# lmcinnes/pynndescent

Measured on AMD Instinct MI355X. Metric: index build: points indexed/sec (recall@10 vs brute force reported alongside), higher is better.
Workload: dtype f32

## Files before the change

include/pynnd_amd.h:

```cpp
#ifndef PYNND_AMD_H
#define PYNND_AMD_H

#include <stdint.h>

#ifdef __cplusplus
extern "C" {
#endif

#define NND_METRIC_SQEUCLIDEAN 0
#define NND_METRIC_ALT_COSINE 1
#define NND_METRIC_ALT_DOT 2
#define NND_METRIC_ALT_INNER_PRODUCT 3
#define NND_METRIC_CORRELATION 4
#define NND_METRIC_ALT_HELLINGER 5

#define NND_ABI_VERSION 6

typedef struct nnd_handle_s *nnd_handle_t;

typedef struct nnd_params {
    int64_t n;
    int32_t dim;
    int32_t metric;
    int32_t n_neighbors;
    int32_t n_trees;
    int32_t leaf_size;
    int32_t max_depth;
    int32_t max_candidates;
    int32_t n_iters;
    float delta;
    int64_t rng_state[3];
    int64_t tree_rng[3];
    int32_t device;
    int32_t join_blocks;
    int32_t flags;
    int32_t reserved[5];
} nnd_params;

#define NND_FLAG_NO_GRAPH 1
#define NND_FLAG_NO_PREP 2
#define NND_FLAG_TEST_SELECT_WAVE 4
#define NND_FLAG_TEST_SMALL_REGIONS 8
#define NND_FLAG_TEST_ROUTE_PLAIN 16
#define NND_FLAG_TEST_FOREST_BY_TREE 32
#define NND_FLAG_TEST_FAIL 64
#define NND_FLAG_TEST_VANISH 128
#define NND_FLAG_TEST_SAMPLE_ATOMIC 256
#define NND_FLAG_TEST_FOREST_FALLBACK_TOPS 512
#define NND_FLAG_TEST_FOREST_FALLBACK_SHARE 1024
#define NND_TEST_FALLBACK_AT(flags) ((((flags) & 512) ? 1 : 0) + (((flags) & 1024) ? 2 : 0))
#define NND_FLAG_TEST_SAMPLE_NOMEM 2048
#define NND_FLAG_TEST_SELECT_HALF 4096
#define NND_FLAG_TEST_GATHER_INLINE 8192
#define NND_FLAG_TEST_JOIN_UNSTAGED 16384

typedef struct nnd_stats {
    int64_t n_iters_run;
    int64_t n_leaves;
    int64_t tree_levels;
    int64_t leaf_pairs;
    int64_t leaf_rows;
    int64_t join_pairs[64];
    int64_t join_rows[64];
    int64_t join_active[64];
    int64_t proposals[64];
    int64_t updates[64];
    float ms_prep, ms_forest, ms_leaf_init, ms_random_init, ms_descent, ms_finalize;
    float ms_sample[64], ms_join[64], ms_merge[64];
    int64_t join_mfma[64];
    int64_t leaf_mfma;
    int64_t n_cells;
    int64_t join_substeps[64];
} nnd_stats;

int32_t nnd_abi_version(void);
const char *nnd_last_global_error(void);
const char *nnd_last_error(nnd_handle_t h);

int32_t nnd_create(nnd_handle_t *out, const nnd_params *params);
int32_t nnd_destroy(nnd_handle_t h);
int32_t nnd_release_pending(void);

int32_t nnd_host_copy(void *dst, const void *src, int64_t bytes);
int32_t nnd_host_sqrt_f32(float *dst, const float *src, int64_t count);
void *nnd_host_alloc(int64_t bytes);
int32_t nnd_host_free(void *p);

int32_t nnd_set_data_host(nnd_handle_t h, const float *x);
int32_t nnd_set_data_device(nnd_handle_t h, const float *x_dev);
int32_t nnd_data_nonfinite(nnd_handle_t h, int32_t *out);
int32_t nnd_data_negative(nnd_handle_t h, int32_t *out);

int32_t nnd_make_forest(nnd_handle_t h);
int32_t nnd_leaf_array_shape(nnd_handle_t h, int64_t *n_leaves, int32_t *max_leaf_size);
int32_t nnd_get_leaf_array(nnd_handle_t h, int32_t *out_host);

int32_t nnd_reset_graph(nnd_handle_t h);
int32_t nnd_init_from_leaves(nnd_handle_t h);
int32_t nnd_init_from_leaf_array(nnd_handle_t h, const int32_t *leaf_array, int64_t n_leaves, int32_t max_leaf_size);
int32_t nnd_init_random(nnd_handle_t h);
int32_t nnd_init_from_graph(nnd_handle_t h, const int32_t *init_idx, const float *init_dist, int32_t width);
int32_t nnd_init_from_neighbor_graph(nnd_handle_t h, const int32_t *init_idx, const float *init_dist, int32_t width);

int32_t nnd_descent_iter(nnd_handle_t h, int64_t *c_out);
int32_t nnd_descent(nnd_handle_t h);

int32_t nnd_finalize_host(nnd_handle_t h, int32_t *out_idx, float *out_dist);
int32_t nnd_finalize_device(nnd_handle_t h, int32_t *out_idx_dev, float *out_dist_dev);

int32_t nnd_build_device(nnd_handle_t h, int32_t *out_idx_dev, float *out_dist_dev);

int32_t nnd_build(const nnd_params *params, const float *x, const int32_t *init_idx, const float *init_dist,
                  int32_t init_width, int32_t *out_idx, float *out_dist, nnd_stats *stats, char *err,
                  int32_t errlen);

int32_t nnd_get_stats(nnd_handle_t h, nnd_stats *out);
int32_t nnd_synchronize(nnd_handle_t h);

int32_t nnd_get_graph(nnd_handle_t h, int32_t *idx, float *dist, uint8_t *flags);
int32_t nnd_get_candidates(nnd_handle_t h, int32_t *new_idx, int32_t *old_idx);
int32_t nnd_sample_candidates(nnd_handle_t h);
int32_t nnd_pairwise_gram(nnd_handle_t h, const int32_t *rows_a, int32_t na, const int32_t *rows_b, int32_t nb,
                          float *out);

typedef struct nnd_comm_s *nnd_comm_t;
#define NND_COMM_ID_BYTES 128
int32_t nnd_comm_unique_id(void *id_out );
int32_t nnd_comm_create_rccl(nnd_comm_t *out, const void *id, int32_t world, int32_t rank, int32_t device);
int32_t nnd_comm_create_local(nnd_comm_t *out , int32_t world, const int32_t *devices );
typedef int32_t (*nnd_host_exchange_fn)(void *user, const void *send, const int64_t *send_off, const int64_t *send_bytes,
                                        void *recv, const int64_t *recv_off, const int64_t *recv_bytes);
int32_t nnd_comm_create_host(nnd_comm_t *out, int32_t world, int32_t rank, int32_t device, nnd_host_exchange_fn fn, void *user);
int32_t nnd_comm_add_channel_rccl(nnd_comm_t c, const void *id );
int32_t nnd_comm_set_timeout(nnd_comm_t c, int64_t timeout_ms);
int32_t nnd_comm_destroy(nnd_comm_t c);
int32_t nnd_comm_abort(nnd_comm_t c);
int32_t nnd_comm_info(nnd_comm_t c, int32_t *out );
int32_t nnd_comm_self_test(nnd_comm_t c);
int32_t nnd_comm_local_set_serial(nnd_comm_t c, int32_t on);
const char *nnd_comm_last_error(nnd_comm_t c );

typedef struct nnd_shard_s *nnd_shard_t;
typedef struct nnd_shard_info {
    int64_t n_total, own_lo, own_hi;
    int32_t world, rank, local_trees, iters;
    int64_t c[64];
    int64_t offer_records[64];
    int64_t proposal_records[64];
    int64_t deferred[64];
    int64_t dropped_offers;
    int64_t bytes_sent;
    float ms_total;
    float ms_allgather, ms_klist_exchange;
    int32_t n_sections;
    float section_ms[256];
    int64_t section_bytes[256];
    int32_t forest_by_cell;
    int32_t n_sections_overlap;
    int64_t forest_positions;
    int64_t gather_bytes[64];
    int32_t gather_section[64];
} nnd_shard_info;
int32_t nnd_shard_create(nnd_shard_t *out, const nnd_params *params, nnd_comm_t comm, const int64_t *shard_sizes);
int32_t nnd_shard_build(nnd_shard_t s, const float *x_local_dev, void *x_stream, int32_t *out_idx_dev, float *out_dist_dev);
int32_t nnd_shard_build_from_graph(nnd_shard_t s, const float *x_local_dev, void *x_stream, const int32_t *init_idx_dev,
                                   const float *init_dist_dev, int32_t init_width, int32_t *out_idx_dev, float *out_dist_dev);
int32_t nnd_shard_build_update(nnd_shard_t s, const float *x_local_dev, void *x_stream, const int32_t *old_idx_dev, const float *old_dist_dev,
                               int32_t width, int32_t *out_idx_dev, float *out_dist_dev);
int32_t nnd_shard_get_info(nnd_shard_t s, nnd_shard_info *out);
int32_t nnd_shard_get_stats(nnd_shard_t s, nnd_stats *out);
nnd_handle_t nnd_shard_handle(nnd_shard_t s);
int32_t nnd_shard_destroy(nnd_shard_t s);
const char *nnd_shard_last_error(nnd_shard_t s );

int32_t nnd_build_multi(const nnd_params *params, const float *x, int32_t n_devices, const int32_t *devices, int32_t *out_idx,
                        float *out_dist, nnd_stats *stats, nnd_shard_info *info_rank0 , char *err, int32_t errlen);
int32_t nnd_build_multi_from_graph(const nnd_params *params, const float *x, int32_t n_devices, const int32_t *devices,
                                   const int32_t *init_idx, const float *init_dist, int32_t init_width, int32_t *out_idx, float *out_dist,
                                   nnd_stats *stats, nnd_shard_info *info_rank0 , char *err, int32_t errlen);
int32_t nnd_build_multi_update(const nnd_params *params, const float *x, int32_t n_devices, const int32_t *devices, const int32_t *old_idx,
                               const float *old_dist, int32_t width, int32_t *out_idx, float *out_dist, nnd_stats *stats,
                               nnd_shard_info *info_rank0 , char *err, int32_t errlen);

int32_t nnd_set_stream(nnd_handle_t h, void *hip_stream);
int32_t nnd_descent_sample(nnd_handle_t h);
int32_t nnd_descent_join(nnd_handle_t h);

typedef struct nnd_prune_opts {
    float prune_probability;
    int32_t degree_aware;
    int32_t max_degree;
    float aggressiveness;
    float alpha;
    uint32_t seed;
    int32_t reserved[2];
} nnd_prune_opts;
int32_t nnd_diversify_host(nnd_handle_t h, int32_t *idx, float *dist, const nnd_prune_opts *opts, const int32_t *degree);
int32_t nnd_diversify_csr_host(nnd_handle_t h, const int32_t *indptr, const int32_t *indices, float *data, int64_t nnz,
                               const nnd_prune_opts *opts, const int32_t *degree);
int32_t nnd_degree_prune_host(nnd_handle_t h, const int32_t *indptr, float *data, int64_t nnz, int32_t max_degree);

typedef struct nnd_search_graph_stats {
    int64_t forward_nnz;
    int64_t reverse_nnz;
    int64_t union_nnz;
    int64_t final_nnz;
    float min_distance;
    int32_t max_degree_out;
    float ms_device;
    int32_t reserved[3];
} nnd_search_graph_stats;
int32_t nnd_search_graph(nnd_handle_t h, const int32_t *idx, const float *dist, int32_t on_device, int32_t n_neighbors,
                         float pruning_degree_multiplier, float diversify_prob, int32_t degree_aware, float degree_prune_aggressiveness,
                         uint32_t seed, int32_t *fwd_rows_host, float *fwd_dist_host, nnd_search_graph_stats *stats);
int32_t nnd_search_graph_fetch(nnd_handle_t h, int32_t *indptr_host, int32_t *indices_host);

int32_t nnd_hub_tree_build(nnd_handle_t h, const int32_t *rank_order_host, int32_t leaf_size, int32_t max_depth,
                           int64_t *n_nodes_out);
int32_t nnd_hub_tree_fetch(nnd_handle_t h, float *hyperplanes, float *offsets, int32_t *children, int32_t *indices,
                           int32_t *max_leaf_size);

typedef struct nnd_searcher_s *nnd_searcher_t;
int32_t nnd_searcher_create(nnd_searcher_t *out, int32_t device, int64_t n, int32_t dim, int32_t metric, const float *data,
                            const int32_t *indptr, const int32_t *indices, int64_t nnz, const float *hyperplanes,
                            const float *offsets, const int32_t *children, const int32_t *tree_indices, int64_t n_nodes,
                            float min_distance, int32_t n_neighbors, const int64_t *search_rng_state );
int32_t nnd_searcher_query(nnd_searcher_t s, const float *queries , int64_t nq, int32_t k, float epsilon,
                           int32_t *out_idx , float *out_dist );
int64_t nnd_searcher_last_spilled(nnd_searcher_t s);
int32_t nnd_searcher_set_tier(nnd_searcher_t s, int32_t tier);
int32_t nnd_searcher_quantize_u8(nnd_searcher_t s, const float *rows , const float *values, int32_t n_values,
                                 uint8_t *codes_out );
int32_t nnd_searcher_set_codes_u8(nnd_searcher_t s, const float *values, int32_t n_values, const uint8_t *codes );
int32_t nnd_searcher_query_proxy(nnd_searcher_t s, const float *queries , int64_t nq, int32_t k, int32_t search_k,
                                 float epsilon, int32_t *out_idx , float *out_dist );
int32_t nnd_searcher_destroy(nnd_searcher_t s);
const char *nnd_searcher_last_error(nnd_searcher_t s );

#ifdef __cplusplus
}
#endif
#endif
```

pynndescent_amd/_capi.py:

```python
import ctypes as C
import os

import numpy as np

_HERE = os.path.dirname(os.path.abspath(__file__))
LIB_PATH = os.environ.get("PYNND_AMD_LIB", os.path.join(_HERE, "libpynnd_amd.so"))

NND_METRIC_SQEUCLIDEAN = 0
NND_METRIC_ALT_COSINE = 1
NND_METRIC_ALT_DOT = 2
NND_METRIC_ALT_INNER_PRODUCT = 3
NND_METRIC_CORRELATION = 4
NND_METRIC_ALT_HELLINGER = 5
METRIC_CODES = {"euclidean": NND_METRIC_SQEUCLIDEAN, "l2": NND_METRIC_SQEUCLIDEAN, "sqeuclidean": NND_METRIC_SQEUCLIDEAN,
                "cosine": NND_METRIC_ALT_COSINE, "dot": NND_METRIC_ALT_DOT, "inner_product": NND_METRIC_ALT_INNER_PRODUCT,
                "correlation": NND_METRIC_CORRELATION, "hellinger": NND_METRIC_ALT_HELLINGER}
NND_FLAG_NO_GRAPH = 1
NND_FLAG_NO_PREP = 2
NND_FLAG_TEST_SELECT_WAVE = 4
NND_FLAG_TEST_SMALL_REGIONS = 8
NND_FLAG_TEST_ROUTE_PLAIN = 16
NND_FLAG_TEST_FOREST_BY_TREE = 32
NND_FLAG_TEST_FAIL = 64
NND_FLAG_TEST_VANISH = 128
NND_FLAG_TEST_FOREST_FALLBACK_TOPS = 512
NND_FLAG_TEST_FOREST_FALLBACK_SHARE = 1024
NND_FLAG_TEST_GATHER_INLINE = 8192
NND_FLAG_TEST_JOIN_UNSTAGED = 16384
NND_FLAG_TEST_SELECT_HALF = 4096
NND_FLAG_TEST_SAMPLE_NOMEM = 2048
NND_FLAG_TEST_SAMPLE_ATOMIC = 256


class NNDParams(C.Structure):
    _fields_ = [
        ("n", C.c_int64),
        ("dim", C.c_int32),
        ("metric", C.c_int32),
        ("n_neighbors", C.c_int32),
        ("n_trees", C.c_int32),
        ("leaf_size", C.c_int32),
        ("max_depth", C.c_int32),
        ("max_candidates", C.c_int32),
        ("n_iters", C.c_int32),
        ("delta", C.c_float),
        ("rng_state", C.c_int64 * 3),
        ("tree_rng", C.c_int64 * 3),
        ("device", C.c_int32),
        ("join_blocks", C.c_int32),
        ("flags", C.c_int32),
        ("reserved", C.c_int32 * 5),
    ]


class NNDSearchGraphStats(C.Structure):
    _fields_ = [("forward_nnz", C.c_int64), ("reverse_nnz", C.c_int64), ("union_nnz", C.c_int64), ("final_nnz", C.c_int64),
                ("min_distance", C.c_float), ("max_degree_out", C.c_int32), ("ms_device", C.c_float), ("reserved", C.c_int32 * 3)]


class NNDStats(C.Structure):
    _fields_ = [
        ("n_iters_run", C.c_int64),
        ("n_leaves", C.c_int64),
        ("tree_levels", C.c_int64),
        ("leaf_pairs", C.c_int64),
        ("leaf_rows", C.c_int64),
        ("join_pairs", C.c_int64 * 64),
        ("join_rows", C.c_int64 * 64),
        ("join_active", C.c_int64 * 64),
        ("proposals", C.c_int64 * 64),
        ("updates", C.c_int64 * 64),
        ("ms_prep", C.c_float),
        ("ms_forest", C.c_float),
        ("ms_leaf_init", C.c_float),
        ("ms_random_init", C.c_float),
        ("ms_descent", C.c_float),
        ("ms_finalize", C.c_float),
        ("ms_sample", C.c_float * 64),
        ("ms_join", C.c_float * 64),
        ("ms_merge", C.c_float * 64),
        ("join_mfma", C.c_int64 * 64),
        ("leaf_mfma", C.c_int64),
        ("n_cells", C.c_int64),
        ("join_substeps", C.c_int64 * 64),
    ]

    def as_dict(self):
        it = int(self.n_iters_run)
        m = min(it, 64)
        out = {
            "n_iters_run": it, "n_leaves": int(self.n_leaves), "tree_levels": int(self.tree_levels),
            "leaf_pairs": int(self.leaf_pairs), "leaf_rows": int(self.leaf_rows), "leaf_mfma": int(self.leaf_mfma), "n_cells": int(self.n_cells),
        }
        for name in ("join_pairs", "join_rows", "join_active", "proposals", "updates", "join_mfma", "join_substeps"):
            out[name] = [int(v) for v in getattr(self, name)[:m]]
        for name in ("ms_prep", "ms_forest", "ms_leaf_init", "ms_random_init", "ms_descent", "ms_finalize"):
            out[name] = float(getattr(self, name))
        for name in ("ms_sample", "ms_join", "ms_merge"):
            out[name] = [float(v) for v in getattr(self, name)[:m]]
        return out


class NNDShardInfo(C.Structure):
    _fields_ = [
        ("n_total", C.c_int64), ("own_lo", C.c_int64), ("own_hi", C.c_int64),
        ("world", C.c_int32), ("rank", C.c_int32), ("local_trees", C.c_int32), ("iters", C.c_int32),
        ("c", C.c_int64 * 64),
        ("offer_records", C.c_int64 * 64),
        ("proposal_records", C.c_int64 * 64),
        ("deferred", C.c_int64 * 64),
        ("dropped_offers", C.c_int64),
        ("bytes_sent", C.c_int64),
        ("ms_total", C.c_float), ("ms_allgather", C.c_float), ("ms_klist_exchange", C.c_float),
        ("n_sections", C.c_int32),
        ("section_ms", C.c_float * 256),
        ("section_bytes", C.c_int64 * 256),
        ("forest_by_cell", C.c_int32),
        ("n_sections_overlap", C.c_int32),
        ("forest_positions", C.c_int64),
        ("gather_bytes", C.c_int64 * 64),
        ("gather_section", C.c_int32 * 64),
    ]

    def as_dict(self):
        it = min(int(self.iters), 64)
        ns = int(self.n_sections)
        return {"n_total": int(self.n_total), "range": (int(self.own_lo), int(self.own_hi)), "world": int(self.world),
                "rank": int(self.rank), "local_trees": int(self.local_trees), "iters": int(self.iters),
                "c": [int(v) for v in self.c[:it]], "offer_records": [int(v) for v in self.offer_records[:it]],
                "proposal_records": [int(v) for v in self.proposal_records[:it]],
                "exchanged_records": [int(a) + int(b) for a, b in zip(self.offer_records[:it], self.proposal_records[:it])],
                "deferred": [int(v) for v in self.deferred[:it]], "dropped_offers": int(self.dropped_offers),
                "bytes_sent": int(self.bytes_sent), "ms_total": float(self.ms_total),
                "ms_allgather": float(self.ms_allgather), "ms_klist_exchange": float(self.ms_klist_exchange),
                "section_ms": [float(v) for v in self.section_ms[:ns]],
                "section_bytes": [int(v) for v in self.section_bytes[:ns]],
                "forest_by_cell": bool(self.forest_by_cell), "n_sections_overlap": int(self.n_sections_overlap),
                "forest_positions": int(self.forest_positions),
                "gather_bytes": [int(v) for v in self.gather_bytes[:it]], "gather_section": [int(v) for v in self.gather_section[:it]]}


HOST_EXCHANGE_FN = C.CFUNCTYPE(C.c_int32, C.c_void_p, C.c_void_p, C.POINTER(C.c_int64), C.POINTER(C.c_int64), C.c_void_p,
                               C.POINTER(C.c_int64), C.POINTER(C.c_int64))


class NNDPruneOpts(C.Structure):
    _fields_ = [
        ("prune_probability", C.c_float),
        ("degree_aware", C.c_int32),
        ("max_degree", C.c_int32),
        ("aggressiveness", C.c_float),
        ("alpha", C.c_float),
        ("seed", C.c_uint32),
        ("reserved", C.c_int32 * 2),
    ]


_H = C.c_void_p
_SIGNATURES = [
    ("nnd_abi_version", C.c_int32, []),
    ("nnd_last_global_error", C.c_char_p, []),
    ("nnd_last_error", C.c_char_p, [_H]),
    ("nnd_create", C.c_int32, [C.POINTER(_H), C.POINTER(NNDParams)]),
    ("nnd_destroy", C.c_int32, [_H]),
    ("nnd_set_data_host", C.c_int32, [_H, C.c_void_p]),
    ("nnd_set_data_device", C.c_int32, [_H, C.c_void_p]),
    ("nnd_data_nonfinite", C.c_int32, [_H, C.POINTER(C.c_int32)]),
    ("nnd_data_negative", C.c_int32, [_H, C.POINTER(C.c_int32)]),
    ("nnd_release_pending", C.c_int32, []),
    ("nnd_host_copy", C.c_int32, [C.c_void_p, C.c_void_p, C.c_int64]),
    ("nnd_host_sqrt_f32", C.c_int32, [C.c_void_p, C.c_void_p, C.c_int64]),
    ("nnd_host_alloc", C.c_void_p, [C.c_int64]),
    ("nnd_host_free", C.c_int32, [C.c_void_p]),
    ("nnd_make_forest", C.c_int32, [_H]),
    ("nnd_leaf_array_shape", C.c_int32, [_H, C.POINTER(C.c_int64), C.POINTER(C.c_int32)]),
    ("nnd_get_leaf_array", C.c_int32, [_H, C.c_void_p]),
    ("nnd_reset_graph", C.c_int32, [_H]),
    ("nnd_init_from_leaves", C.c_int32, [_H]),
    ("nnd_init_from_leaf_array", C.c_int32, [_H, C.c_void_p, C.c_int64, C.c_int32]),
    ("nnd_init_random", C.c_int32, [_H]),
    ("nnd_init_from_graph", C.c_int32, [_H, C.c_void_p, C.c_void_p, C.c_int32]),
    ("nnd_init_from_neighbor_graph", C.c_int32, [_H, C.c_void_p, C.c_void_p, C.c_int32]),
    ("nnd_descent_iter", C.c_int32, [_H, C.POINTER(C.c_int64)]),
    ("nnd_descent", C.c_int32, [_H]),
    ("nnd_finalize_host", C.c_int32, [_H, C.c_void_p, C.c_void_p]),
    ("nnd_finalize_device", C.c_int32, [_H, C.c_void_p, C.c_void_p]),
    ("nnd_build_device", C.c_int32, [_H, C.c_void_p, C.c_void_p]),
    ("nnd_build", C.c_int32, [C.POINTER(NNDParams), C.c_void_p, C.c_void_p, C.c_void_p, C.c_int32, C.c_void_p,
                              C.c_void_p, C.POINTER(NNDStats), C.c_char_p, C.c_int32]),
    ("nnd_get_stats", C.c_int32, [_H, C.POINTER(NNDStats)]),
    ("nnd_synchronize", C.c_int32, [_H]),
    ("nnd_get_graph", C.c_int32, [_H, C.c_void_p, C.c_void_p, C.c_void_p]),
    ("nnd_get_candidates", C.c_int32, [_H, C.c_void_p, C.c_void_p]),
    ("nnd_sample_candidates", C.c_int32, [_H]),
    ("nnd_pairwise_gram", C.c_int32, [_H, C.c_void_p, C.c_int32, C.c_void_p, C.c_int32, C.c_void_p]),
    ("nnd_descent_sample", C.c_int32, [_H]),
    ("nnd_descent_join", C.c_int32, [_H]),
    ("nnd_set_stream", C.c_int32, [_H, C.c_void_p]),
    ("nnd_comm_unique_id", C.c_int32, [C.c_void_p]),
    ("nnd_comm_create_rccl", C.c_int32, [C.POINTER(_H), C.c_void_p, C.c_int32, C.c_int32, C.c_int32]),
    ("nnd_comm_create_local", C.c_int32, [C.POINTER(_H), C.c_int32, C.c_void_p]),
    ("nnd_comm_create_host", C.c_int32, [C.POINTER(_H), C.c_int32, C.c_int32, C.c_int32, C.c_void_p, C.c_void_p]),
    ("nnd_comm_add_channel_rccl", C.c_int32, [_H, C.c_void_p]),
    ("nnd_comm_set_timeout", C.c_int32, [_H, C.c_int64]),
    ("nnd_comm_info", C.c_int32, [_H, C.POINTER(C.c_int32)]),
    ("nnd_comm_self_test", C.c_int32, [_H]),
    ("nnd_comm_destroy", C.c_int32, [_H]),
    ("nnd_comm_abort", C.c_int32, [_H]),
    ("nnd_comm_local_set_serial", C.c_int32, [_H, C.c_int32]),
    ("nnd_comm_last_error", C.c_char_p, [_H]),
    ("nnd_shard_create", C.c_int32, [C.POINTER(_H), C.POINTER(NNDParams), _H, C.c_void_p]),
    ("nnd_shard_build", C.c_int32, [_H, C.c_void_p, C.c_void_p, C.c_void_p, C.c_void_p]),
    ("nnd_shard_get_info", C.c_int32, [_H, C.POINTER(NNDShardInfo)]),
    ("nnd_shard_get_stats", C.c_int32, [_H, C.POINTER(NNDStats)]),
    ("nnd_shard_handle", _H, [_H]),
    ("nnd_shard_destroy", C.c_int32, [_H]),
    ("nnd_shard_last_error", C.c_char_p, [_H]),
    ("nnd_build_multi", C.c_int32, [C.POINTER(NNDParams), C.c_void_p, C.c_int32, C.c_void_p, C.c_void_p, C.c_void_p,
                                    C.POINTER(NNDStats), C.POINTER(NNDShardInfo), C.c_char_p, C.c_int32]),
    ("nnd_build_multi_from_graph", C.c_int32, [C.POINTER(NNDParams), C.c_void_p, C.c_int32, C.c_void_p, C.c_void_p, C.c_void_p, C.c_int32,
                                               C.c_void_p, C.c_void_p, C.POINTER(NNDStats), C.POINTER(NNDShardInfo), C.c_char_p, C.c_int32]),
    ("nnd_shard_build_from_graph", C.c_int32, [_H, C.c_void_p, C.c_void_p, C.c_void_p, C.c_void_p, C.c_int32, C.c_void_p, C.c_void_p]),
    ("nnd_shard_build_update", C.c_int32, [_H, C.c_void_p, C.c_void_p, C.c_void_p, C.c_void_p, C.c_int32, C.c_void_p, C.c_void_p]),
    ("nnd_build_multi_update", C.c_int32, [C.POINTER(NNDParams), C.c_void_p, C.c_int32, C.c_void_p, C.c_void_p, C.c_void_p, C.c_int32,
                                           C.c_void_p, C.c_void_p, C.POINTER(NNDStats), C.POINTER(NNDShardInfo), C.c_char_p, C.c_int32]),
    ("nnd_diversify_host", C.c_int32, [_H, C.c_void_p, C.c_void_p, C.POINTER(NNDPruneOpts), C.c_void_p]),
    ("nnd_diversify_csr_host", C.c_int32, [_H, C.c_void_p, C.c_void_p, C.c_void_p, C.c_int64, C.POINTER(NNDPruneOpts),
                                           C.c_void_p]),
    ("nnd_degree_prune_host", C.c_int32, [_H, C.c_void_p, C.c_void_p, C.c_int64, C.c_int32]),
    ("nnd_search_graph", C.c_int32, [_H, C.c_void_p, C.c_void_p, C.c_int32, C.c_int32, C.c_float, C.c_float, C.c_int32, C.c_float, C.c_uint32,
                                     C.c_void_p, C.c_void_p, C.POINTER(NNDSearchGraphStats)]),
    ("nnd_search_graph_fetch", C.c_int32, [_H, C.c_void_p, C.c_void_p]),
    ("nnd_hub_tree_build", C.c_int32, [_H, C.c_void_p, C.c_int32, C.c_int32, C.POINTER(C.c_int64)]),
    ("nnd_hub_tree_fetch", C.c_int32, [_H, C.c_void_p, C.c_void_p, C.c_void_p, C.c_void_p, C.POINTER(C.c_int32)]),
    ("nnd_searcher_create", C.c_int32, [C.POINTER(_H), C.c_int32, C.c_int64, C.c_int32, C.c_int32, C.c_void_p, C.c_void_p, C.c_void_p,
                                        C.c_int64, C.c_void_p, C.c_void_p, C.c_void_p, C.c_void_p, C.c_int64, C.c_float, C.c_int32,
                                        C.c_void_p]),
    ("nnd_searcher_query", C.c_int32, [_H, C.c_void_p, C.c_int64, C.c_int32, C.c_float, C.c_void_p, C.c_void_p]),
    ("nnd_searcher_last_spilled", C.c_int64, [_H]),
    ("nnd_searcher_set_tier", C.c_int32, [_H, C.c_int32]),
    ("nnd_searcher_quantize_u8", C.c_int32, [_H, C.c_void_p, C.c_void_p, C.c_int32, C.c_void_p]),
    ("nnd_searcher_set_codes_u8", C.c_int32, [_H, C.c_void_p, C.c_int32, C.c_void_p]),
    ("nnd_searcher_query_proxy", C.c_int32, [_H, C.c_void_p, C.c_int64, C.c_int32, C.c_int32, C.c_float, C.c_void_p, C.c_void_p]),
    ("nnd_searcher_destroy", C.c_int32, [_H]),
    ("nnd_searcher_last_error", C.c_char_p, [_H]),
]
EXPORTED_SYMBOLS = [s[0] for s in _SIGNATURES]

_lib = None


def load_library():
    global _lib
    if _lib is not None:
        return _lib
    if not os.path.exists(LIB_PATH):
        raise RuntimeError(
            "%s not found: build it with `python -c 'import __graft_entry__ as g; g.build()'` or "
            "`make -C pynndescent_amd/csrc`. pynndescent_amd has no CPU fallback." % LIB_PATH
        )
    lib = C.CDLL(LIB_PATH)
    for name, restype, argtypes in _SIGNATURES:
        fn = getattr(lib, name)
        fn.restype = restype
        fn.argtypes = argtypes
    _lib = lib
    return lib


def _ptr(a):
    return None if a is None else a.ctypes.data_as(C.c_void_p)


class NNDError(RuntimeError):
    pass


class Builder:

    def __init__(self, n, dim, metric, n_neighbors, n_trees, leaf_size, max_depth, max_candidates, n_iters, delta,
                 rng_state, tree_rng, device=0, join_blocks=0, flags=0):
        self.lib = load_library()
        p = NNDParams()
        p.n, p.dim, p.metric = int(n), int(dim), int(metric)
        p.n_neighbors, p.n_trees, p.leaf_size = int(n_neighbors), int(n_trees), int(leaf_size)
        p.max_depth, p.max_candidates, p.n_iters = int(max_depth), int(max_candidates), int(n_iters)
        p.delta = float(delta)
        for i in range(3):
            p.rng_state[i] = int(rng_state[i])
            p.tree_rng[i] = int(tree_rng[i])
        p.device, p.join_blocks, p.flags = int(device), int(join_blocks), int(flags)
        self.params = p
        self.n, self.dim, self.k, self.mc = int(n), int(dim), int(n_neighbors), int(max_candidates)
        self._h = _H()
        if self.lib.nnd_create(C.byref(self._h), C.byref(p)) != 0:
            raise NNDError(self.lib.nnd_last_global_error().decode())
        self._keepalive = None

    def _check(self, rc):
        if rc != 0:
            raise NNDError(self.lib.nnd_last_error(self._h).decode())

    def close(self):
        if getattr(self, "_h", None) is not None and self._h.value:
            self.lib.nnd_destroy(self._h)
            self._h = _H()

    def __del__(self):
        try:
            self.close()
        except Exception:
            pass

    def set_data_host(self, x):
        x = np.ascontiguousarray(x, dtype=np.float32)
        assert x.shape == (self.n, self.dim)
        self._check(self.lib.nnd_set_data_host(self._h, _ptr(x)))

    def data_nonfinite(self):
        out = C.c_int32()
        self._check(self.lib.nnd_data_nonfinite(self._h, C.byref(out)))
        return bool(out.value)

    def data_negative(self):
        out = C.c_int32()
        self._check(self.lib.nnd_data_negative(self._h, C.byref(out)))
        return bool(out.value)

    def set_data_device(self, dev_ptr, keepalive=None):
        self._keepalive = keepalive
        self._check(self.lib.nnd_set_data_device(self._h, C.c_void_p(int(dev_ptr))))

    def make_forest(self):
        self._check(self.lib.nnd_make_forest(self._h))

    def leaf_array(self):
        nl, ms = C.c_int64(), C.c_int32()
        self._check(self.lib.nnd_leaf_array_shape(self._h, C.byref(nl), C.byref(ms)))
        out = np.empty((max(nl.value, 1), max(ms.value, 1)), np.int32)
        self._check(self.lib.nnd_get_leaf_array(self._h, _ptr(out)))
        return out[: nl.value]

    def reset_graph(self):
        self._check(self.lib.nnd_reset_graph(self._h))

    def init_from_leaves(self):
        self._check(self.lib.nnd_init_from_leaves(self._h))

    def init_from_leaf_array(self, leaf_array):
        la = np.ascontiguousarray(leaf_array, dtype=np.int32)
        assert la.ndim == 2
        self._check(self.lib.nnd_init_from_leaf_array(self._h, _ptr(la), la.shape[0], la.shape[1]))

    def init_random(self):
        self._check(self.lib.nnd_init_random(self._h))

    def init_from_graph(self, idx, dist=None):
        idx = np.ascontiguousarray(idx, np.int32)
        dist = None if dist is None else np.ascontiguousarray(dist, np.float32)
        self._check(self.lib.nnd_init_from_graph(self._h, _ptr(idx), _ptr(dist), idx.shape[1]))

    def init_from_neighbor_graph(self, idx, dist):
        idx = np.ascontiguousarray(idx, np.int32)
        dist = np.ascontiguousarray(dist, np.float32)
        self._check(self.lib.nnd_init_from_neighbor_graph(self._h, _ptr(idx), _ptr(dist), idx.shape[1]))

    def descent_iter(self):
        c = C.c_int64()
        self._check(self.lib.nnd_descent_iter(self._h, C.byref(c)))
        return c.value

    def descent(self):
        self._check(self.lib.nnd_descent(self._h))

    def sample_candidates(self):
        self._check(self.lib.nnd_sample_candidates(self._h))

    def finalize(self):
        idx = host_pool.empty((self.n, self.k), np.int32)
        dist = host_pool.empty((self.n, self.k), np.float32)
        self._check(self.lib.nnd_finalize_host(self._h, _ptr(idx), _ptr(dist)))
        return idx, dist

    def finalize_device(self, idx_ptr, dist_ptr):
        self._check(self.lib.nnd_finalize_device(self._h, C.c_void_p(int(idx_ptr)), C.c_void_p(int(dist_ptr))))

    def build_device(self, idx_ptr, dist_ptr):
        self._check(self.lib.nnd_build_device(self._h, C.c_void_p(int(idx_ptr)), C.c_void_p(int(dist_ptr))))

    def synchronize(self):
        self._check(self.lib.nnd_synchronize(self._h))

    def stats(self, raw=False):
        s = NNDStats()
        self._check(self.lib.nnd_get_stats(self._h, C.byref(s)))
        return s if raw else s.as_dict()

    def graph(self):
        idx = np.empty((self.n, self.k), np.int32)
        dist = np.empty((self.n, self.k), np.float32)
        flags = np.empty((self.n, self.k), np.uint8)
        self._check(self.lib.nnd_get_graph(self._h, _ptr(idx), _ptr(dist), _ptr(flags)))
        return idx, dist, flags

    def candidates(self):
        new = np.empty((self.n, self.mc), np.int32)
        old = np.empty((self.n, self.mc), np.int32)
        self._check(self.lib.nnd_get_candidates(self._h, _ptr(new), _ptr(old)))
        return new, old

    def set_stream(self, stream_ptr):
        self._check(self.lib.nnd_set_stream(self._h, C.c_void_p(int(stream_ptr)) if stream_ptr else None))

    def descent_sample(self):
        self._check(self.lib.nnd_descent_sample(self._h))

    def descent_join(self):
        self._check(self.lib.nnd_descent_join(self._h))

    @staticmethod
    def _prune_opts(prune_probability=1.0, degree_aware=False, max_degree=1, aggressiveness=1.0, alpha=1.0, seed=0):
        o = NNDPruneOpts()
        o.prune_probability, o.degree_aware, o.max_degree = float(prune_probability), int(bool(degree_aware)), int(max_degree)
        o.aggressiveness, o.alpha, o.seed = float(aggressiveness), float(alpha), int(seed) & 0xFFFFFFFF
        return o

    def diversify(self, idx, dist, degree=None, **opts):
        idx = np.ascontiguousarray(idx, np.int32).copy()
        dist = np.ascontiguousarray(dist, np.float32).copy()
        assert idx.shape == (self.n, self.k) and dist.shape == idx.shape
        o = self._prune_opts(**opts)
        degree = None if degree is None else np.ascontiguousarray(degree, np.int32)
        self._check(self.lib.nnd_diversify_host(self._h, _ptr(idx), _ptr(dist), C.byref(o), _ptr(degree)))
        return idx, dist

    def diversify_csr(self, indptr, indices, data, degree=None, **opts):
        indptr = np.ascontiguousarray(indptr, np.int32)
        indices = np.ascontiguousarray(indices, np.int32)
        data = np.ascontiguousarray(data, np.float32).copy()
        assert indptr.shape[0] == self.n + 1
        o = self._prune_opts(**opts)
        degree = None if degree is None else np.ascontiguousarray(degree, np.int32)
        self._check(self.lib.nnd_diversify_csr_host(self._h, _ptr(indptr), _ptr(indices), _ptr(data), data.shape[0],
                                                    C.byref(o), _ptr(degree)))
        return data

    def search_graph(self, idx, dist, n_neighbors, pruning_degree_multiplier=1.5, diversify_prob=1.0, degree_aware=False,
                     degree_prune_aggressiveness=1.0, seed=0, on_device=False, want_forward=False):
        st = NNDSearchGraphStats()
        fr = fd = None
        if want_forward:
            fr = np.empty((self.n, self.k), np.int32)
            fd = np.empty((self.n, self.k), np.float32)
        if on_device:
            pi, pd = C.c_void_p(int(idx)), C.c_void_p(int(dist))
        else:
            idx = np.ascontiguousarray(idx, dtype=np.int32)
            dist = np.ascontiguousarray(dist, dtype=np.float32)
            assert idx.shape == (self.n, self.k) and dist.shape == (self.n, self.k)
            pi, pd = _ptr(idx), _ptr(dist)
        self._check(self.lib.nnd_search_graph(self._h, pi, pd, 1 if on_device else 0, int(n_neighbors), float(pruning_degree_multiplier),
                                              float(diversify_prob), 1 if degree_aware else 0, float(degree_prune_aggressiveness),
                                              int(seed) & 0xFFFFFFFF, _ptr(fr) if want_forward else None, _ptr(fd) if want_forward else None,
                                              C.byref(st)))
        indptr = np.empty(self.n + 1, np.int32)
        indices = np.empty(max(int(st.final_nnz), 1), np.int32)
        self._check(self.lib.nnd_search_graph_fetch(self._h, _ptr(indptr), _ptr(indices)))
        stats = {f: getattr(st, f) for f, _ in NNDSearchGraphStats._fields_ if f != "reserved"}
        out = (indptr, indices[: int(st.final_nnz)], stats)
        return out + (fr, fd) if want_forward else out

    def degree_prune(self, indptr, data, max_degree):
        indptr = np.ascontiguousarray(indptr, np.int32)
        data = np.ascontiguousarray(data, np.float32).copy()
        self._check(self.lib.nnd_degree_prune_host(self._h, _ptr(indptr), _ptr(data), data.shape[0], int(max_degree)))
        return data

    def hub_tree(self, rank_order, leaf_size, max_depth):
        ro = np.ascontiguousarray(rank_order, np.int32)
        assert ro.shape == (self.n,)
        nn = C.c_int64()
        self._check(self.lib.nnd_hub_tree_build(self._h, _ptr(ro), int(leaf_size), int(max_depth), C.byref(nn)))
        hyper = np.empty((nn.value, self.dim), np.float32)
        offs = np.empty((nn.value,), np.float32)
        children = np.empty((nn.value, 2), np.int32)
        indices = np.empty((self.n,), np.int32)
        ml = C.c_int32()
        self._check(self.lib.nnd_hub_tree_fetch(self._h, _ptr(hyper), _ptr(offs), _ptr(children), _ptr(indices), C.byref(ml)))
        return hyper, offs, children, indices, int(ml.value)

    def pairwise_gram(self, rows_a, rows_b):
        a = np.ascontiguousarray(rows_a, np.int32)
        b = np.ascontiguousarray(rows_b, np.int32)
        out = np.empty((a.shape[0], b.shape[0]), np.float32)
        self._check(self.lib.nnd_pairwise_gram(self._h, _ptr(a), a.shape[0], _ptr(b), b.shape[0], _ptr(out)))
        return out


class Searcher:

    def __init__(self, data, search_graph, tree, metric, min_distance, n_neighbors, search_rng_state, device=0):
        self.lib = load_library()
        data = np.ascontiguousarray(data, np.float32)
        self.n, self.dim = data.shape
        indptr = np.ascontiguousarray(search_graph.indptr, np.int32)
        indices = np.ascontiguousarray(search_graph.indices, np.int32)
        if tree is not None:
            hyper = np.ascontiguousarray(tree.hyperplanes, np.float32)
            offs = np.ascontiguousarray(tree.offsets, np.float32)
            children = np.ascontiguousarray(tree.children, np.int32)
            tidx = np.ascontiguousarray(tree.indices, np.int32)
            n_nodes = hyper.shape[0]
        else:
            hyper = offs = children = tidx = None
            n_nodes = 0
        rng = np.ascontiguousarray(search_rng_state, np.int64)
        self.has_codes = False
        self._h = _H()
        rc = self.lib.nnd_searcher_create(C.byref(self._h), int(device), self.n, self.dim, int(metric), _ptr(data), _ptr(indptr),
                                          _ptr(indices), int(indices.shape[0]), _ptr(hyper), _ptr(offs), _ptr(children), _ptr(tidx),
                                          int(n_nodes), float(min_distance), int(n_neighbors), _ptr(rng))
        if rc != 0:
            raise NNDError(self.lib.nnd_searcher_last_error(None).decode())

    def query(self, queries, k, epsilon):
        q = np.ascontiguousarray(queries, np.float32)
        assert q.ndim == 2 and q.shape[1] == self.dim
        idx = np.empty((q.shape[0], k), np.int32)
        dist = np.empty((q.shape[0], k), np.float32)
        if self.lib.nnd_searcher_query(self._h, _ptr(q), q.shape[0], int(k), float(epsilon), _ptr(idx), _ptr(dist)) != 0:
            raise NNDError(self.lib.nnd_searcher_last_error(self._h).decode())
        return idx, dist

    def quantize_u8(self, values, rows=None, fetch=True):
        values = np.ascontiguousarray(values, np.float32)
        if rows is not None:
            rows = np.ascontiguousarray(rows, np.float32)
            assert rows.shape == (self.n, self.dim)
        codes = np.empty((self.n, self.dim), np.uint8) if fetch else None
        if self.lib.nnd_searcher_quantize_u8(self._h, _ptr(rows), _ptr(values), int(values.shape[0]), _ptr(codes)) != 0:
            raise NNDError(self.lib.nnd_searcher_last_error(self._h).decode())
        self.has_codes = True
        return codes

    def set_codes_u8(self, values, codes):
        values = np.ascontiguousarray(values, np.float32)
        codes = np.ascontiguousarray(codes, np.uint8)
        assert codes.shape == (self.n, self.dim)
        if self.lib.nnd_searcher_set_codes_u8(self._h, _ptr(values), int(values.shape[0]), _ptr(codes)) != 0:
            raise NNDError(self.lib.nnd_searcher_last_error(self._h).decode())
# ... 109 lines not shown
```

pynndescent_amd/csrc/capi.hip:

```cpp
#include <stdlib.h>
#include <string.h>

#include <atomic>
#include <mutex>
#include <string>
#include <thread>
#include <vector>

#include "common.h"
#include "state.h"

static thread_local char g_err[512] = {0};

static void gerr(const char *fmt, ...) {
    va_list ap;
    va_start(ap, fmt);
    vsnprintf(g_err, sizeof(g_err), fmt, ap);
    va_end(ap);
}

extern "C" int32_t nnd_abi_version(void) { return NND_ABI_VERSION; }
extern "C" const char *nnd_last_global_error(void) { return g_err; }
extern "C" const char *nnd_last_error(nnd_handle_t h) { return h ? h->err : g_err; }

#define API_HIP(expr)                                                                                \
    do {                                                                                             \
        hipError_t _e = (expr);                                                                      \
        if (_e != hipSuccess) {                                                                      \
            ctx->set_error("%s failed: %s (%s:%d)", #expr, hipGetErrorString(_e), __FILE__, __LINE__); \
            return 1;                                                                                \
        }                                                                                            \
    } while (0)

void nnd_release_parked();
template <typename T>
static int dalloc(nnd_ctx *ctx, T **p, size_t count) {
    if (hipMalloc((void **)p, sizeof(T) * (count ? count : 1)) != hipSuccess) {
        (void)hipGetLastError();
        nnd_release_parked();
        API_HIP(hipMalloc((void **)p, sizeof(T) * (count ? count : 1)));
    }
    static const int poison = [] { const char *e = nnd_knob("NND_POISON"); return e ? atoi(e) : 0; }();
    if (poison) {
        API_HIP(hipMemsetAsync(*p, poison & 0xFF, sizeof(T) * (count ? count : 1), ctx->stream));
        API_HIP(hipStreamSynchronize(ctx->stream));
    }
    return 0;
}

struct nnd_scratch {
    std::vector<void *> ptrs;
    ~nnd_scratch() {
        for (void *p : ptrs)
            if (p) (void)hipFree(p);
    }
    template <typename T>
    T *get(nnd_ctx *ctx, size_t count) {
        void *p = nullptr;
        hipError_t e = hipMalloc(&p, sizeof(T) * (count ? count : 1));
        if (e != hipSuccess) {
            ctx->set_error("hipMalloc of %zu scratch bytes failed: %s", sizeof(T) * count, hipGetErrorString(e));
            return nullptr;
        }
        ptrs.push_back(p);
        return (T *)p;
    }
};

std::recursive_mutex &nnd_lifecycle_mutex() {
#ifdef NND_TEST_NO_LIFECYCLE_LOCK
    static thread_local std::recursive_mutex m;
#else
    static std::recursive_mutex m;
#endif
    return m;
}

static void free_all(nnd_ctx *ctx) {
    auto F = [](void *p) {
        if (p) (void)hipFree(p);
    };
    if (ctx->x_owned) F((void *)ctx->x_orig);
    for (void *&a : ctx->slim_alloc) { F(a); a = nullptr; }
    F(ctx->xp); F(ctx->nrm); F(ctx->nr2); F(ctx->xh); F(ctx->mean); F(ctx->knn_e); F(ctx->knn_d); F(ctx->th); F(ctx->pbuf_r);
    F(ctx->pdirty); F(ctx->out_idx); F(ctx->out_dist);
    F(ctx->rv_pos); F(ctx->rv_in_cursor); F(ctx->rv_in_rec); F(ctx->rv_ov);
    for (int i = 0; i < 2; i++) { F(ctx->perm[i]); F(ctx->pos_seg[i]); F(ctx->seg_start[i]); F(ctx->seg_len[i]); }
    F(ctx->inv); F(ctx->side); F(ctx->side_pt); F(ctx->leaf_flag); F(ctx->scan_out); F(ctx->scan_blk); F(ctx->seg_nleft); F(ctx->seg_child);
    F(ctx->xs); F(ctx->xsh); F(ctx->nr2s); F(ctx->node_hf); F(ctx->node_hh); F(ctx->node_child); F(ctx->node_pack); F(ctx->node_hfc); F(ctx->route_roots); F(ctx->route_ws); F(ctx->s_leaf_depth);
    F(ctx->cell_count); F(ctx->cell_start); F(ctx->cell_depth); F(ctx->small_list);
    F(ctx->hyper); F(ctx->hyper_h); F(ctx->leaf_start); F(ctx->leaf_len); F(ctx->wl_start); F(ctx->wl_len); F(ctx->colsum_partial); F(ctx->counters_sum);
    if (ctx->h_pin) { (void)hipHostFree(ctx->h_pin); ctx->h_pin = nullptr; }
    if (ctx->h_tree_begin) { (void)hipHostFree(ctx->h_tree_begin); ctx->h_tree_begin = nullptr; }
    F(ctx->tree_begin_dev); F(ctx->counters);
    if (ctx->ev0) (void)hipEventDestroy(ctx->ev0);
    if (ctx->ev1) (void)hipEventDestroy(ctx->ev1);
    if (ctx->ev_spin) (void)hipEventDestroy(ctx->ev_spin);
    for (hipEvent_t e : ctx->tev) if (e) (void)hipEventDestroy(e);
    ctx->tev.clear();
    F(ctx->shard_bounds); F(ctx->shard_cursors);
    nnd_hub_tree_free(ctx);
    nnd_search_graph_free(ctx);
    if (ctx->stream && ctx->stream_owned) (void)hipStreamDestroy(ctx->stream);
}

static nnd_ctx *take_parked(const nnd_params *p);
extern "C" int32_t nnd_create(nnd_handle_t *out, const nnd_params *p) { return nnd_create_impl(out, p, nullptr, 0, 0); }

static void jb_knobs(nnd_ctx *ctx) {
    if (const char *e = nnd_knob("NND_JB_MAX")) ctx->jb_max = atoi(e) < 1 ? 1 : atoi(e);
    if (const char *e = nnd_knob("NND_JB_DIV")) ctx->jb_div = atoi(e) < 1 ? 1 : atoi(e);
    if (const char *e = nnd_knob("NND_JB_FIRST")) ctx->jb_first = atoi(e) < 0 ? 0 : atoi(e);
}
static int auto_join_blocks(int k, int mc) { return (k <= 64 ? 1 : (k + 31) / 32) * (mc > 64 ? 2 : 1); }

int nnd_create_impl(nnd_handle_t *out, const nnd_params *p, const int64_t *bounds_host, int n_ranks, int rank) {
    if (!out || !p) { gerr("nnd_create: null argument"); return 1; }
    *out = nullptr;
    if (p->n < 1 || p->dim < 1) { gerr("nnd_create: need n >= 1 and dim >= 1 (got n=%lld dim=%d)", (long long)p->n, p->dim); return 1; }
    if (p->metric < NND_METRIC_SQEUCLIDEAN || p->metric > NND_METRIC_ALT_HELLINGER) { gerr("nnd_create: unknown metric %d", p->metric); return 1; }
    if (p->n_neighbors < 1 || p->n_neighbors > NND_WIDE_K) { gerr("nnd_create: n_neighbors must be in 1..%d (got %d)", NND_WIDE_K, p->n_neighbors); return 1; }
    if (p->max_candidates < 1 || p->max_candidates > 128) { gerr("nnd_create: max_candidates must be in 1..128 (got %d)", p->max_candidates); return 1; }
    if (p->n_trees < 0 || p->n_trees > 4096 || p->leaf_size < 1) { gerr("nnd_create: bad n_trees (0..4096) / leaf_size"); return 1; }
    if (p->n >= (int64_t)0x7FFFFFF0) { gerr("nnd_create: n too large for int32 ids"); return 1; }
    if (p->n_trees > 0 && (int64_t)p->n_trees * p->n >= (int64_t)0x7FFFFFF0) {
        gerr("nnd_create: n_trees * n = %lld exceeds the forest's int32 position space (2^31)", (long long)((int64_t)p->n_trees * p->n));
        return 1;
    }
    int ndev = 0;
    if (hipGetDeviceCount(&ndev) != hipSuccess || ndev == 0) { gerr("nnd_create: no HIP device visible (this library has no CPU path)"); return 1; }
    if (p->device < 0 || p->device >= ndev) { gerr("nnd_create: device %d out of range (%d visible)", p->device, ndev); return 1; }
    hipDeviceProp_t prop;
    if (hipGetDeviceProperties(&prop, p->device) != hipSuccess) { gerr("nnd_create: hipGetDeviceProperties failed"); return 1; }
    if (strncmp(prop.gcnArchName, "gfx950", 6) != 0) { gerr("nnd_create: device %d is %s; this build targets gfx950 (MI355X) only", p->device, prop.gcnArchName); return 1; }
    if (hipSetDevice(p->device) != hipSuccess) { gerr("nnd_create: hipSetDevice failed"); return 1; }
    if (!bounds_host) {
        if (nnd_ctx *parked = take_parked(p)) {
            *out = parked;
            return 0;
        }
        nnd_release_parked();
    }

    std::lock_guard<std::recursive_mutex> lifecycle(nnd_lifecycle_mutex());
    nnd_ctx *ctx = new nnd_ctx();
    ctx->p = *p;
    ctx->n = p->n;
    ctx->own_lo = 0;
    ctx->own_hi = p->n;
    if (bounds_host) {
        if (n_ranks < 1 || n_ranks > 64 || rank < 0 || rank >= n_ranks || bounds_host[0] != 0 || bounds_host[n_ranks] != p->n) {
            gerr("nnd_create: bad shard bounds (need 1 <= n_ranks <= 64, bounds from 0 to n)");
            delete ctx;
            return 1;
        }
        for (int r = 0; r < n_ranks; r++)
            if (bounds_host[r] > bounds_host[r + 1]) { gerr("nnd_create: shard bounds must not decrease"); delete ctx; return 1; }
        ctx->n_ranks = n_ranks;
        ctx->own_lo = bounds_host[rank];
        ctx->own_hi = bounds_host[rank + 1];
        ctx->slim = n_ranks > 1;
    }
    ctx->d = p->dim;
    ctx->dp = (p->dim + 31) & ~31;
    ctx->k = p->n_neighbors;
    ctx->ks = (p->n_neighbors + 15) & ~15;
    ctx->mc = p->max_candidates;
    ctx->mcp = p->max_candidates <= 16 ? 16 : (p->max_candidates <= 32 ? 32 : (p->max_candidates <= 64 ? 64 : 128));
    if (ctx->ks > 64 && ctx->mcp < 32) ctx->mcp = 32;
    ctx->rcap = p->max_candidates <= 32 ? 32 : (p->max_candidates <= 64 ? 64 : 128);
    if (const char *rc_env = nnd_knob("NND_RCAP")) {
        const int r = atoi(rc_env);
        if (r == 16 || r == 32 || r == 64) ctx->rcap = r;
    }
    ctx->pcap = 64;
    if (const char *pc_env = nnd_knob("NND_PCAP")) {
        const int r = atoi(pc_env);
        if (r == 16 || r == 32 || r == 64) ctx->pcap = r;
    }
    ctx->jb_auto = ctx->p.join_blocks < 1;
    if (ctx->p.join_blocks < 1) ctx->p.join_blocks = auto_join_blocks(ctx->p.n_neighbors, ctx->p.max_candidates);
    jb_knobs(ctx);
    ctx->seed = nnd_mix32((uint32_t)p->rng_state[0] ^ nnd_mix32((uint32_t)p->rng_state[1] + 0x9E3779B9u) ^
                          nnd_mix32((uint32_t)p->rng_state[2] + 0x7F4A7C15u));
    ctx->tree_seed = nnd_mix32((uint32_t)p->tree_rng[0] ^ nnd_mix32((uint32_t)p->tree_rng[1] + 0x9E3779B9u) ^
                               nnd_mix32((uint32_t)p->tree_rng[2] + 0x7F4A7C15u));
    int rc = 0;
    do {
        if (hipStreamCreateWithFlags(&ctx->stream, hipStreamNonBlocking) != hipSuccess) { ctx->set_error("hipStreamCreate failed"); rc = 1; break; }
        if (hipEventCreate(&ctx->ev0) != hipSuccess || hipEventCreate(&ctx->ev1) != hipSuccess ||
            hipEventCreateWithFlags(&ctx->ev_spin, hipEventDisableTiming) != hipSuccess) { ctx->set_error("hipEventCreate failed"); rc = 1; break; }
        const size_t n = (size_t)ctx->n;
        const bool graph = !(p->flags & NND_FLAG_NO_GRAPH), prepared = !(p->flags & NND_FLAG_NO_PREP);
        if (!prepared && graph) { ctx->set_error("NND_FLAG_NO_PREP needs NND_FLAG_NO_GRAPH (the build reads the prepared rows)"); rc = 1; break; }
        if (prepared) {
            if ((rc = dalloc(ctx, &ctx->xp, n * ctx->dp))) break;
            if ((rc = dalloc(ctx, &ctx->nrm, n))) break;
            if (p->n_trees > 0 && (rc = dalloc(ctx, &ctx->xh, n * ctx->dp))) break;
            if (p->n_trees > 0 && (rc = dalloc(ctx, &ctx->nr2, n))) break;
            if ((rc = dalloc(ctx, &ctx->mean, (size_t)ctx->dp + 4))) break;
        }
        if (graph) {
            if ((rc = dalloc(ctx, &ctx->knn_e, n * ctx->ks))) break;
            if ((rc = dalloc(ctx, &ctx->knn_d, n * ctx->ks))) break;
            if ((rc = dalloc(ctx, &ctx->th, n))) break;
            const size_t rows = ctx->slim ? (size_t)(ctx->own_hi - ctx->own_lo) : n;
            int32_t *a_cand = nullptr;
            uint32_t *a_rbuf = nullptr;
            uint8_t *a_active = nullptr;
            if ((rc = dalloc(ctx, &a_cand, rows * 2 * ctx->mcp))) break;
            ctx->slim_alloc[0] = a_cand;
            if ((rc = dalloc(ctx, &a_rbuf, rows * 2 * ctx->rcap))) break;
            ctx->slim_alloc[1] = a_rbuf;
            if ((rc = dalloc(ctx, &a_active, rows))) break;
            ctx->slim_alloc[2] = a_active;
            ctx->cand = a_cand - (size_t)ctx->own_lo * (ctx->slim ? 1 : 0) * 2 * ctx->mcp;
            ctx->rbuf = a_rbuf - (size_t)ctx->own_lo * (ctx->slim ? 1 : 0) * 2 * ctx->rcap;
            ctx->active = a_active - (size_t)ctx->own_lo * (ctx->slim ? 1 : 0);
            uint64_t *a_pbuf = nullptr;
            if ((rc = dalloc(ctx, &a_pbuf, rows * ctx->pcap))) break;
            ctx->slim_alloc[3] = a_pbuf;
            ctx->pbuf = a_pbuf - (size_t)ctx->own_lo * (ctx->slim ? 1 : 0) * ctx->pcap;
            if (ctx->slim && (rc = dalloc(ctx, &ctx->pbuf_r, n * ctx->pcap_r))) break;
            if ((rc = dalloc(ctx, &ctx->pdirty, n))) break;
            if (hipMemsetAsync(ctx->pdirty, 0, n, ctx->stream) != hipSuccess) { ctx->set_error("hipMemset failed"); rc = 1; break; }
            if (ctx->n_ranks > 0) {
                if (hipMalloc((void **)&ctx->shard_bounds, sizeof(int64_t) * 65) != hipSuccess || hipMalloc((void **)&ctx->shard_cursors, sizeof(long long) * 66) != hipSuccess ||
                    hipMemcpy(ctx->shard_bounds, bounds_host, sizeof(int64_t) * (size_t)(n_ranks + 1), hipMemcpyHostToDevice) != hipSuccess) {
                    ctx->set_error("allocation of the shard tables failed"); rc = 1; break;
                }
            }
        }
        if ((rc = dalloc(ctx, &ctx->counters, (size_t)CNT_COUNT * NND_CNT_STRIPES))) break;
        if ((rc = dalloc(ctx, &ctx->counters_sum, (size_t)CNT_COUNT))) break;
        if (hipHostMalloc((void **)&ctx->h_pin, sizeof(nnd_pin_words), hipHostMallocDefault) != hipSuccess) { ctx->set_error("hipHostMalloc failed"); rc = 1; break; }
        memset(ctx->h_pin, 0, sizeof(nnd_pin_words));
        if (hipHostGetDevicePointer((void **)&ctx->h_pin_dev, ctx->h_pin, 0) != hipSuccess) { (void)hipGetLastError(); ctx->h_pin_dev = nullptr; }
        if (p->n_trees > 0) {
            ctx->P = (int64_t)p->n_trees * ctx->n;
            const size_t P = (size_t)ctx->P;
            ctx->max_segs = ctx->P / (p->leaf_size + 1) + p->n_trees + 8;
            const char *whole = nnd_knob("NND_FOREST_WHOLE");
            if (graph && p->n >= 131072 && ctx->dp <= 256 && !(whole && whole[0] == '1')) {
                const char *ss = nnd_knob("NND_SAMPLE_STRIDE");
                ctx->s_stride = ss ? atoi(ss) : 16;
                if (ctx->s_stride < 2) ctx->s_stride = 2;
                ctx->s_m = p->n / ctx->s_stride;
                const char *cl = nnd_knob("NND_CELL_LEAF");
                const char *es = nnd_knob("NND_EARLY_STOP");
                ctx->early_stop = es ? atoi(es) : 0;
                ctx->cell_leaf = cl ? atoi(cl) : 24;
                if (ctx->cell_leaf < 8) ctx->cell_leaf = 8;
                const int64_t Ps = (int64_t)p->n_trees * ctx->s_m;
                ctx->node_cap = Ps / (ctx->cell_leaf / 4 > 1 ? ctx->cell_leaf / 4 : 1) + 4 * p->n_trees + 64;
                ctx->cell_cap = ctx->node_cap + p->n_trees;
                ctx->max_segs += ctx->cell_cap;
                if ((rc = dalloc(ctx, &ctx->xs, (size_t)ctx->s_m * ctx->dp))) break;
                if ((rc = dalloc(ctx, &ctx->xsh, (size_t)ctx->s_m * ctx->dp))) break;
                if ((rc = dalloc(ctx, &ctx->nr2s, (size_t)ctx->s_m))) break;
                if ((rc = dalloc(ctx, &ctx->node_hf, (size_t)ctx->node_cap * (ctx->dp + 4)))) break;
                if ((rc = dalloc(ctx, &ctx->node_hh, (size_t)ctx->node_cap * ctx->dp))) break;
                if ((rc = dalloc(ctx, &ctx->node_child, (size_t)ctx->node_cap * 2))) break;
                if ((rc = dalloc(ctx, &ctx->node_pack, (size_t)ctx->node_cap * (2 * ctx->dp + 16)))) break;
                if ((rc = dalloc(ctx, &ctx->node_hfc, (size_t)ctx->node_cap * (ctx->dp + 4)))) break;
                if ((rc = dalloc(ctx, &ctx->route_roots, (size_t)NND_ROUTE_ROOTS_WORDS))) break;
                if ((rc = dalloc(ctx, &ctx->s_leaf_depth, (size_t)Ps))) break;
                if ((rc = dalloc(ctx, &ctx->cell_count, (size_t)ctx->cell_cap))) break;
                if ((rc = dalloc(ctx, &ctx->cell_start, (size_t)ctx->cell_cap))) break;
                if ((rc = dalloc(ctx, &ctx->cell_depth, (size_t)ctx->cell_cap))) break;
                if ((rc = dalloc(ctx, &ctx->small_list, (size_t)ctx->cell_cap * NND_WORK_LIST_ROWS))) break;
            }
            const size_t S = (size_t)ctx->max_segs;
            for (int i = 0; i < 2 && !rc; i++) {
                if ((rc = dalloc(ctx, &ctx->perm[i], P))) break;
                if ((rc = dalloc(ctx, &ctx->pos_seg[i], P))) break;
                if ((rc = dalloc(ctx, &ctx->seg_start[i], S))) break;
                if ((rc = dalloc(ctx, &ctx->seg_len[i], S))) break;
            }
            if (rc) break;
            if ((rc = dalloc(ctx, &ctx->inv, P))) break;
            if ((rc = dalloc(ctx, &ctx->side, P))) break;
            if ((rc = dalloc(ctx, &ctx->side_pt, P))) break;
            if ((rc = dalloc(ctx, &ctx->leaf_flag, P))) break;
            if ((rc = dalloc(ctx, &ctx->scan_out, P + 1))) break;
            if ((rc = dalloc(ctx, &ctx->scan_blk, P / 2048 + 2))) break;
            if ((rc = dalloc(ctx, &ctx->seg_nleft, S))) break;
            if ((rc = dalloc(ctx, &ctx->seg_child, (NND_SEG_CHILD_WORDS + NND_WORK_LIST_ROWS) * S))) break;
            if ((rc = dalloc(ctx, &ctx->hyper, S * (size_t)(ctx->dp + 4)))) break;
            if ((rc = dalloc(ctx, &ctx->hyper_h, S * (size_t)ctx->dp))) break;
            if ((rc = dalloc(ctx, &ctx->tree_begin_dev, (size_t)4097))) break;
            if (hipHostMalloc((void **)&ctx->h_tree_begin, sizeof(long long) * (size_t)4097, hipHostMallocDefault) != hipSuccess) { ctx->set_error("hipHostMalloc failed"); rc = 1; break; }
        }
    } while (0);
    if (rc) {
        gerr("nnd_create: %s", ctx->err);
        free_all(ctx);
        delete ctx;
        return 1;
    }
    *out = ctx;
    return 0;
}

static std::mutex g_park_mu;
static nnd_ctx *g_parked = nullptr;

static void destroy_now(nnd_ctx *ctx) {
    std::lock_guard<std::recursive_mutex> lifecycle(nnd_lifecycle_mutex());
    (void)hipSetDevice(ctx->p.device);
    if (ctx->stream) (void)hipStreamSynchronize(ctx->stream);
    free_all(ctx);
    delete ctx;
}
void nnd_release_parked() {
    nnd_ctx *old = nullptr;
    {
        std::lock_guard<std::mutex> lk(g_park_mu);
        old = g_parked;
        g_parked = nullptr;
    }
    if (old) destroy_now(old);
}
static bool same_geometry(const nnd_params &a, const nnd_params &b) {
    return a.n == b.n && a.dim == b.dim && a.metric == b.metric && a.n_neighbors == b.n_neighbors && a.n_trees == b.n_trees &&
           a.leaf_size == b.leaf_size && a.max_candidates == b.max_candidates && a.device == b.device && a.flags == b.flags;
}
static nnd_ctx *take_parked(const nnd_params *p) {
    nnd_ctx *ctx = nullptr;
    {
        std::lock_guard<std::mutex> lk(g_park_mu);
        if (g_parked && same_geometry(g_parked->p, *p)) {
            ctx = g_parked;
            g_parked = nullptr;
        }
    }
    if (!ctx) return nullptr;
    (void)hipSetDevice(p->device);
    ctx->p = *p;
    jb_knobs(ctx);
    ctx->jb_auto = ctx->p.join_blocks < 1;
    if (ctx->p.join_blocks < 1) ctx->p.join_blocks = auto_join_blocks(ctx->p.n_neighbors, ctx->p.max_candidates);
    ctx->seed = nnd_mix32((uint32_t)p->rng_state[0] ^ nnd_mix32((uint32_t)p->rng_state[1] + 0x9E3779B9u) ^ nnd_mix32((uint32_t)p->rng_state[2] + 0x7F4A7C15u));
    ctx->tree_seed = nnd_mix32((uint32_t)p->tree_rng[0] ^ nnd_mix32((uint32_t)p->tree_rng[1] + 0x9E3779B9u) ^ nnd_mix32((uint32_t)p->tree_rng[2] + 0x7F4A7C15u));
    ctx->iter = 0;
    ctx->stats = nnd_stats{};
    ctx->err[0] = 0;
    ctx->forest_built = false;
    ctx->h_leaf_valid = false;
    ctx->n_leaves = 0;
    ctx->max_leaf = 0;
    ctx->own_order = nullptr;
    ctx->lists_replicated = false;
    nnd_hub_tree_free(ctx);
    if (!ctx->stream_owned) {
        ctx->stream = nullptr;
        if (hipStreamCreateWithFlags(&ctx->stream, hipStreamNonBlocking) != hipSuccess) { destroy_now(ctx); return nullptr; }
        ctx->stream_owned = true;
    }
    if (!ctx->x_owned) ctx->x_orig = nullptr;
    ctx->x_valid = false;
    ctx->tlog.clear();
    ctx->tev_used = 0;
    return ctx;
}

extern "C" int32_t nnd_destroy(nnd_handle_t ctx) {
    if (!ctx) return 0;
    (void)hipSetDevice(ctx->p.device);
    if (ctx->stream) (void)hipStreamSynchronize(ctx->stream);
    nnd_ctx *old = nullptr;
    if (ctx->n_ranks == 0) {
        std::lock_guard<std::mutex> lk(g_park_mu);
        old = g_parked;
        g_parked = ctx;
    } else {
        old = ctx;
    }
    if (old) destroy_now(old);
    return 0;
}
extern "C" int32_t nnd_release_pending(void) {
    nnd_release_parked();
    return 0;
}

#define ENTER(ctx)                                           \
    if (!ctx) { gerr("null handle"); return 1; }             \
    API_HIP(hipSetDevice(ctx->p.device));

static int need_data(nnd_ctx *ctx) {
    if (!ctx->x_orig || !ctx->x_valid) { ctx->set_error("no data set (call nnd_set_data_host/device first)"); return 1; }
    return 0;
}
static int need_graph(nnd_ctx *ctx) {
    if (ctx->p.flags & NND_FLAG_NO_GRAPH) { ctx->set_error("this handle was created with NND_FLAG_NO_GRAPH: it has no k-lists / candidate tables (pruning pass and hub tree only)"); return 1; }
    return 0;
}

static int after_data(nnd_ctx *ctx) {
    if (ctx->p.flags & NND_FLAG_NO_PREP) return 0;
    const int t_ = t_begin(ctx);
    if (nnd_launch_prep(ctx)) return 1;
    if (!(ctx->p.flags & NND_FLAG_NO_GRAPH) && nnd_launch_reset_graph(ctx)) return 1;
    t_end(ctx, t_, &ctx->stats.ms_prep, false);
    t_flush(ctx);
    return 0;
}

static std::mutex g_up_mu[64];
static char *g_up_stage[64][16] = {};
static hipEvent_t g_up_ev[64][16] = {};
static int h2d_parallel(nnd_ctx *ctx, void *dst_dev, const void *src, size_t bytes) {
    constexpr size_t STAGE = (size_t)8 << 20;
    int P = 8;
    if (const char *e = nnd_knob("NND_H2D_THREADS")) { const int v = atoi(e); if (v >= 1 && v <= 16) P = v; }
    bool direct = bytes < (size_t)(16u << 20) || ctx->p.device < 0 || ctx->p.device >= 64;
    if (!direct) {
        hipPointerAttribute_t at;
        if (hipPointerGetAttributes(&at, src) == hipSuccess && at.type == hipMemoryTypeHost) direct = true;
        else (void)hipGetLastError();
    }
    if (direct) {
        API_HIP(hipMemcpyAsync(dst_dev, src, bytes, hipMemcpyHostToDevice, ctx->stream));
        return 0;
    }
    const int dev = ctx->p.device;
    std::lock_guard<std::mutex> lk(g_up_mu[dev]);
    API_HIP(hipSetDevice(dev));
    for (int b = 0; b < P; b++) {
        if (!g_up_stage[dev][b] && hipHostMalloc((void **)&g_up_stage[dev][b], STAGE, hipHostMallocDefault) != hipSuccess) {
            (void)hipGetLastError();
            g_up_stage[dev][b] = nullptr;
            API_HIP(hipMemcpyAsync(dst_dev, src, bytes, hipMemcpyHostToDevice, ctx->stream));
            return 0;
        }
        if (!g_up_ev[dev][b]) API_HIP(hipEventCreateWithFlags(&g_up_ev[dev][b], hipEventDisableTiming));
    }
    const size_t nchunks = (bytes + STAGE - 1) / STAGE;
    std::atomic<int> failed{0};
    hipStream_t st = ctx->stream;
    auto work = [&](int t) {
        if (hipSetDevice(dev) != hipSuccess) { failed = 1; return; }
        bool first = true;
        for (size_t c = (size_t)t; c < nchunks && !failed; c += P) {
            const size_t o = c * STAGE, len = bytes - o < STAGE ? bytes - o : STAGE;
            if (!first && hipEventSynchronize(g_up_ev[dev][t]) != hipSuccess) { failed = 1; return; }
            first = false;
            memcpy(g_up_stage[dev][t], (const char *)src + o, len);
            if (hipMemcpyAsync((char *)dst_dev + o, g_up_stage[dev][t], len, hipMemcpyHostToDevice, st) != hipSuccess ||
                hipEventRecord(g_up_ev[dev][t], st) != hipSuccess) { failed = 1; return; }
        }
        if (!first && hipEventSynchronize(g_up_ev[dev][t]) != hipSuccess) failed = 1;
    };
    std::vector<std::thread> th;
    for (int t = 1; t < P; t++) th.emplace_back(work, t);
    work(0);
    for (auto &t : th) t.join();
    if (failed) {
        (void)hipStreamSynchronize(st);
        (void)hipGetLastError();
        ctx->set_error("nnd_set_data_host: staged host-to-device copy failed");
        return 1;
    }
// ... 298 lines not shown
                if (po >= len) break;
                const size_t pl = len - po < piece ? len - po : piece;
                th.emplace_back([=] { memcpy(to + po, from + po, pl); });
            }
            memcpy(to, from, len < piece ? len : piece);
            for (auto &t : th) t.join();
        }
    }
    return 0;
}

template <typename F>
static void host_parallel(size_t bytes, size_t unit, F fn) {
    const size_t total = bytes / unit;
    int parts = bytes >= ((size_t)32 << 20) ? 16 : (bytes >= ((size_t)4 << 20) ? 8 : 1);
    const unsigned hc = std::thread::hardware_concurrency();
    if (hc && (unsigned)parts > hc) parts = (int)hc;
    const size_t per = ((total + parts - 1) / parts + (4096 / unit) - 1) / (4096 / unit) * (4096 / unit);
    std::vector<std::thread> th;
    for (int t = 1; t < parts; t++) {
        const size_t o = (size_t)t * per;
        if (o >= total) break;
        const size_t c = total - o < per ? total - o : per;
        th.emplace_back([=] { fn(o, c); });
    }
    fn(0, total < per ? total : per);
    for (auto &t : th) t.join();
}
extern "C" void *nnd_host_alloc(int64_t bytes) {
    void *p = nullptr;
    if (bytes <= 0) return nullptr;
    if (hipHostMalloc(&p, (size_t)bytes, hipHostMallocDefault) != hipSuccess) {
        (void)hipGetLastError();
        return nullptr;
    }
    return p;
}
extern "C" int32_t nnd_host_free(void *p) {
    if (p && hipHostFree(p) != hipSuccess) { (void)hipGetLastError(); gerr("nnd_host_free: not a pointer of nnd_host_alloc"); return 1; }
    return 0;
}
extern "C" int32_t nnd_host_copy(void *dst, const void *src, int64_t bytes) {
    if (bytes < 0 || (bytes > 0 && (!dst || !src))) { gerr("nnd_host_copy: bad arguments"); return 1; }
    host_parallel((size_t)bytes, 1, [=](size_t o, size_t c) { memcpy((char *)dst + o, (const char *)src + o, c); });
    return 0;
}
#if !defined(__HIP_DEVICE_COMPILE__) && (defined(__x86_64__) || defined(_M_X64))
#include <immintrin.h>
__attribute__((target("avx2"))) static void host_sqrt_avx2(float *dst, const float *src, size_t n) {
    size_t i = 0;
    for (; i + 8 <= n; i += 8) _mm256_storeu_ps(dst + i, _mm256_sqrt_ps(_mm256_loadu_ps(src + i)));
    for (; i < n; i++) dst[i] = sqrtf(src[i]);
}
static bool host_has_avx2() { return __builtin_cpu_supports("avx2"); }
#else
static void host_sqrt_avx2(float *dst, const float *src, size_t n) { for (size_t i = 0; i < n; i++) dst[i] = sqrtf(src[i]); }
static bool host_has_avx2() { return false; }
#endif
extern "C" int32_t nnd_host_sqrt_f32(float *dst, const float *src, int64_t count) {
    if (count < 0 || (count > 0 && (!dst || !src))) { gerr("nnd_host_sqrt_f32: bad arguments"); return 1; }
    const bool avx2 = host_has_avx2();
    host_parallel((size_t)count * sizeof(float), sizeof(float), [=](size_t o, size_t c) {
        if (avx2) host_sqrt_avx2(dst + o, src + o, c);
        else
            for (size_t i = o; i < o + c; i++) dst[i] = sqrtf(src[i]);
    });
    return 0;
}

static int out_buffers(nnd_ctx *ctx, size_t cnt) {
    if (cnt <= ctx->out_cap) return 0;
    if (ctx->out_idx) { API_HIP(hipFree(ctx->out_idx)); ctx->out_idx = nullptr; }
    if (ctx->out_dist) { API_HIP(hipFree(ctx->out_dist)); ctx->out_dist = nullptr; }
    ctx->out_cap = 0;
    API_HIP(hipMalloc((void **)&ctx->out_idx, sizeof(int32_t) * cnt));
    API_HIP(hipMalloc((void **)&ctx->out_dist, sizeof(float) * cnt));
    ctx->out_cap = cnt;
    return 0;
}

extern "C" int32_t nnd_finalize_host(nnd_handle_t ctx, int32_t *out_idx, float *out_dist) {
    ENTER(ctx);
    if (need_graph(ctx)) return 1;
    if (need_data(ctx)) return 1;
    size_t cnt = (size_t)(ctx->own_hi - ctx->own_lo) * ctx->k;
    if (out_buffers(ctx, cnt)) return 1;
    if (nnd_finalize_device(ctx, ctx->out_idx, ctx->out_dist)) return 1;
    if (d2h_parallel(ctx, out_idx, ctx->out_idx, sizeof(int32_t) * cnt, 4)) return 1;
    if (d2h_parallel(ctx, out_dist, ctx->out_dist, sizeof(float) * cnt, 4)) return 1;
    return 0;
}

extern "C" int32_t nnd_build_device(nnd_handle_t ctx, int32_t *out_idx_dev, float *out_dist_dev) {
    ENTER(ctx);
    if (need_graph(ctx)) return 1;
    if (need_data(ctx)) return 1;
    if (nnd_launch_reset_graph(ctx)) return 1;
    if (ctx->p.n_trees > 0) {
        const int tf = t_begin(ctx);
        if (nnd_launch_forest(ctx)) return 1;
        t_end(ctx, tf, &ctx->stats.ms_forest, false);
        const int tl = t_begin(ctx);
        if (nnd_launch_leaf_init(ctx)) return 1;
        t_end(ctx, tl, &ctx->stats.ms_leaf_init, false);
    }
    const int tr = t_begin(ctx);
    if (nnd_launch_random_init(ctx)) return 1;
    t_end(ctx, tr, &ctx->stats.ms_random_init, false);
    if (descent_loop(ctx, true)) return 1;
    const int t_ = t_begin(ctx);
    if (nnd_launch_finalize(ctx, out_idx_dev, out_dist_dev)) return 1;
    t_end(ctx, t_, &ctx->stats.ms_finalize, false);
    t_flush(ctx);
    return 0;
}

extern "C" int32_t nnd_build(const nnd_params *params, const float *x, const int32_t *init_idx, const float *init_dist,
                             int32_t init_width, int32_t *out_idx, float *out_dist, nnd_stats *stats, char *err,
                             int32_t errlen) {
    auto fail = [&](const char *msg) {
        if (err && errlen > 0) { strncpy(err, msg, (size_t)errlen - 1); err[errlen - 1] = 0; }
        return 1;
    };
    nnd_handle_t h = nullptr;
    nnd_params p = *params;
    if (init_idx) p.n_trees = 0;
    if (nnd_create(&h, &p)) return fail(g_err);
    int rc = nnd_set_data_host(h, x);
    if (!rc) {
        if (init_idx) {
            rc = nnd_init_from_graph(h, init_idx, init_dist, init_width);
            if (!rc) rc = nnd_descent(h);
            if (!rc) rc = nnd_finalize_host(h, out_idx, out_dist);
        } else {
            if (!rc) rc = out_buffers(h, (size_t)h->n * h->k);
            if (!rc) rc = nnd_build_device(h, h->out_idx, h->out_dist);
            if (!rc) rc = d2h_parallel(h, out_idx, h->out_idx, sizeof(int32_t) * (size_t)h->n * h->k, 4);
            if (!rc) rc = d2h_parallel(h, out_dist, h->out_dist, sizeof(float) * (size_t)h->n * h->k, 4);
        }
    }
    if (stats) *stats = h->stats;
    std::string msg = h->err;
    nnd_destroy(h);
    if (rc) return fail(msg.c_str());
    return 0;
}

extern "C" int32_t nnd_get_stats(nnd_handle_t ctx, nnd_stats *out) {
    if (!ctx || !out) { gerr("null argument"); return 1; }
    *out = ctx->stats;
    return 0;
}

extern "C" int32_t nnd_synchronize(nnd_handle_t ctx) {
    ENTER(ctx);
    API_HIP(nnd_sync_spin(ctx));
    return 0;
}

extern "C" int32_t nnd_get_graph(nnd_handle_t ctx, int32_t *idx, float *dist, uint8_t *flags) {
    ENTER(ctx);
    if (need_graph(ctx)) return 1;
    size_t cnt = (size_t)ctx->n * ctx->ks;
    std::vector<uint32_t> he(cnt);
    std::vector<float> hd(cnt);
    API_HIP(hipMemcpyAsync(he.data(), ctx->knn_e, sizeof(uint32_t) * cnt, hipMemcpyDeviceToHost, ctx->stream));
    API_HIP(hipMemcpyAsync(hd.data(), ctx->knn_d, sizeof(float) * cnt, hipMemcpyDeviceToHost, ctx->stream));
    API_HIP(nnd_sync_spin(ctx));
    for (int64_t v = 0; v < ctx->n; v++)
        for (int j = 0; j < ctx->k; j++) {
            uint32_t e = he[v * ctx->ks + j];
            size_t o = (size_t)v * ctx->k + j;
            if (idx) idx[o] = e == NND_EMPTY_E ? -1 : (int32_t)(e & NND_IDX_MASK);
            if (dist) dist[o] = hd[v * ctx->ks + j];
            if (flags) flags[o] = e == NND_EMPTY_E ? 0 : (uint8_t)(e >> 31);
        }
    return 0;
}

extern "C" int32_t nnd_get_candidates(nnd_handle_t ctx, int32_t *new_idx, int32_t *old_idx) {
    ENTER(ctx);
    if (need_graph(ctx)) return 1;
    size_t cnt = (size_t)ctx->n * 2 * ctx->mcp;
    std::vector<int32_t> hc(cnt);
    API_HIP(hipMemcpyAsync(hc.data(), ctx->cand, sizeof(int32_t) * cnt, hipMemcpyDeviceToHost, ctx->stream));
    API_HIP(nnd_sync_spin(ctx));
    for (int64_t v = 0; v < ctx->n; v++)
        for (int j = 0; j < ctx->mc; j++) {
            if (new_idx) new_idx[v * ctx->mc + j] = hc[v * 2 * ctx->mcp + j];
            if (old_idx) old_idx[v * ctx->mc + j] = hc[v * 2 * ctx->mcp + ctx->mcp + j];
        }
    return 0;
}

extern "C" int32_t nnd_pairwise_gram(nnd_handle_t ctx, const int32_t *rows_a, int32_t na, const int32_t *rows_b,
                                     int32_t nb, float *out) {
    ENTER(ctx);
    if (ctx->p.flags & NND_FLAG_NO_PREP) { ctx->set_error("nnd_pairwise_gram: this handle holds no prepared rows (NND_FLAG_NO_PREP)"); return 1; }
    if (need_data(ctx)) return 1;
    nnd_scratch tmp;
    int32_t *da = tmp.get<int32_t>(ctx, (size_t)na), *db = tmp.get<int32_t>(ctx, (size_t)nb);
    float *dout = tmp.get<float>(ctx, (size_t)na * nb);
    if (!da || !db || !dout) return 1;
    API_HIP(hipMemcpyAsync(da, rows_a, sizeof(int32_t) * na, hipMemcpyHostToDevice, ctx->stream));
    API_HIP(hipMemcpyAsync(db, rows_b, sizeof(int32_t) * nb, hipMemcpyHostToDevice, ctx->stream));
    if (nnd_launch_pairwise(ctx, da, na, db, nb, dout)) return 1;
    API_HIP(hipMemcpyAsync(out, dout, sizeof(float) * (size_t)na * nb, hipMemcpyDeviceToHost, ctx->stream));
    API_HIP(nnd_sync_spin(ctx));
    return 0;
}

extern "C" int32_t nnd_set_stream(nnd_handle_t ctx, void *hip_stream) {
    ENTER(ctx);
    API_HIP(hipStreamSynchronize(ctx->stream));
    if (hip_stream) {
        if (ctx->stream_owned && ctx->stream) { API_HIP(hipStreamDestroy(ctx->stream)); }
        ctx->stream = (hipStream_t)hip_stream;
        ctx->stream_owned = false;
    } else if (!ctx->stream_owned) {
        API_HIP(hipStreamCreateWithFlags(&ctx->stream, hipStreamNonBlocking));
        ctx->stream_owned = true;
    }
    return 0;
}

extern "C" int32_t nnd_descent_sample(nnd_handle_t ctx) {
    ENTER(ctx);
    if (need_graph(ctx)) return 1;
    static float sink;
    const int t_ = t_begin(ctx);
    if (nnd_launch_sample(ctx)) return 1;
    t_end(ctx, t_, ctx->iter < 64 ? &ctx->stats.ms_sample[ctx->iter] : &sink, false);
    return 0;
}
extern "C" int32_t nnd_descent_join(nnd_handle_t ctx) {
    ENTER(ctx);
    if (need_graph(ctx)) return 1;
    if (nnd_zero_counters(ctx)) return 1;
    static float sink;
    const int t_ = t_begin(ctx);
    if (nnd_launch_join(ctx, ctx->own_lo, ctx->own_hi)) return 1;
    t_end(ctx, t_, ctx->iter < 64 ? &ctx->stats.ms_join[ctx->iter] : &sink, false);
    if (nnd_read_counters(ctx)) return 1;
    t_flush(ctx);
    if (ctx->iter < 64) {
        ctx->stats.join_pairs[ctx->iter] = ctx->h_counters[CNT_PAIRS];
        ctx->stats.join_rows[ctx->iter] = ctx->h_counters[CNT_ROWS];
        ctx->stats.join_active[ctx->iter] = ctx->h_counters[CNT_ACTIVE];
        ctx->stats.proposals[ctx->iter] = ctx->h_counters[CNT_PROPOSALS];
    }
    return 0;
}

static nnd_prune_opts prune_defaults(const nnd_prune_opts *o) {
    nnd_prune_opts d{};
    d.prune_probability = 1.0f;
    d.alpha = 1.0f;
    d.max_degree = 1;
    return o ? *o : d;
}

extern "C" int32_t nnd_diversify_host(nnd_handle_t ctx, int32_t *idx , float *dist ,
                                      const nnd_prune_opts *opts, const int32_t *degree ) {
    ENTER(ctx);
    if (ctx->p.flags & NND_FLAG_NO_PREP) { ctx->set_error("nnd_diversify_host: this handle holds no prepared rows (NND_FLAG_NO_PREP)"); return 1; }
    if (need_data(ctx)) return 1;
    const nnd_prune_opts o = prune_defaults(opts);
    if (o.degree_aware && (!degree || o.max_degree < 1)) { ctx->set_error("nnd_diversify_host: the degree-aware method needs degrees and max_degree >= 1"); return 1; }
    size_t cnt = (size_t)ctx->n * ctx->k;
    nnd_scratch tmp;
    int32_t *di = tmp.get<int32_t>(ctx, cnt);
    float *dd = tmp.get<float>(ctx, cnt);
    int32_t *dg = o.degree_aware ? tmp.get<int32_t>(ctx, (size_t)ctx->n) : nullptr;
    if (!di || !dd || (o.degree_aware && !dg)) return 1;
    API_HIP(hipMemcpyAsync(di, idx, sizeof(int32_t) * cnt, hipMemcpyHostToDevice, ctx->stream));
    API_HIP(hipMemcpyAsync(dd, dist, sizeof(float) * cnt, hipMemcpyHostToDevice, ctx->stream));
    if (dg) API_HIP(hipMemcpyAsync(dg, degree, sizeof(int32_t) * (size_t)ctx->n, hipMemcpyHostToDevice, ctx->stream));
    if (nnd_launch_diversify_rows(ctx, di, dd, &o, dg)) return 1;
    API_HIP(hipMemcpyAsync(idx, di, sizeof(int32_t) * cnt, hipMemcpyDeviceToHost, ctx->stream));
    API_HIP(hipMemcpyAsync(dist, dd, sizeof(float) * cnt, hipMemcpyDeviceToHost, ctx->stream));
    API_HIP(nnd_sync_spin(ctx));
    return 0;
}

extern "C" int32_t nnd_diversify_csr_host(nnd_handle_t ctx, const int32_t *indptr , const int32_t *indices,
                                          float *data , int64_t nnz, const nnd_prune_opts *opts,
                                          const int32_t *degree ) {
    ENTER(ctx);
    if (ctx->p.flags & NND_FLAG_NO_PREP) { ctx->set_error("nnd_diversify_csr_host: this handle holds no prepared rows (NND_FLAG_NO_PREP)"); return 1; }
    if (need_data(ctx)) return 1;
    const nnd_prune_opts o = prune_defaults(opts);
    if (o.degree_aware && !degree) { ctx->set_error("nnd_diversify_csr_host: the degree-aware method needs degrees"); return 1; }
    nnd_scratch tmp;
    int32_t *dp = tmp.get<int32_t>(ctx, (size_t)(ctx->n + 1)), *di = tmp.get<int32_t>(ctx, (size_t)nnz);
    float *dd = tmp.get<float>(ctx, (size_t)nnz);
    int *flag = tmp.get<int>(ctx, 1);
    int32_t *dg = o.degree_aware ? tmp.get<int32_t>(ctx, (size_t)ctx->n) : nullptr;
    if (!dp || !di || !dd || !flag || (o.degree_aware && !dg)) return 1;
    API_HIP(hipMemsetAsync(flag, 0, sizeof(int), ctx->stream));
    API_HIP(hipMemcpyAsync(dp, indptr, sizeof(int32_t) * (size_t)(ctx->n + 1), hipMemcpyHostToDevice, ctx->stream));
    API_HIP(hipMemcpyAsync(di, indices, sizeof(int32_t) * (size_t)nnz, hipMemcpyHostToDevice, ctx->stream));
    API_HIP(hipMemcpyAsync(dd, data, sizeof(float) * (size_t)nnz, hipMemcpyHostToDevice, ctx->stream));
    if (dg) API_HIP(hipMemcpyAsync(dg, degree, sizeof(int32_t) * (size_t)ctx->n, hipMemcpyHostToDevice, ctx->stream));
    if (nnd_launch_diversify_csr(ctx, dp, di, dd, flag, &o, dg)) return 1;
    int too_long = 0;
    API_HIP(hipMemcpyAsync(data, dd, sizeof(float) * (size_t)nnz, hipMemcpyDeviceToHost, ctx->stream));
// ... 55 lines not shown
```

pynndescent_amd/csrc/rpforest.hip:

```cpp
#include <atomic>
#include <chrono>

#include "common.h"
#include "state.h"

#define RP_EPS 1e-8f

static constexpr int SCAN_ITEMS = 8;
static constexpr int SCAN_BLOCK = 256;
static constexpr int SCAN_TILE = SCAN_ITEMS * SCAN_BLOCK;

__global__ void k_forest_init(int32_t *__restrict__ perm, int32_t *__restrict__ pos_seg, uint8_t *__restrict__ leaf_flag,
                              int32_t *__restrict__ inv, int64_t n, int64_t P, int splittable) {
    int64_t g = (int64_t)blockIdx.x * blockDim.x + threadIdx.x;
    if (g >= P) return;
    int64_t t = g / n;
    int64_t i = g - t * n;
    perm[g] = (int32_t)i;
    inv[g] = splittable ? (int32_t)t : -1;
    pos_seg[g] = splittable ? (int32_t)t : -1;
    leaf_flag[g] = (!splittable && i == 0) ? 1 : 0;
}
__global__ void k_forest_init_segs(int32_t *__restrict__ seg_start, int32_t *__restrict__ seg_len, int n_trees,
                                   int64_t n) {
// ... 321 lines not shown
#pragma unroll
    for (int i = 0; i < SCAN_ITEMS; i++) {
        if (base + i < P) out[base + i] = run;
        run += f[i];
    }
}

__global__ __launch_bounds__(SCAN_BLOCK) void k_scan_i32_reduce(const int32_t *__restrict__ data, int64_t n, int32_t *__restrict__ blk) {
    __shared__ int wsum[SCAN_BLOCK / 64];
    const int64_t base = (int64_t)blockIdx.x * SCAN_TILE + (int64_t)threadIdx.x * SCAN_ITEMS;
    int s = 0;
#pragma unroll
    for (int i = 0; i < SCAN_ITEMS; i++) s += base + i < n ? data[base + i] : 0;
    s = nnd_wave_sum_i32(s);
    if (nnd_lane() == 0) wsum[threadIdx.x >> 6] = s;
    __syncthreads();
    if (threadIdx.x == 0) {
        int t = 0;
        for (int w = 0; w < SCAN_BLOCK / 64; w++) t += wsum[w];
        blk[blockIdx.x] = t;
    }
}
__global__ __launch_bounds__(SCAN_BLOCK) void k_scan_i32_apply(int32_t *__restrict__ data, int64_t n, const int32_t *__restrict__ blk) {
    __shared__ int wsum[SCAN_BLOCK / 64];
    const int lane = nnd_lane(), w = threadIdx.x >> 6;
    const int64_t base = (int64_t)blockIdx.x * SCAN_TILE + (int64_t)threadIdx.x * SCAN_ITEMS;
    int f[SCAN_ITEMS], s = 0;
#pragma unroll
    for (int i = 0; i < SCAN_ITEMS; i++) {
        f[i] = base + i < n ? data[base + i] : 0;
        s += f[i];
    }
    const int incl = nnd_wave_incl_scan_i32(s);
    if (lane == 63) wsum[w] = incl;
    __syncthreads();
    int run = blk[blockIdx.x] + incl - s;
    for (int i = 0; i < w; i++) run += wsum[i];
#pragma unroll
    for (int i = 0; i < SCAN_ITEMS; i++) {
        if (base + i < n) data[base + i] = run;
        run += f[i];
    }
}

__global__ void k_seg_count(const int32_t *__restrict__ seg_start, const int32_t *__restrict__ seg_len, int n_segs,
                            const int32_t *__restrict__ scan, const int32_t *__restrict__ scan_total, int64_t P,
                            int32_t *__restrict__ nleft) {
    int s = blockIdx.x * blockDim.x + threadIdx.x;
    if (s >= n_segs) return;
    int a = seg_start[s], len = seg_len[s];
    int64_t e = (int64_t)a + len;
    int hi = e < P ? scan[e] : scan_total[0];
    int nl = hi - scan[a];
    if (nl == 0 || nl == len) nl = -((len + 1) / 2) - 1;
    nleft[s] = nl;
}

__global__ __launch_bounds__(256) void k_children(const int32_t *__restrict__ seg_start, const int32_t *__restrict__ seg_len,
                                                  const int32_t *__restrict__ nleft, int n_segs, int leaf_size,
                                                  int child_can_split, int fin_max, int child_depth,
                                                  int32_t *__restrict__ next_start, int32_t *__restrict__ next_len,
                                                  int32_t *__restrict__ seg_child, uint8_t *__restrict__ leaf_flag,
                                                  int32_t *__restrict__ fin_start, int32_t *__restrict__ fin_len,
                                                  int32_t *__restrict__ fin_depth, long long *__restrict__ counters,
                                                  int32_t *__restrict__ node_child, int node_base, int next_base,
                                                  int32_t *__restrict__ leaf_depth, int node_top, long long *__restrict__ host_words,
                                                  long long seq) {
    __shared__ int part[256], partf[256];
    if (threadIdx.x == 0) {
        atomicExch((unsigned long long *)&counters[CNT_ACTIVE_POS], 0ull);
        atomicExch((unsigned long long *)&counters[CNT_MAX_STAY], 0ull);
    }
    int chunk = (n_segs + 255) / 256;
    int s0 = threadIdx.x * chunk, s1 = s0 + chunk < n_segs ? s0 + chunk : n_segs;
    int cnt = 0, cntf = 0;
    for (int s = s0; s < s1; s++) {
        int len = seg_len[s], nl = nleft[s];
        if (nl < 0) nl = -nl - 1;
        int lens[2] = {nl, len - nl};
#pragma unroll
        for (int c = 0; c < 2; c++) {
            if (child_can_split && lens[c] > leaf_size) {
                if (lens[c] > fin_max) cnt++; else cntf++;
            }
        }
    }
    part[threadIdx.x] = cnt;
    partf[threadIdx.x] = cntf;
    __syncthreads();
    if (threadIdx.x == 0) {
        int run = 0, runf = (int)counters[CNT_FIN_COUNT];
        for (int i = 0; i < 256; i++) {
            int v = part[i]; part[i] = run; run += v;
            int vf = partf[i]; partf[i] = runf; runf += vf;
        }
        counters[CNT_ACTIVE_SEGS] = run;
        counters[CNT_FIN_COUNT] = runf;
    }
    __syncthreads();
    int run = part[threadIdx.x], runf = partf[threadIdx.x];
    long long active_pos = 0;
    int max_stay = 0;
    for (int s = s0; s < s1; s++) {
        int a = seg_start[s], len = seg_len[s], nl = nleft[s];
        if (nl < 0) nl = -nl - 1;
        int lens[2] = {nl, len - nl};
        int starts[2] = {a, a + nl};
#pragma unroll
        for (int c = 0; c < 2; c++) {
            if (child_can_split && lens[c] > leaf_size) {
                if (lens[c] > fin_max) {
                    next_start[run] = starts[c];
                    next_len[run] = lens[c];
                    if (node_child) node_child[2 * (node_base + s) + c] = next_base + run;
                    seg_child[2 * s + c] = run++;
                    active_pos += lens[c];
                    if (lens[c] > max_stay) max_stay = lens[c];
                } else {
                    fin_start[runf] = starts[c];
                    fin_len[runf] = lens[c];
                    fin_depth[runf] = child_depth;
                    if (node_child) node_child[2 * (node_base + s) + c] = node_top - runf;
                    runf++;
                    seg_child[2 * s + c] = -1;
                }
            } else {
                seg_child[2 * s + c] = -1;
                if (lens[c] > 0) leaf_flag[starts[c]] = 1;
                if (node_child) {
                    node_child[2 * (node_base + s) + c] = -2 - starts[c];
                    if (lens[c] > 0) leaf_depth[starts[c]] = child_depth;
                }
            }
        }
    }
    if (active_pos) atomicAdd((unsigned long long *)&counters[CNT_ACTIVE_POS], (unsigned long long)active_pos);
    if (max_stay) atomicMax((unsigned long long *)&counters[CNT_MAX_STAY], (unsigned long long)max_stay);
    if (host_words) {
        __syncthreads();
        if (threadIdx.x == 0) {
#pragma unroll
            for (int q = 0; q < NND_LEVEL_WORDS; q++)
                host_words[q] = __hip_atomic_load(&counters[CNT_ACTIVE_SEGS + q], __ATOMIC_RELAXED, __HIP_MEMORY_SCOPE_AGENT);
            __threadfence_system();
            __hip_atomic_store(&host_words[NND_LEVEL_WORDS], seq, __ATOMIC_RELEASE, __HIP_MEMORY_SCOPE_SYSTEM);
        }
    }
}

__global__ void k_scatter(const int32_t *__restrict__ perm, const int32_t *__restrict__ pos_seg,
                          const uint8_t *__restrict__ side, const int32_t *__restrict__ scan,
                          const int32_t *__restrict__ seg_start, const int32_t *__restrict__ nleft,
                          const int32_t *__restrict__ seg_child, int64_t P, int64_t n, int32_t *__restrict__ perm_out,
                          int32_t *__restrict__ pos_seg_out, int32_t *__restrict__ inv) {
    int64_t g = (int64_t)blockIdx.x * blockDim.x + threadIdx.x;
    if (g >= P) return;
    int s = pos_seg[g];
    if (s < 0) {
        perm_out[g] = perm[g];
        pos_seg_out[g] = -1;
        return;
    }
    int a = seg_start[s];
    int nl = nleft[s];
    int right;
    int64_t dest;
    if (nl < 0) {
        nl = -nl - 1;
        int off = (int)(g - a);
        right = off & 1;
        dest = right ? (int64_t)a + nl + (off >> 1) : (int64_t)a + (off >> 1);
    } else {
        int L = scan[g] - scan[a];
        right = side[g];
        dest = right ? (int64_t)a + nl + ((int)(g - a) - L) : (int64_t)a + L;
    }
    int32_t p = perm[g];
    perm_out[dest] = p;
    pos_seg_out[dest] = seg_child[2 * s + right];
    if (inv) inv[(g / n) * n + p] = seg_child[2 * s + right];
}

#ifndef NND_FIN_MAX
#define NND_FIN_MAX 2048
#endif
static constexpr int FIN_MAX = NND_FIN_MAX;
#ifndef NND_BIG_MAX
#define NND_BIG_MAX 8192
#endif
static constexpr int BIG_MAX = NND_BIG_MAX;
static constexpr int FIN_STACK = 40;
static constexpr int FIN_SMALL = 512;
static constexpr int FIN_WS = 40;

__device__ __forceinline__ void rp_top2_push(uint64_t &a, uint64_t &b, uint64_t k) {
    if (k < a) {
        b = a;
        a = k;
    } else if (k < b) {
        b = k;
    }
}
__device__ __forceinline__ uint64_t rp_shfl_xor_u64(uint64_t v, int o) {
    const uint32_t lo = (uint32_t)__shfl_xor((int)(uint32_t)v, o, 64), hi = (uint32_t)__shfl_xor((int)(uint32_t)(v >> 32), o, 64);
    return ((uint64_t)hi << 32) | lo;
}

struct rp_record {
    float *hf;
    uint16_t *hh;
    int32_t *child;
    int32_t *leaf_depth;
    int hs, node_top, down_base, lvl_end;
    int *counter, *overflow;
    int min_len, max_len;
};
struct rp_tree_map {
    int tree_bias = 0;
    const int32_t *tree_begin = nullptr;
    int n_tree_begin = 0;
};
__device__ __forceinline__ uint32_t rp_tree_of(const rp_tree_map &tm, int64_t a, int64_t n) {
    if (!tm.tree_begin) return (uint32_t)(a / n) + (uint32_t)tm.tree_bias;
    int t = 0;
    for (int q = 1; q < tm.n_tree_begin; q++) t = a >= tm.tree_begin[q] ? q : t;
    return (uint32_t)t;
}

template <bool BIG, int NTHR, int CAP, bool RECORD = false>
__global__ __launch_bounds__(NTHR, NTHR == 64 ? 5 : 1) void k_finish_subtrees(const float *__restrict__ xp, const uint16_t *__restrict__ xh,
                                                         const float2 *__restrict__ nr, int metric, int dp, int64_t n,
                                                         int32_t *__restrict__ perm,
                                                         const int32_t *__restrict__ seg_start,
                                                         const int32_t *__restrict__ seg_len,
                                                         const int32_t *__restrict__ seg_depth, int depth0, int n_segs,
                                                         int angular, uint32_t seed, int max_depth, int leaf_size,
                                                         uint8_t *__restrict__ leaf_flag, int32_t *__restrict__ tmp_g,
                                                         uint8_t *__restrict__ side_g, int fin_max,
                                                         int32_t *__restrict__ fin_start, int32_t *__restrict__ fin_len,
                                                         int32_t *__restrict__ fin_depth, long long *__restrict__ fin_count,
                                                         rp_tree_map tm, const float *__restrict__ scal, rp_record rec = rp_record{}) {
    extern __shared__ __attribute__((aligned(16))) unsigned char fsm[];
    const int s = blockIdx.x;
    if (s >= n_segs) return;
    const int a = seg_start[s], len = seg_len[s];
    if (len <= 0) return;
    if (RECORD && (len < rec.min_len || len > rec.max_len)) return;
    constexpr int NLDS = BIG ? 0 : CAP;
    constexpr int NW = NTHR / 64;
    int32_t *ids = BIG ? perm + a : (int32_t *)fsm;
    int32_t *tmp = BIG ? tmp_g + a : (int32_t *)fsm + NLDS;
    uint8_t *sd = BIG ? side_g + a : (uint8_t *)((int32_t *)fsm + 2 * NLDS);
    float *h = (float *)(fsm + (size_t)NLDS * 9);
    uint16_t *hb = (uint16_t *)(h + dp + 4);
    int32_t *stk = (int32_t *)(hb + dp);
    int32_t *wsum = stk + FIN_STACK * 4;
    uint64_t *wkeys = (uint64_t *)(wsum + 8);
    const int tid = threadIdx.x, lane = nnd_lane(), w = tid >> 6;
    const uint32_t seedt = seed ^ (rp_tree_of(tm, a, n) * 0x9E3779B9u);
    const float hsc = scal[0], hinv = 1.0f / hsc, inv_s2 = scal[1];
    float cellA = 0.0f, cellB = 0.0f;
    if (!BIG) {
        for (int i = tid; i < len; i += NTHR) {
            const int32_t id = perm[a + i];
            ids[i] = id;
            const float2 nrv = nr[id];
            const float xnm = nnd_metric_unit(metric) ? nrv.x : sqrtf(nrv.x);
            cellA = fmaxf(cellA, nrv.y + RP_ACC * xnm);
            cellB = fmaxf(cellB, xnm + nrv.y);
        }
        cellA = nnd_wave_max_f32_u(cellA);
        cellB = nnd_wave_max_f32_u(cellB);
        if (NW > 1) {
            if (lane == 0) {
                ((float *)wsum)[w] = cellA;
                ((float *)wsum)[8 + w] = cellB;
            }
            __syncthreads();
#pragma unroll
            for (int q = 0; q < NW; q++) {
                cellA = fmaxf(cellA, ((float *)wsum)[q]);
                cellB = fmaxf(cellB, ((float *)wsum)[8 + q]);
            }
            __syncthreads();
        }
    }
    if (tid == 0) {
        stk[0] = 0; stk[1] = len; stk[2] = seg_depth ? seg_depth[s] : depth0;
        stk[3] = RECORD ? rec.node_top - s : 0;
        wsum[7] = 1;
    }
    __syncthreads();
    while (true) {
        const int sp = wsum[7];
        if (sp == 0) break;
        const int ss = stk[(sp - 1) * 4], l = stk[(sp - 1) * 4 + 1], dep = stk[(sp - 1) * 4 + 2], me = stk[(sp - 1) * 4 + 3];
        __syncthreads();
        if (tid == 0) wsum[7] = sp - 1;
        if (!(l > leaf_size && (max_depth - dep) > 0)) {
            if (tid == 0 && l > 0) leaf_flag[a + ss] = 1;
            if (!RECORD && l > 1) {
                for (int i = tid; i < l; i += NTHR) {
                    const int32_t id = ids[ss + i];
                    int r = 0;
                    for (int j = 0; j < l; j++) r += ids[ss + j] < id ? 1 : 0;
                    tmp[r] = id;
                }
                __syncthreads();
                for (int i = tid; i < l; i += NTHR) ids[ss + i] = tmp[i];
            }
            __syncthreads();
            continue;
        }
        if (BIG && l <= fin_max) {
            if (tid == 0) {
                const int idx = (int)atomicAdd((unsigned long long *)fin_count, 1ull);
                fin_start[idx] = a + ss;
                fin_len[idx] = l;
                fin_depth[idx] = dep;
            }
            __syncthreads();
            continue;
        }
        uint64_t k1 = ~0ull, k2 = ~0ull;
        for (int i = tid; i < l; i += NTHR) {
            const uint32_t id = (uint32_t)ids[ss + i];
            rp_top2_push(k1, k2, ((uint64_t)nnd_hash3(seedt, id, (uint32_t)(2 * dep)) << 32) | id);
        }
        {
            const uint64_t g1 = nnd_wave_min_u64_u(k1);
            const uint64_t g2 = nnd_wave_min_u64_u(k1 == g1 ? k2 : k1);
            k1 = g1;
            k2 = g2;
        }
        if (lane == 0) {
            wkeys[2 * w] = k1;
            wkeys[2 * w + 1] = k2;
        }
        __syncthreads();
        k1 = k2 = ~0ull;
#pragma unroll
        for (int q = 0; q < 2 * NW; q++) rp_top2_push(k1, k2, wkeys[q]);
        const int64_t idl = (int64_t)(uint32_t)k1, idr = (int64_t)(uint32_t)k2;
        const float *xl = xp + idl * dp;
        const float *xr = xp + idr * dp;
        float part = 0.0f, psq = 0.0f;
        for (int j = tid; j < dp; j += NTHR) {
            const float lv = xl[j], rv = xr[j];
            const float v = lv - rv;
            h[j] = v;
            part += angular ? v * v : v * (lv + rv);
            psq += v * v;
        }
        part = nnd_wave_sum_f32_u(part);
        psq = nnd_wave_sum_f32_u(psq);
        if (lane == 0) {
            ((float *)wsum)[w] = part;
        }
        __syncthreads();
        float tot = 0.0f;
#pragma unroll
        for (int q = 0; q < NW; q++) tot += ((float *)wsum)[q];
        __syncthreads();
        if (lane == 0) ((float *)wsum)[w] = psq;
        __syncthreads();
        float totsq = 0.0f;
#pragma unroll
        for (int q = 0; q < NW; q++) totsq += ((float *)wsum)[q];
        __syncthreads();
        if (angular) {
            const float nh = sqrtf(tot);
            const float inv = nh < RP_EPS ? 1.0f : 1.0f / nh;
            for (int j = tid; j < dp; j += NTHR) h[j] *= inv;
            if (tid == 0) { h[dp] = 0.0f; h[dp + 1] = nh * inv; }
        } else if (tid == 0) {
            h[dp] = -0.5f * tot;
            h[dp + 1] = sqrtf(totsq);
        }
        __syncthreads();
        float pres = 0.0f;
        for (int j = tid; j < dp; j += NTHR) {
            const float v = h[j];
            const uint16_t b = nnd_f32_to_h16(v, hsc);
            hb[j] = b;
            const float e = v - nnd_h16_to_f32(b, hinv);
            pres += e * e;
        }
        pres = nnd_wave_sum_f32_u(pres);
        if (lane == 0) ((float *)wsum)[w] = pres;
        __syncthreads();
        float rhv = 0.0f;
#pragma unroll
        for (int q = 0; q < NW; q++) rhv += ((float *)wsum)[q];
        rhv = sqrtf(rhv) * 1.000001f;
        if (RECORD) {
            float *rh = rec.hf + (int64_t)me * rec.hs;
            uint16_t *rb = rec.hh + (int64_t)me * dp;
            for (int j = tid; j < dp; j += NTHR) {
                rh[j] = h[j];
                rb[j] = hb[j];
            }
            if (tid == 0) {
                rh[dp] = h[dp];
                rh[dp + 1] = h[dp + 1];
                rh[dp + 2] = rhv;
            }
        }
        const int sub = tid & 3, grp = tid >> 2;
        const int nch = dp >> 3;
        const float off = h[dp], hnorm = h[dp + 1];
        const uint4 *h8 = (const uint4 *)hb;
        constexpr int GQ = NTHR / 4;
        for (int i0 = 0; i0 < l; i0 += 2 * GQ) {
            int64_t pt[2];
            float acc[2], xn[2], rxv[2];
#pragma unroll
            for (int u = 0; u < 2; u++) {
                const int i = i0 + u * GQ + grp;
                pt[u] = ids[ss + (i < l ? i : 0)];
                acc[u] = 0.0f;
            }
            if (BIG) {
#pragma unroll
                for (int u = 0; u < 2; u++) {
                    const float2 nrv = nr[pt[u]];
                    xn[u] = nrv.x;
                    rxv[u] = nrv.y;
                }
            }
            for (int c = sub; c < nch; c += 16) {
                uint4 q[2][4], p[4];
#pragma unroll
                for (int u = 0; u < 2; u++)
#pragma unroll
                    for (int j = 0; j < 4; j++) q[u][j] = ((const uint4 *)(xh + pt[u] * dp))[c + 4 * j < nch ? c + 4 * j : c];
#pragma unroll
                for (int j = 0; j < 4; j++) p[j] = h8[c + 4 * j < nch ? c + 4 * j : c];
#pragma unroll
                for (int u = 0; u < 2; u++)
#pragma unroll
                    for (int j = 0; j < 4; j++)
                        if (c + 4 * j < nch) acc[u] = rp_dot8(q[u][j], p[j], acc[u]);
            }
#pragma unroll
            for (int u = 0; u < 2; u++) {
                const int i = i0 + u * GQ + grp;
                if (i >= l) continue;
                const float m = rp_quad_sum(acc[u]) * inv_s2 + off;
                const float band = BIG ? rp_band(nnd_metric_unit(metric) ? xn[u] : sqrtf(xn[u]), rxv[u], hnorm, rhv) : hnorm * cellA + rhv * cellB + RP_EPS;
                const uint8_t side = rp_side(m, band, xp + pt[u] * dp, h, off, dp, sub, seedt, (uint32_t)pt[u], dep);
                if (sub == 0) sd[i] = side;
            }
        }
        __syncthreads();
        const int per = (l + NTHR - 1) / NTHR;
        const int b0 = tid * per < l ? tid * per : l, b1 = b0 + per < l ? b0 + per : l;
        int cntl, incl, nl, woff;
        for (int attempt = 0;; attempt++) {
            cntl = 0;
            for (int i = b0; i < b1; i++) cntl += sd[i] == 0;
            incl = nnd_wave_incl_scan_i32(cntl);
            if (lane == 63) wsum[w] = incl;
            __syncthreads();
            woff = 0;
            for (int i = 0; i < w; i++) woff += wsum[i];
            nl = 0;
#pragma unroll
            for (int q = 0; q < NW; q++) nl += wsum[q];
            if (nl != 0 && nl != l) break;
            __syncthreads();
            for (int i = b0; i < b1; i++) {
                const uint32_t id = (uint32_t)ids[ss + i];
                sd[i] = attempt == 0 ? (uint8_t)(nnd_hash3(seedt ^ 0x5bd1e995u, id, (uint32_t)(2 * dep + 1)) & 1u)
                                     : (uint8_t)((int64_t)id == idl ? 0 : 1);
            }
            __syncthreads();
        }
        int run = woff + incl - cntl;
        for (int i = b0; i < b1; i++) {
            int dest;
            if (sd[i] == 0) dest = run++;
            else dest = nl + (i - run);
            tmp[dest] = ids[ss + i];
        }
        __syncthreads();
        for (int i = tid; i < l; i += NTHR) ids[ss + i] = tmp[i];
        if (tid == 0) {
            int top = wsum[7];
            const bool left_big = nl >= l - nl;
#pragma unroll
            for (int q = 0; q < 2; q++) {
                const bool left = (q == 0) == left_big;
                const int cs = left ? ss : ss + nl, cl = left ? nl : l - nl;
                int cid = 0;
                if (RECORD) {
                    bool split = cl > leaf_size && (max_depth - (dep + 1)) > 0;
                    if (split) {
                        cid = rec.down_base - atomicAdd(rec.counter, 1);
                        if (cid <= rec.lvl_end) {
                            *rec.overflow = 1;
                            split = false;
                        }
                    }
                    if (!split) {
                        rec.child[2 * me + (left ? 0 : 1)] = -2 - (a + cs);
                        leaf_flag[a + cs] = 1;
                        rec.leaf_depth[a + cs] = dep + 1;
                        continue;
                    }
                    rec.child[2 * me + (left ? 0 : 1)] = cid;
                }
                stk[top * 4] = cs; stk[top * 4 + 1] = cl; stk[top * 4 + 2] = dep + 1; stk[top * 4 + 3] = cid;
                top++;
            }
            wsum[7] = top;
        }
        __syncthreads();
    }
    if (!BIG)
        for (int i = tid; i < len; i += NTHR) perm[a + i] = ids[i];
}

__global__ void k_leaf_starts(const uint8_t *__restrict__ leaf_flag, const int32_t *__restrict__ scan, int64_t P,
                              int32_t *__restrict__ leaf_start) {
    int64_t g = (int64_t)blockIdx.x * blockDim.x + threadIdx.x;
    if (g < P && leaf_flag[g]) leaf_start[scan[g]] = (int32_t)g;
}
__global__ void k_leaf_lens(const int32_t *__restrict__ leaf_start, int64_t n_leaves, int64_t n, int64_t P,
                            int32_t *__restrict__ leaf_len, int32_t *__restrict__ max_len) {
    int64_t i = (int64_t)blockIdx.x * blockDim.x + threadIdx.x;
    int len = 0;
    if (i < n_leaves) {
        int64_t a = leaf_start[i];
        int64_t e = i + 1 < n_leaves ? leaf_start[i + 1] : P;
        int64_t tree_end = (a / n + 1) * n;
        if (e > tree_end) e = tree_end;
        len = (int)(e - a);
        leaf_len[i] = len;
    }
#pragma unroll
    for (int o = 32; o > 0; o >>= 1) {
        const int other = __shfl_xor(len, o, 64);
        len = other > len ? other : len;
    }
    if (nnd_lane() == 0 && len > 0) atomicMax(max_len, len);
}
__global__ void k_tree_leaf_begin(const int32_t *__restrict__ scan, int n_trees, int64_t n, const int32_t *__restrict__ tree_begin,
                                  int64_t P, int32_t n_leaves, long long *__restrict__ out) {
    int t = blockIdx.x * blockDim.x + threadIdx.x;
    if (t >= n_trees) return;
    const int64_t g = tree_begin ? tree_begin[t] : (int64_t)t * n;
    out[t] = g < P ? scan[g] : n_leaves;
}
__global__ void k_fill_leaf_array(const int32_t *__restrict__ perm, const int32_t *__restrict__ leaf_start,
                                  const int32_t *__restrict__ leaf_len, int64_t n_leaves, int max_leaf,
                                  int32_t *__restrict__ out) {
    int64_t t = (int64_t)blockIdx.x * blockDim.x + threadIdx.x;
    if (t >= n_leaves * max_leaf) return;
    int64_t i = t / max_leaf;
    int j = (int)(t - i * max_leaf);
    out[t] = j < leaf_len[i] ? perm[leaf_start[i] + j] : -1;
}

__global__ void k_gather_sample(const float *__restrict__ xp, const uint16_t *__restrict__ xh, const float2 *__restrict__ nr,
                                int dp, int64_t j_lo, int64_t j_hi, int64_t stride, uint32_t seed, float *__restrict__ xs,
                                uint16_t *__restrict__ xsh, float2 *__restrict__ nrs) {
    const int sub = threadIdx.x & 15;
    const int64_t j = j_lo + (int64_t)blockIdx.x * (blockDim.x >> 4) + (threadIdx.x >> 4);
    if (j >= j_hi) return;
    const int64_t i = j * stride + (int64_t)(nnd_hash2(seed ^ 0x7F4A7C15u, (uint32_t)j) % (uint32_t)stride);
    for (int c = sub; c < (dp >> 2); c += 16) ((float4 *)(xs + j * dp))[c] = ((const float4 *)(xp + i * dp))[c];
    for (int c = sub; c < (dp >> 3); c += 16) ((uint4 *)(xsh + j * dp))[c] = ((const uint4 *)(xh + i * dp))[c];
    if (sub == 0) nrs[j] = nr[i];
}

__device__ __forceinline__ uint32_t rp_pack_h16(float a, float b, float scale) {
    return (uint32_t)nnd_f32_to_h16(a, scale) | ((uint32_t)nnd_f32_to_h16(b, scale) << 16);
}
__device__ __forceinline__ float rp_dot4f(float4 a, float4 b, float acc) {
    acc = __builtin_fmaf(a.x, b.x, acc);
    acc = __builtin_fmaf(a.y, b.y, acc);
    acc = __builtin_fmaf(a.z, b.z, acc);
    return __builtin_fmaf(a.w, b.w, acc);
}

struct rp_pack_map {
    int64_t n_low, high_lo;
    int node_base, cell_base;
    const int32_t *cell_gid;
};
__global__ void k_pack_nodes(const uint16_t *__restrict__ node_hh, const float *__restrict__ node_hf, int hs,
                             const int32_t *__restrict__ node_child, const int32_t *__restrict__ leafscan, int dp, int64_t n_packed,
                             rp_pack_map mp, unsigned char *__restrict__ pack, float *__restrict__ hf_out) {
    const int sub = threadIdx.x & 15;
    const int64_t vp = (int64_t)blockIdx.x * (blockDim.x >> 4) + (threadIdx.x >> 4);
    if (vp >= n_packed) return;
    const int64_t v = vp < mp.n_low ? vp : mp.high_lo + (vp - mp.n_low);
    const int rec = 2 * dp + 16;
    uint4 *dst = (uint4 *)(pack + vp * rec);
    const uint4 *src = (const uint4 *)(node_hh + v * dp);
    for (int c = sub; c < (dp >> 3); c += 16) dst[c] = src[c];
    const float *h = node_hf + v * hs;
    if (hf_out)
        for (int c = sub; c < (hs >> 2); c += 16) ((float4 *)(hf_out + vp * hs))[c] = ((const float4 *)h)[c];
    if (sub == 0) {
        int ch[2];
#pragma unroll
        for (int q = 0; q < 2; q++) {
            const int c = node_child[2 * v + q];
            if (c >= 0) {
                ch[q] = (int)((int64_t)c < mp.n_low ? c : c - (mp.high_lo - mp.n_low)) + mp.node_base;
            } else {
                const int lc = leafscan[-2 - c];
                ch[q] = -2 - (mp.cell_gid ? mp.cell_gid[lc] : mp.cell_base + lc);
            }
        }
        dst[dp >> 3] = make_uint4(__float_as_uint(h[dp]), (rp_bf16_up(h[dp + 1]) << 16) | rp_bf16_up(h[dp + 2]), (uint32_t)ch[0], (uint32_t)ch[1]);
    }
}

template <int NC, int TB>
__global__ __launch_bounds__(512) void k_route(const float *__restrict__ xp, const float2 *__restrict__ nr, int metric, int dp,
                                               int64_t n, int n_trees, const unsigned char *__restrict__ node_pack,
                                               const float *__restrict__ node_hf, int hs, uint32_t seed,
                                               int32_t *__restrict__ cell_count, int32_t *__restrict__ cell_of,
                                               int32_t *__restrict__ rank_of, int n_top, int l_top, const float *__restrict__ scal) {
    extern __shared__ __attribute__((aligned(16))) unsigned char top_tab[];
    const int rec = 2 * dp + 16;
    const float hsc = scal[0], inv_s2 = scal[1];
    {
        const uint4 *src = (const uint4 *)node_pack;
        uint4 *dst = (uint4 *)top_tab;
        const int total = n_top * (rec >> 4);
        for (int q = threadIdx.x; q < total; q += blockDim.x) dst[q] = src[q];
    }
    __syncthreads();
    const int sub = threadIdx.x & 3;
    const int qpb = blockDim.x >> 2;
    for (int64_t i0 = (int64_t)blockIdx.x * qpb; i0 < n; i0 += (int64_t)gridDim.x * qpb) {
        const int64_t i = i0 + (threadIdx.x >> 2);
        if (i >= n) continue;
        float4 xa[NC], xb[NC];
        uint4 xq[NC];
        {
            const float4 *row = (const float4 *)(xp + i * dp);
#pragma unroll
            for (int q = 0; q < NC; q++) {
                const int c = sub + 4 * q;
                xa[q] = row[2 * c];
                xb[q] = row[2 * c + 1];
            }
#pragma unroll
            for (int q = 0; q < NC; q++)
                xq[q] = make_uint4(rp_pack_h16(xa[q].x, xa[q].y, hsc), rp_pack_h16(xa[q].z, xa[q].w, hsc), rp_pack_h16(xb[q].x, xb[q].y, hsc),
                                   rp_pack_h16(xb[q].z, xb[q].w, hsc));
        }
        const float2 nrv = nr[i];
        const float xn = nrv.x, rx = nrv.y;
        const float xnorm = nnd_metric_unit(metric) ? xn : sqrtf(xn);
        for (int t0 = 0; t0 < n_trees; t0 += TB) {
            int node[TB];
            int rk[TB];
#pragma unroll
            for (int u = 0; u < TB; u++) {
                node[u] = t0 + u < n_trees ? t0 + u : -1;
                rk[u] = 0;
            }
            for (int depth = 0;; depth++) {
                bool any = false;
#pragma unroll
                for (int u = 0; u < TB; u++) any |= node[u] >= 0;
                if (!__ballot(any)) break;
                uint4 p[TB][NC], meta[TB];
                bool high = false;
#pragma unroll
                for (int u = 0; u < TB; u++) high |= node[u] >= n_top;
                if (depth < l_top && !__ballot(high)) {
#pragma unroll
                    for (int u = 0; u < TB; u++) {
                        const uint4 *r8 = (const uint4 *)(top_tab + (size_t)(node[u] >= 0 ? node[u] : 0) * rec);
#pragma unroll
                        for (int q = 0; q < NC; q++) p[u][q] = r8[sub + 4 * q];
                        meta[u] = r8[dp >> 3];
                    }
                } else {
#pragma unroll
                    for (int u = 0; u < TB; u++) {
                        const uint4 *r8 = (const uint4 *)(node_pack + (int64_t)(node[u] >= 0 ? node[u] : 0) * rec);
#pragma unroll
                        for (int q = 0; q < NC; q++) p[u][q] = r8[sub + 4 * q];
                        meta[u] = r8[dp >> 3];
                    }
                }
                float acc[TB];
#pragma unroll
                for (int u = 0; u < TB; u++) {
                    acc[u] = 0.0f;
#pragma unroll
                    for (int q = 0; q < NC; q++) acc[u] = rp_dot8(xq[q], p[u][q], acc[u]);
                }
#pragma unroll
                for (int u = 0; u < TB; u++) {
                    if (node[u] < 0) continue;
                    const float off = __uint_as_float(meta[u].x), hnorm = __uint_as_float(meta[u].y & 0xFFFF0000u),
                                rh = __uint_as_float(meta[u].y << 16);
                    float m = rp_quad_sum(acc[u]) * inv_s2 + off;
                    const float band = rp_band(xnorm, rx, hnorm, rh);
                    if (RP_IN_BAND(m, band)) {
                        const float4 *h4 = (const float4 *)(node_hf + (int64_t)node[u] * hs);
                        float e = 0.0f;
#pragma unroll
                        for (int q = 0; q < NC; q++) {
                            const int c = sub + 4 * q;
                            e = rp_dot4f(xa[q], h4[2 * c], e);
                            e = rp_dot4f(xb[q], h4[2 * c + 1], e);
                        }
                        m = rp_quad_sum(e) + off;
                    }
                    const int64_t slot = (int64_t)(t0 + u) * n + i;
                    int side;
                    if (fabsf(m) < RP_EPS) side = (int)(nnd_hash3(seed ^ 0x5bd1e995u, (uint32_t)slot, (uint32_t)depth) & 1u);
                    else side = m > 0.0f ? 0 : 1;
                    const int nxt = (int)(side ? meta[u].w : meta[u].z);
                    if (nxt <= -2) {
                        if (sub == 0) {
                            const int cell = -2 - nxt;
                            cell_of[slot] = cell;
                            rk[u] = atomicAdd(&cell_count[cell], 1);
                        }
                        node[u] = -1;
                    } else {
                        node[u] = nxt;
                    }
                }
            }
            if (sub == 0) {
#pragma unroll
                for (int u = 0; u < TB; u++)
                    if (t0 + u < n_trees) rank_of[(int64_t)(t0 + u) * n + i] = rk[u];
            }
        }
    }
}

#define RP_GLOBAL_TAG 0x40000000

__global__ __launch_bounds__(256) void k_top_heap(const unsigned char *__restrict__ pack, int rec, int dp, const int32_t *__restrict__ roots,
                                                  int L1, unsigned char *__restrict__ top_rec, int32_t *__restrict__ top_node,
                                                  int32_t *__restrict__ bucket_root) {
    __shared__ int32_t hn[256];
    const int t = blockIdx.x, nslots = 1 << L1, r16 = rec >> 4;
    if (threadIdx.x == 0) {
        hn[0] = -1;
        hn[1] = roots[t];
    }
    __syncthreads();
    for (int l = 0; l < L1; l++) {
        for (int sl = (1 << l) + threadIdx.x; sl < (2 << l); sl += blockDim.x) {
            const int nd = hn[sl];
            int c0 = -1, c1 = -1;
            if (nd >= 0) {
                const uint4 meta = *(const uint4 *)(pack + (int64_t)nd * rec + 2 * dp);
                c0 = (int)meta.z;
                c1 = (int)meta.w;
// ... 362 lines not shown
                }
                int side;
                if (fabsf(m) < RP_EPS) side = (int)(nnd_hash3(seed ^ 0x5bd1e995u, (uint32_t)slot, (uint32_t)depth) & 1u);
                else side = m > 0.0f ? 0 : 1;
                const int nxt = (int)(side ? meta.w : meta.z);
                if (nxt <= -2) {
                    if (sub == 0) {
                        const int cell = -2 - nxt;
                        if (glob) {
                            const int64_t o = (int64_t)t * nrows + (pi - row_lo);
                            cell_of[o] = cell;
                            rank_of[o] = atomicAdd(&cell_count[cell], 1);
                        } else {
                            rk = (cell << 16) | atomicAdd(&lcnt[cell], 1);
                        }
                    }
                    cur = -1;
                } else {
                    cur = nxt;
                }
            }
            if (sub == 0 && on) rowbuf[idx] = (uint32_t)rk;
        }
        __syncthreads();
        for (int q = threadIdx.x; q < R + 8; q += blockDim.x) {
            const int c = lcnt[q];
            if (c) {
                lbase[q] = atomicAdd(&cell_count[lcell[q]], c);
                lcnt[q] = 0;
            }
        }
        __syncthreads();
        for (int idx = threadIdx.x; idx < cnt_rows; idx += blockDim.x) {
            const uint32_t v = rowbuf[idx];
            if (v == 0xFFFFFFFFu) continue;
            const int lc = (int)(v >> 16);
            const int64_t o = (int64_t)t * nrows + (bucket_rows[base + idx] - row_lo);
            cell_of[o] = lcell[lc];
            rank_of[o] = lbase[lc] + (int)(v & 0xFFFFu);
        }
        __syncthreads();
    }
}

__global__ void k_cell_depths(const uint8_t *__restrict__ leaf_flag, const int32_t *__restrict__ leafscan,
                              const int32_t *__restrict__ leaf_depth, int64_t ps, int32_t *__restrict__ cell_depth) {
    const int64_t g = (int64_t)blockIdx.x * blockDim.x + threadIdx.x;
    if (g < ps && leaf_flag[g]) cell_depth[leafscan[g]] = leaf_depth[g];
}

__global__ void k_cell_lists(const int32_t *__restrict__ cell_count, const int32_t *__restrict__ cell_start,
                             const int32_t *__restrict__ cell_depth, int n_cells, int fin_small, int fin_max,
                             int32_t *__restrict__ small_list, int32_t *__restrict__ fin_start, int32_t *__restrict__ fin_len,
                             int32_t *__restrict__ fin_depth, int32_t *__restrict__ big_start, int32_t *__restrict__ big_len,
                             int32_t *__restrict__ big_depth, int64_t list_stride,
                             long long *__restrict__ counts ) {
    const int c = blockIdx.x * blockDim.x + threadIdx.x;
    const int len = c < n_cells ? cell_count[c] : 0;
    const int cls = len <= 0 ? -1 : (len <= fin_small ? 2 : (len <= fin_max ? 0 : 1));
#pragma unroll
    for (int k = 0; k < 3; k++) {
        const unsigned long long m = __ballot(cls == k);
        if (!m) continue;
        long long base = 0;
        if (nnd_lane() == __builtin_ctzll(m)) base = (long long)atomicAdd((unsigned long long *)&counts[k], (unsigned long long)__popcll(m));
        base = ((long long)__shfl((int)(base >> 32), __builtin_ctzll(m), 64) << 32) | (unsigned)__shfl((int)base, __builtin_ctzll(m), 64);
        if (cls == k) {
            const int64_t idx = base + nnd_prefix_popc(m);
            int32_t *st = k == 2 ? small_list : (k == 0 ? fin_start : big_start);
            int32_t *ln = k == 2 ? small_list + list_stride : (k == 0 ? fin_len : big_len);
            int32_t *dp_ = k == 2 ? small_list + 2 * list_stride : (k == 0 ? fin_depth : big_depth);
            st[idx] = cell_start[c];
            ln[idx] = len;
            dp_[idx] = cell_depth[c];
        }
    }
}

__global__ void k_place(const int32_t *__restrict__ cell_of, const int32_t *__restrict__ rank_of,
                        const int32_t *__restrict__ cell_start, int64_t nrows, int64_t row_lo, int32_t *__restrict__ perm) {
    const int64_t r = (int64_t)blockIdx.x * blockDim.x + threadIdx.x;
    if (r >= nrows) return;
    const int64_t slot = (int64_t)blockIdx.y * nrows + r;
    perm[cell_start[cell_of[slot]] + rank_of[slot]] = (int32_t)(row_lo + r);
}

enum forest_rc { FOREST_OK = 0, FOREST_ERROR = 1, FOREST_FALLBACK = 2 };
static forest_rc forest_fallback(const char *reason) {
    if (nnd_knob("NND_FOREST_DEBUG")) fprintf(stderr, "forest: fallback: %s\n", reason);
    return FOREST_FALLBACK;
}
#define FOREST_HIP_CHECK(expr) NND_HIP_CHECK_AS(expr, #expr, FOREST_ERROR)

static forest_rc run_scan(nnd_ctx *ctx, int mode, const int32_t *pos_seg, uint8_t *bytes, int32_t *total_dev, int64_t P, int64_t n,
                          const int32_t *perm = nullptr) {
    int nb = (int)((P + SCAN_TILE - 1) / SCAN_TILE);
    hipLaunchKernelGGL(k_scan_reduce, dim3(nb), dim3(SCAN_BLOCK), 0, ctx->stream, mode, pos_seg, bytes, P, ctx->scan_blk, perm,
                       ctx->side_pt, n);
    hipLaunchKernelGGL(k_scan_apply<true>, dim3(nb), dim3(SCAN_BLOCK), 0, ctx->stream, mode == 2 ? 0 : mode, pos_seg, bytes, P,
                       ctx->scan_blk, ctx->scan_out, total_dev);
    FOREST_HIP_CHECK(hipGetLastError());
    return FOREST_OK;
}

static forest_rc scan_i32_inplace(nnd_ctx *ctx, int32_t *data, int64_t n, int32_t *total_dev) {
    if (n <= SCAN_TILE) {
        hipLaunchKernelGGL(k_scan_blocks, dim3(1), dim3(256), 0, ctx->stream, data, (int)n, total_dev);
    } else {
        const int nb = (int)((n + SCAN_TILE - 1) / SCAN_TILE);
        hipLaunchKernelGGL(k_scan_i32_reduce, dim3(nb), dim3(SCAN_BLOCK), 0, ctx->stream, data, n, ctx->scan_blk);
        hipLaunchKernelGGL(k_scan_blocks, dim3(1), dim3(256), 0, ctx->stream, ctx->scan_blk, nb, total_dev);
        hipLaunchKernelGGL(k_scan_i32_apply, dim3(nb), dim3(SCAN_BLOCK), 0, ctx->stream, data, n, ctx->scan_blk);
    }
    FOREST_HIP_CHECK(hipGetLastError());
    return FOREST_OK;
}

static forest_rc read_scan_total(nnd_ctx *ctx, int32_t *out) {
    FOREST_HIP_CHECK(hipMemcpyAsync(&ctx->h_pin->scan_total, nnd_scan_total(ctx), sizeof(int32_t), hipMemcpyDeviceToHost, ctx->stream));
    FOREST_HIP_CHECK(nnd_sync_spin(ctx));
    *out = ctx->h_pin->scan_total;
    return FOREST_OK;
}

static size_t fin_smem_bytes(int dp, int cap ) {
    const size_t tail = sizeof(float) * (dp + 4) + sizeof(uint16_t) * dp + sizeof(int32_t) * (FIN_STACK * 4 + FIN_WS);
    return (size_t)cap * 9 + tail;
}

struct forest_rows {
    const float *xp;
    const uint16_t *xh;
    const float2 *nr;
    int64_t n;
    int leaf_size;
};
static forest_rows whole_set_rows(const nnd_ctx *ctx) { return {ctx->xp, ctx->xh, ctx->nr2, ctx->n, ctx->p.leaf_size}; }

struct forest_view {
    forest_rows rows;
    int64_t P;
    int fin_max;
    bool record;
    int T = 0;
    rp_tree_map tm;
    int cur = 0, depth = 0;
    int64_t S = 0;
    long long active_pos = 0;
    int64_t node_base = 0;
    bool inv_live = true;
    nnd_level_flag *flag_dev = nullptr;
    std::vector<int64_t> level_base;
    int64_t n_low = 0, high_lo = 0;
};

template <bool BIG, int NTHR, int CAP, bool RECORD = false>
static forest_rc launch_finisher(nnd_ctx *ctx, const forest_rows &r, int32_t *perm, int32_t *other, const nnd_work_list &wl, int depth0,
                                 long long count, const rp_tree_map &tm, const rp_record &rec = rp_record{}) {
    const nnd_work_list fin = nnd_fin_list(ctx);
    hipLaunchKernelGGL((k_finish_subtrees<BIG, NTHR, CAP, RECORD>), dim3((unsigned)count), dim3(NTHR), fin_smem_bytes(ctx->dp, CAP), ctx->stream,
                       r.xp, r.xh, r.nr, ctx->p.metric, ctx->dp, r.n, perm, wl.start, wl.len, wl.depth, depth0, (int)count,
                       nnd_metric_unit(ctx->p.metric), ctx->tree_seed, ctx->p.max_depth, r.leaf_size, ctx->leaf_flag,
                       BIG ? other : (int32_t *)nullptr, BIG ? ctx->side : (uint8_t *)nullptr, FIN_MAX, fin.start, fin.len, fin.depth,
                       ctx->counters + CNT_FIN_COUNT, tm, ctx->mean + ctx->dp, rec);
    FOREST_HIP_CHECK(hipGetLastError());
    return FOREST_OK;
}

static forest_rc read_fin_count(nnd_ctx *ctx, long long *out) {
    FOREST_HIP_CHECK(hipMemcpyAsync(&ctx->h_pin->fin_count, ctx->counters + CNT_FIN_COUNT, sizeof(long long), hipMemcpyDeviceToHost, ctx->stream));
    FOREST_HIP_CHECK(nnd_sync_spin(ctx));
    *out = ctx->h_pin->fin_count;
    return FOREST_OK;
}

static forest_rc launch_finishers(nnd_ctx *ctx, int32_t *perm, int32_t *other, const nnd_work_list &big, int depth0, long long n_big,
                                  long long n_small, const rp_tree_map &tm) {
    const forest_rows rows = whole_set_rows(ctx);
    forest_rc rc;
    if (n_small > 0 && (rc = launch_finisher<false, 64, FIN_SMALL>(ctx, rows, perm, other, nnd_small_list(ctx), 0, n_small, tm))) return rc;
    if (n_big > 0 && (rc = launch_finisher<true, 256, 0>(ctx, rows, perm, other, big, depth0, n_big, tm))) return rc;
    long long nfin = 0;
    if ((rc = read_fin_count(ctx, &nfin))) return rc;
    if (nfin > ctx->max_segs) {
        ctx->set_error("rp-forest: %lld finisher segments exceed the allocation of %lld", nfin, (long long)ctx->max_segs);
        return FOREST_ERROR;
    }
    if (nfin > 0) return launch_finisher<false, 256, FIN_MAX>(ctx, rows, perm, other, nnd_fin_list(ctx), 0, nfin, tm);
    return FOREST_OK;
}

static forest_rc levels_start(nnd_ctx *ctx, forest_view &v) {
    const int64_t n = v.rows.n;
    if (v.T <= 0) v.T = ctx->p.n_trees;
    const int T = v.T;
    const int splittable = (n > v.rows.leaf_size && ctx->p.max_depth > 0) ? 1 : 0;
    hipLaunchKernelGGL(k_forest_init, dim3((unsigned)((v.P + 255) / 256)), dim3(256), 0, ctx->stream, ctx->perm[0], ctx->pos_seg[0],
                       ctx->leaf_flag, ctx->inv, n, v.P, splittable);
    hipLaunchKernelGGL(k_forest_init_segs, dim3((T + 63) / 64), dim3(64), 0, ctx->stream, ctx->seg_start[0],
                       ctx->seg_len[0], T, n);
    v.cur = v.depth = 0;
    v.S = splittable ? T : 0;
    v.active_pos = v.P;
    v.node_base = 0;
    v.inv_live = true;
    v.flag_dev = (ctx->h_pin_dev && !ctx->wait_hook && !nnd_knob("NND_NO_LEVEL_FLAG")) ? &ctx->h_pin_dev->flag : nullptr;
    long long *fin_count = ctx->counters + CNT_FIN_COUNT;
    FOREST_HIP_CHECK(hipMemsetAsync(fin_count, 0, sizeof(long long), ctx->stream));
    if (!v.record && v.S > 0 && n <= v.fin_max) {
        const nnd_work_list fin = nnd_fin_list(ctx);
        std::vector<int32_t> h_s(T), h_l(T), h_d(T, 0);
        for (int t = 0; t < T; t++) { h_s[t] = (int32_t)(t * n); h_l[t] = (int32_t)n; }
        FOREST_HIP_CHECK(hipMemcpyAsync(fin.start, h_s.data(), sizeof(int32_t) * T, hipMemcpyHostToDevice, ctx->stream));
        FOREST_HIP_CHECK(hipMemcpyAsync(fin.len, h_l.data(), sizeof(int32_t) * T, hipMemcpyHostToDevice, ctx->stream));
        FOREST_HIP_CHECK(hipMemcpyAsync(fin.depth, h_d.data(), sizeof(int32_t) * T, hipMemcpyHostToDevice, ctx->stream));
        long long cntf = T;
        FOREST_HIP_CHECK(hipMemcpyAsync(fin_count, &cntf, sizeof(long long), hipMemcpyHostToDevice, ctx->stream));
        FOREST_HIP_CHECK(hipStreamSynchronize(ctx->stream));
        v.S = 0;
    }
    return FOREST_OK;
}

static forest_rc level_launch(nnd_ctx *ctx, forest_view &v) {
    const forest_rows &r = v.rows;
    const int64_t n = r.n, P = v.P, S = v.S, node_base = v.node_base;
    const int dp = ctx->dp, hs = dp + 4, cur = v.cur, depth = v.depth;
    const uint32_t pos_bias = (uint32_t)((int64_t)v.tm.tree_bias * n);
    const unsigned gridP = (unsigned)((P + 255) / 256);
    int32_t *scan_total = nnd_scan_total(ctx);
    if (S > ctx->max_segs) {
        ctx->set_error("rp-forest: %lld segments exceed the allocation of %lld", (long long)S, (long long)ctx->max_segs);
        return FOREST_ERROR;
    }
    if (v.record && node_base + S > ctx->node_cap) return forest_fallback("a recorded level outgrows the node tables");
    if (v.record) v.level_base.push_back(node_base);
    float *hyper = v.record ? ctx->node_hf + node_base * hs : ctx->hyper;
    uint16_t *hyper_h = v.record ? ctx->node_hh + node_base * dp : ctx->hyper_h;
    hipLaunchKernelGGL(k_hyperplane, dim3((unsigned)((S + 3) / 4)), dim3(256), 0, ctx->stream, r.xp, dp,
                       ctx->perm[cur], ctx->seg_start[cur], ctx->seg_len[cur], (int)S, nnd_metric_unit(ctx->p.metric), ctx->tree_seed, depth,
                       hyper, hs, hyper_h, pos_bias, ctx->mean + ctx->dp);
    const bool fused = v.inv_live && (S * (int64_t)dp * 2 <= (int64_t)6 << 20) && (v.active_pos * 2 >= 3 * n);
    if (fused) {
        hipLaunchKernelGGL(k_margin_fused, dim3((unsigned)((n + 63) / 64)), dim3(256), 0, ctx->stream, r.xp, r.xh, r.nr,
                           ctx->p.metric, dp, n, v.T, ctx->inv, hyper, hs, hyper_h, ctx->tree_seed, depth, ctx->side_pt, pos_bias, ctx->mean + ctx->dp);
    } else {
        v.inv_live = false;
        hipLaunchKernelGGL(k_margin, dim3((unsigned)((P + 63) / 64)), dim3(256), 0, ctx->stream, r.xp, r.xh, r.nr,
                           ctx->p.metric, dp, ctx->perm[cur], ctx->pos_seg[cur], P, hyper, hs, hyper_h, ctx->tree_seed, depth,
                           ctx->side, pos_bias, ctx->mean + ctx->dp);
    }
    if (run_scan(ctx, fused ? 2 : 0, ctx->pos_seg[cur], ctx->side, scan_total, P, n, ctx->perm[cur])) return FOREST_ERROR;
    hipLaunchKernelGGL(k_seg_count, dim3((unsigned)((S + 255) / 256)), dim3(256), 0, ctx->stream, ctx->seg_start[cur],
                       ctx->seg_len[cur], (int)S, ctx->scan_out, scan_total, P, ctx->seg_nleft);
    int child_can_split = (ctx->p.max_depth - (depth + 1)) > 0 ? 1 : 0;
    if (v.record && ctx->early_stop > 0 && v.active_pos * ctx->early_stop < P) child_can_split = 0;
    const nnd_work_list fin = nnd_fin_list(ctx);
    hipLaunchKernelGGL(k_children, dim3(1), dim3(256), 0, ctx->stream, ctx->seg_start[cur], ctx->seg_len[cur],
                       ctx->seg_nleft, (int)S, r.leaf_size, child_can_split, v.fin_max, depth + 1, ctx->seg_start[1 - cur],
                       ctx->seg_len[1 - cur], ctx->seg_child, ctx->leaf_flag, fin.start, fin.len, fin.depth, ctx->counters,
                       v.record ? ctx->node_child : (int32_t *)nullptr, (int)node_base, (int)(node_base + S), ctx->s_leaf_depth,
                       (int)ctx->node_cap - 1, (long long *)v.flag_dev, v.flag_dev ? ++ctx->flag_seq : 0);
    hipLaunchKernelGGL(k_scatter, dim3(gridP), dim3(256), 0, ctx->stream, ctx->perm[cur], ctx->pos_seg[cur], ctx->side,
                       ctx->scan_out, ctx->seg_start[cur], ctx->seg_nleft, ctx->seg_child, P, n, ctx->perm[1 - cur],
                       ctx->pos_seg[1 - cur], v.inv_live ? ctx->inv : (int32_t *)nullptr);
    FOREST_HIP_CHECK(hipGetLastError());
    return FOREST_OK;
}

static forest_rc level_handover(nnd_ctx *ctx, const forest_view &v, nnd_level_words *next) {
    if (!v.flag_dev) {
        FOREST_HIP_CHECK(hipMemcpyAsync(&ctx->h_pin->level, ctx->counters + CNT_ACTIVE_SEGS, sizeof(nnd_level_words), hipMemcpyDeviceToHost,
                                        ctx->stream));
        FOREST_HIP_CHECK(nnd_sync_spin(ctx));
        *next = ctx->h_pin->level;
        return FOREST_OK;
    }
    volatile long long *seqw = &ctx->h_pin->flag.seq;
    const auto t_spin = std::chrono::steady_clock::now();
    unsigned spins = 0;
    while (*seqw != ctx->flag_seq) {
        if ((++spins & 0xFFFFu) == 0 && std::chrono::steady_clock::now() - t_spin > std::chrono::seconds(30)) {
            ctx->set_error("rp-forest: the device did not hand over the segment count of level %d within 30 s", v.depth);
            return FOREST_ERROR;
        }
    }
    std::atomic_thread_fence(std::memory_order_acquire);
    *next = ctx->h_pin->flag.w;
    return FOREST_OK;
}

static forest_rc record_subtrees(nnd_ctx *ctx, forest_view &v) {
    const int64_t node_base = v.node_base;
    v.level_base.push_back(node_base);
    forest_rc rc;
    long long nfin = 0;
    if ((rc = read_fin_count(ctx, &nfin))) return rc;
    if (nfin > ctx->max_segs || node_base + nfin + 1 >= ctx->node_cap) return forest_fallback("the subtrees to record outgrow the node tables");
    v.n_low = node_base;
    v.high_lo = ctx->node_cap;
    if (nfin == 0) return FOREST_OK;
    int *flags = (int *)(ctx->counters + CNT_REC_FLAGS);
    FOREST_HIP_CHECK(hipMemsetAsync(flags, 0, 2 * sizeof(int), ctx->stream));
    rp_record rec{ctx->node_hf, ctx->node_hh, ctx->node_child, ctx->s_leaf_depth, ctx->dp + 4, (int)ctx->node_cap - 1,
                  (int)(ctx->node_cap - 1 - nfin), (int)node_base, flags, flags + 1, 0, FIN_MAX};
    rp_record rs = rec, rl = rec;
    rs.min_len = 0; rs.max_len = FIN_SMALL;
    rl.min_len = FIN_SMALL + 1; rl.max_len = FIN_MAX;
    const nnd_work_list fin = nnd_fin_list(ctx);
    if ((rc = launch_finisher<false, 64, FIN_SMALL, true>(ctx, v.rows, ctx->perm[v.cur], nullptr, fin, 0, nfin, v.tm, rs))) return rc;
    if (v.fin_max > FIN_SMALL && (rc = launch_finisher<false, 256, FIN_MAX, true>(ctx, v.rows, ctx->perm[v.cur], nullptr, fin, 0, nfin, v.tm, rl)))
        return rc;
    FOREST_HIP_CHECK(hipMemcpyAsync(ctx->h_pin->rec_flags, flags, 2 * sizeof(int), hipMemcpyDeviceToHost, ctx->stream));
    FOREST_HIP_CHECK(nnd_sync_spin(ctx));
    if (ctx->h_pin->rec_flags[1]) return forest_fallback("the recording finisher ran out of node slots");
    v.high_lo = ctx->node_cap - nfin - ctx->h_pin->rec_flags[0];
    return FOREST_OK;
}

static forest_rc forest_levels(nnd_ctx *ctx, forest_view &v) {
    forest_rc rc = levels_start(ctx, v);
    if (rc) return rc;
    while (v.S > 0) {
        nnd_level_words next;
        if ((rc = level_launch(ctx, v)) || (rc = level_handover(ctx, v, &next))) return rc;
        v.node_base += v.S;
        v.S = next.segs;
        v.active_pos = next.active_pos;
        v.cur = 1 - v.cur;
        v.depth++;
        if (!v.record && v.S > 0 && (v.active_pos * 2 < 3 * v.rows.n) && next.max_stay <= BIG_MAX) {
            const nnd_work_list stayers{ctx->seg_start[v.cur], ctx->seg_len[v.cur], nullptr};
            return launch_finishers(ctx, ctx->perm[v.cur], ctx->perm[1 - v.cur], stayers, v.depth, v.S, 0, v.tm);
        }
    }
    if (v.record) return record_subtrees(ctx, v);
    return launch_finishers(ctx, ctx->perm[v.cur], ctx->perm[1 - v.cur], nnd_work_list{}, 0, 0, 0, v.tm);
}

static forest_rc device_cus(nnd_ctx *ctx, int *out) {
    static int n_cu_dev[64] = {0};
    int &n_cu = n_cu_dev[ctx->p.device & 63];
    if (n_cu == 0) {
        hipDeviceProp_t prop;
        FOREST_HIP_CHECK(hipGetDeviceProperties(&prop, ctx->p.device));
        n_cu = prop.multiProcessorCount;
    }
    *out = n_cu;
    return FOREST_OK;
}

struct rp_route_io {
    const unsigned char *pack;
    const float *hf;
    const int32_t *roots;
    int T;
    int64_t row_lo, nrows;
    int64_t n_cells;
    int32_t *cell_count, *cell_of, *rank_of;
    int32_t *code, *bucket_rows, *bucket_ab;
};

template <int NC, int TB>
static forest_rc launch_route(nnd_ctx *ctx, const rp_route_io &io, int n_top, int l_top) {
    auto kern = k_route<NC, TB>;
    const size_t smem = (size_t)n_top * (2 * ctx->dp + 16);
    static bool attr_dev[64] = {false};
    if (!attr_dev[ctx->p.device & 63]) {
        FOREST_HIP_CHECK(hipFuncSetAttribute((const void *)kern, hipFuncAttributeMaxDynamicSharedMemorySize, 72 * 1024));
        attr_dev[ctx->p.device & 63] = true;
    }
    int n_cu = 0;
    if (device_cus(ctx, &n_cu)) return FOREST_ERROR;
    int64_t blocks = (ctx->n + 127) / 128;
    if (blocks > 2 * (int64_t)n_cu) blocks = 2 * (int64_t)n_cu;
    hipLaunchKernelGGL(kern, dim3((unsigned)blocks), dim3(512), smem, ctx->stream, ctx->xp, ctx->nr2, ctx->p.metric, ctx->dp, ctx->n,
                       io.T, io.pack, io.hf, ctx->dp + 4, ctx->tree_seed, io.cell_count, io.cell_of, io.rank_of, n_top, l_top, ctx->mean + ctx->dp);
    FOREST_HIP_CHECK(hipGetLastError());
    return FOREST_OK;
}

static forest_rc route_plain(nnd_ctx *ctx, const rp_route_io &io, const forest_view &v) {
    const int dp = ctx->dp;
    int l_top = 0;
    while (l_top + 1 < (int)v.level_base.size() && v.level_base[l_top + 1] * (2 * dp + 16) <= 72 * 1024) l_top++;
    const int n_top = (int)v.level_base[l_top];
    switch (dp / 32) {
        case 1: return launch_route<1, 4>(ctx, io, n_top, l_top);
        case 2: return launch_route<2, 4>(ctx, io, n_top, l_top);
        case 3: return launch_route<3, 2>(ctx, io, n_top, l_top);
        case 4: return launch_route<4, 2>(ctx, io, n_top, l_top);
        case 5: return launch_route<5, 1>(ctx, io, n_top, l_top);
        case 6: return launch_route<6, 1>(ctx, io, n_top, l_top);
        case 7: return launch_route<7, 1>(ctx, io, n_top, l_top);
        case 8: return launch_route<8, 1>(ctx, io, n_top, l_top);
        default: break;
    }
    return FOREST_FALLBACK;
}

#ifndef NND_ROUTE_L1
#define NND_ROUTE_L1 6
#endif
#ifndef NND_ROUTE_CHUNK
#define NND_ROUTE_CHUNK 2048
#endif
#ifndef NND_ROUTE_RMAX
#define NND_ROUTE_RMAX 384
#endif

struct rp_route_geom {
    int L1, ns, nb, R, chunk, tg;
    int64_t max_items;
    size_t o_top_rec, o_top_node, o_bucket_root, o_bcount, o_bcursor, o_bstart, o_nitems, o_btcnt, o_btnode, o_btchild, o_btrec, o_btcell, o_items, total;
};
static rp_route_geom route_geometry(int dp, int T, int64_t nrows, int64_t n_cells) {
    rp_route_geom g;
    const int rec = 2 * dp + 16;
    g.L1 = NND_ROUTE_L1;
    if (g.L1 < 7 && n_cells / ((int64_t)T << g.L1) > NND_ROUTE_RMAX / 2) g.L1 = 7;
    g.ns = 1 << g.L1;
    g.nb = T * g.ns;
    int64_t r = 6 * n_cells / g.nb + 16;
    const int64_t r_lds = (int64_t)150 * 1024 / rec;
    if (r > NND_ROUTE_RMAX) r = NND_ROUTE_RMAX;
    if (r > r_lds) r = r_lds;
    g.R = (int)(r < 64 ? 64 : r);
    g.chunk = NND_ROUTE_CHUNK;
    g.tg = (int)((size_t)140 * 1024 / ((size_t)g.ns * (rec + 8)));
    if (g.tg < 1) g.tg = 1;
    if (g.tg > T) g.tg = T;
    g.max_items = (int64_t)g.nb + (int64_t)T * nrows / g.chunk + 1;
    size_t at = 0;
    auto take = [&](size_t bytes) { const size_t o = at; at += (bytes + 255) & ~(size_t)255; return o; };
    g.o_top_rec = take((size_t)g.nb * rec);
    g.o_top_node = take(sizeof(int32_t) * g.nb);
    g.o_bucket_root = take(sizeof(int32_t) * g.nb);
    g.o_bcount = take(sizeof(int32_t) * g.nb);
    g.o_bcursor = take(sizeof(int32_t) * g.nb);
    g.o_bstart = take(sizeof(int32_t) * (g.nb + 1));
    g.o_nitems = take(sizeof(int32_t) * 4);
    g.o_btcnt = take(sizeof(int32_t) * g.nb);
    g.o_btnode = take(sizeof(int32_t) * (size_t)g.nb * g.R);
    g.o_btchild = take(sizeof(int32_t) * (size_t)g.nb * g.R * 2);
    g.o_btrec = take((size_t)g.nb * g.R * rec);
    g.o_btcell = take(sizeof(int32_t) * (size_t)g.nb * (g.R + 8));
    g.o_items = take(sizeof(int2) * (size_t)g.max_items);
    g.total = at;
    return g;
}

template <int NC>
static forest_rc launch_route_coherent(nnd_ctx *ctx, const rp_route_io &io, const rp_route_geom &g) {
    const int dp = ctx->dp, rec = 2 * dp + 16, hs = dp + 4;
    unsigned char *ws = ctx->route_ws;
    unsigned char *top_rec = ws + g.o_top_rec;
    int32_t *top_node = (int32_t *)(ws + g.o_top_node), *bucket_root = (int32_t *)(ws + g.o_bucket_root);
    int32_t *bcount = (int32_t *)(ws + g.o_bcount), *bcursor = (int32_t *)(ws + g.o_bcursor), *bstart = (int32_t *)(ws + g.o_bstart);
    int32_t *n_items = (int32_t *)(ws + g.o_nitems), *bt_cnt = (int32_t *)(ws + g.o_btcnt), *bt_node = (int32_t *)(ws + g.o_btnode);
    int32_t *bt_child = (int32_t *)(ws + g.o_btchild);
    unsigned char *bt_rec = ws + g.o_btrec;
    int32_t *bt_cell = (int32_t *)(ws + g.o_btcell);
    int2 *items = (int2 *)(ws + g.o_items);
    auto ktop = k_route_top<NC>;
    auto kbkt = k_route_bucket<NC>;
    static bool attr_dev[64] = {false};
    if (!attr_dev[ctx->p.device & 63]) {
        FOREST_HIP_CHECK(hipFuncSetAttribute((const void *)ktop, hipFuncAttributeMaxDynamicSharedMemorySize, 160 * 1024));
        FOREST_HIP_CHECK(hipFuncSetAttribute((const void *)kbkt, hipFuncAttributeMaxDynamicSharedMemorySize, 160 * 1024));
        attr_dev[ctx->p.device & 63] = true;
    }
    int n_cu = 0;
    if (device_cus(ctx, &n_cu)) return FOREST_ERROR;
    FOREST_HIP_CHECK(hipMemsetAsync(bcount, 0, g.o_bstart - g.o_bcount, ctx->stream));
    hipLaunchKernelGGL(k_top_heap, dim3((unsigned)io.T), dim3(256), 0, ctx->stream, io.pack, rec, dp, io.roots, g.L1, top_rec, top_node,
                       bucket_root);
    hipLaunchKernelGGL(k_bucket_tables, dim3((unsigned)g.nb), dim3(64), 0, ctx->stream, io.pack, rec, dp, bucket_root, g.R, bt_cnt, bt_node,
                       bt_child, bt_rec, bt_cell);
    for (int tg0 = 0; tg0 < io.T; tg0 += g.tg) {
        const int tgn = io.T - tg0 < g.tg ? io.T - tg0 : g.tg;
        const size_t smem = (size_t)tgn * g.ns * (rec + 8);
        int64_t blocks = (io.nrows + 511) / 512;
        if (blocks > n_cu) blocks = n_cu;
        hipLaunchKernelGGL(ktop, dim3((unsigned)blocks), dim3(1024), smem, ctx->stream, ctx->xp, ctx->xh, ctx->nr2, ctx->p.metric, dp, ctx->n, io.row_lo,
                           io.nrows, tg0, tgn, g.L1, top_rec, top_node, io.hf, hs, ctx->tree_seed, io.cell_count, io.cell_of, io.rank_of,
                           io.code, bcount, ctx->mean + ctx->dp);
    }
    hipLaunchKernelGGL(k_bucket_prefix, dim3(1), dim3(256), 0, ctx->stream, bcount, g.nb, g.chunk, bstart, items, n_items, (int)g.max_items);
    hipLaunchKernelGGL(k_bucket_scatter, dim3((unsigned)((io.nrows + 4095) / 4096), (unsigned)io.T), dim3(256), 0, ctx->stream, io.code,
                       io.nrows, io.row_lo, g.L1, bstart, bcursor, io.bucket_rows, ctx->nr2, ctx->p.metric, (uint32_t *)io.bucket_ab);
    const size_t smem2 = (size_t)g.R * rec + sizeof(int32_t) * 3 * (size_t)(g.R + 8) + sizeof(uint32_t) * (size_t)g.chunk;
    int per_cu = 0;
    FOREST_HIP_CHECK(hipOccupancyMaxActiveBlocksPerMultiprocessor(&per_cu, (const void *)kbkt, 1024, smem2));
    if (per_cu < 1) per_cu = 1;
    int64_t blocks2 = (int64_t)n_cu * per_cu;
    if (blocks2 > g.max_items) blocks2 = g.max_items;
    hipLaunchKernelGGL(kbkt, dim3((unsigned)blocks2), dim3(1024), smem2, ctx->stream, ctx->xp, ctx->xh, ctx->nr2, ctx->p.metric, dp, ctx->n,
                       io.row_lo, io.nrows, g.L1, g.chunk, io.pack, io.hf, hs, items, n_items, bstart, io.bucket_rows, (const uint32_t *)io.bucket_ab, g.R, bt_cnt, bt_node,
                       bt_rec, bt_cell, ctx->tree_seed, io.cell_count, io.cell_of, io.rank_of, ctx->mean + ctx->dp);
    FOREST_HIP_CHECK(hipGetLastError());
    return FOREST_OK;
}

static forest_rc route_coherent(nnd_ctx *ctx, const rp_route_io &io) {
    const int dp = ctx->dp;
    if (dp % 32 != 0 || dp > 256 || io.T < 1 || io.T > NND_ROUTE_TREES_MAX) return FOREST_FALLBACK;
    const rp_route_geom g = route_geometry(dp, io.T, io.nrows, io.n_cells);
    if (g.total > ctx->route_ws_cap) {
        FOREST_HIP_CHECK(hipStreamSynchronize(ctx->stream));
        if (ctx->route_ws) { FOREST_HIP_CHECK(hipFree(ctx->route_ws)); ctx->route_ws = nullptr; }
        ctx->route_ws_cap = 0;
        FOREST_HIP_CHECK(hipMalloc((void **)&ctx->route_ws, g.total + g.total / 4));
        ctx->route_ws_cap = g.total + g.total / 4;
    }
    switch (dp / 32) {
        case 1: return launch_route_coherent<1>(ctx, io, g);
        case 2: return launch_route_coherent<2>(ctx, io, g);
        case 3: return launch_route_coherent<3>(ctx, io, g);
        case 4: return launch_route_coherent<4>(ctx, io, g);
        case 5: return launch_route_coherent<5>(ctx, io, g);
        case 6: return launch_route_coherent<6>(ctx, io, g);
        case 7: return launch_route_coherent<7>(ctx, io, g);
        case 8: return launch_route_coherent<8>(ctx, io, g);
        default: break;
    }
    return FOREST_FALLBACK;
}

__global__ void k_iota_i32(int32_t *__restrict__ out, int n, int base) {
    const int i = blockIdx.x * blockDim.x + threadIdx.x;
    if (i < n) out[i] = base + i;
}

static forest_rc forest_tops(nnd_ctx *ctx, forest_view &v, int32_t *n_cells_out) {
    forest_rc rc = forest_levels(ctx, v);
    if (rc) return rc;
    int32_t n_cells = 0;
    if ((rc = run_scan(ctx, 1, nullptr, ctx->leaf_flag, nnd_scan_total(ctx), v.P, v.rows.n)) || (rc = read_scan_total(ctx, &n_cells))) return rc;
    if (n_cells > ctx->cell_cap) return forest_fallback("the recorded trees have more cells than the cell tables hold");
    hipLaunchKernelGGL(k_cell_depths, dim3((unsigned)((v.P + 255) / 256)), dim3(256), 0, ctx->stream, ctx->leaf_flag, ctx->scan_out,
                       ctx->s_leaf_depth, v.P, ctx->cell_depth);
    FOREST_HIP_CHECK(hipGetLastError());
    *n_cells_out = n_cells;
    return FOREST_OK;
}

static forest_rc forest_place_finish(nnd_ctx *ctx, int32_t n_cells, int T, int64_t row_lo, int64_t nrows, const int32_t *cell_of,
                                     const int32_t *rank_of, int64_t P_used, rp_tree_map tm) {
    FOREST_HIP_CHECK(hipMemcpyAsync(ctx->cell_start, ctx->cell_count, sizeof(int32_t) * (size_t)n_cells, hipMemcpyDeviceToDevice, ctx->stream));
    if (scan_i32_inplace(ctx, ctx->cell_start, n_cells, nnd_scan_total(ctx))) return FOREST_ERROR;
    FOREST_HIP_CHECK(hipMemsetAsync(ctx->leaf_flag, 0, (size_t)P_used, ctx->stream));
    long long *counts = ctx->counters + CNT_FIN_COUNT;
    FOREST_HIP_CHECK(hipMemsetAsync(counts, 0, 3 * sizeof(long long), ctx->stream));
    const nnd_work_list fin = nnd_fin_list(ctx), big = nnd_big_list(ctx), small = nnd_small_list(ctx);
    hipLaunchKernelGGL(k_cell_lists, dim3((unsigned)((n_cells + 255) / 256)), dim3(256), 0, ctx->stream, ctx->cell_count, ctx->cell_start,
                       ctx->cell_depth, (int)n_cells, FIN_SMALL, FIN_MAX, small.start, fin.start, fin.len, fin.depth, big.start,
                       big.len, big.depth, small.len - small.start, counts);
    if (cell_of)
        hipLaunchKernelGGL(k_place, dim3((unsigned)((nrows + 255) / 256), (unsigned)T), dim3(256), 0, ctx->stream, cell_of, rank_of,
                           ctx->cell_start, nrows, row_lo, ctx->perm[0]);
    FOREST_HIP_CHECK(hipGetLastError());
    FOREST_HIP_CHECK(hipMemcpyAsync(&ctx->h_pin->n_big, ctx->counters + CNT_BIG_COUNT, 2 * sizeof(long long), hipMemcpyDeviceToHost, ctx->stream));
    FOREST_HIP_CHECK(nnd_sync_spin(ctx));
    const long long n_big = ctx->h_pin->n_big, n_small = ctx->h_pin->n_small;
    if (n_big > ctx->max_segs) return forest_fallback("more over-long cells than the big work list holds");
    if (launch_finishers(ctx, ctx->perm[0], ctx->perm[1], big, 0, n_big, n_small, tm)) return FOREST_ERROR;
    ctx->cur = 0;
    return FOREST_OK;
}

static forest_rc forest_by_routing(nnd_ctx *ctx, int *levels_out) {
    const int64_t n = ctx->n, P = ctx->P, M = ctx->s_m, Ps = (int64_t)ctx->p.n_trees * M;
    const int T = ctx->p.n_trees, dp = ctx->dp;
    hipLaunchKernelGGL(k_gather_sample, dim3((unsigned)((M + 15) / 16)), dim3(256), 0, ctx->stream, ctx->xp, ctx->xh, ctx->nr2,
                       dp, (int64_t)0, M, ctx->s_stride, ctx->tree_seed, ctx->xs, ctx->xsh, ctx->nr2s);
    static const int rec_fin = [] { const char *e = nnd_knob("NND_REC_FIN"); const int r = e ? atoi(e) : FIN_SMALL; return r <= FIN_SMALL ? FIN_SMALL : FIN_MAX; }();
    forest_view v{{ctx->xs, ctx->xsh, ctx->nr2s, M, ctx->cell_leaf}, Ps, rec_fin, true};
    int32_t n_cells = 0;
    forest_rc rc = forest_tops(ctx, v, &n_cells);
    if (rc) return rc;
    if (n_cells + P / (ctx->p.leaf_size + 1) > ctx->max_segs) return forest_fallback("cells and leaves could outgrow the segment tables");
    FOREST_HIP_CHECK(hipMemsetAsync(ctx->cell_count, 0, sizeof(int32_t) * (size_t)n_cells, ctx->stream));
    const int64_t n_packed = v.n_low + (ctx->node_cap - v.high_lo);
    rp_pack_map mp{v.n_low, v.high_lo, 0, 0, nullptr};
    hipLaunchKernelGGL(k_pack_nodes, dim3((unsigned)((n_packed + 15) / 16)), dim3(256), 0, ctx->stream, ctx->node_hh, ctx->node_hf,
                       dp + 4, ctx->node_child, ctx->scan_out, dp, n_packed, mp, ctx->node_pack, ctx->node_hfc);
    int32_t *roots = ctx->route_roots;
    hipLaunchKernelGGL(k_iota_i32, dim3((unsigned)((T + 255) / 256)), dim3(256), 0, ctx->stream, roots, T, 0);
    rp_route_io io{ctx->node_pack, ctx->node_hfc, roots, T, 0, n, n_cells, ctx->cell_count, ctx->pos_seg[0], ctx->pos_seg[1], ctx->inv, ctx->scan_out, ctx->perm[1]};
    rc = FOREST_FALLBACK;
    if (!(ctx->p.flags & NND_FLAG_TEST_ROUTE_PLAIN)) rc = route_coherent(ctx, io);
    if (rc == FOREST_FALLBACK) rc = route_plain(ctx, io, v);
    if (rc) return rc;
    rc = forest_place_finish(ctx, n_cells, T, 0, n, ctx->pos_seg[0], ctx->pos_seg[1], P, rp_tree_map{});
    if (rc) return rc;
    *levels_out = v.depth;
    ctx->stats.n_cells = n_cells;
    return FOREST_OK;
}

static forest_rc forest_leaf_tables(nnd_ctx *ctx, int64_t P, int T, const int32_t *tree_begin_dev) {
    const int64_t n = ctx->n;
    const int leaf_size = ctx->p.leaf_size;
    unsigned gridP = (unsigned)((P + 255) / 256);
    int32_t nl = 0;
    if (run_scan(ctx, 1, nullptr, ctx->leaf_flag, nnd_scan_total(ctx), P, n) || read_scan_total(ctx, &nl)) return FOREST_ERROR;
    ctx->n_leaves = nl;
    if (nl + 1 > ctx->leaf_cap) {
        if (ctx->leaf_start) { FOREST_HIP_CHECK(hipFree(ctx->leaf_start)); ctx->leaf_start = nullptr; }
        if (ctx->leaf_len) { FOREST_HIP_CHECK(hipFree(ctx->leaf_len)); ctx->leaf_len = nullptr; }
        ctx->leaf_cap = (int64_t)(nl + 1) + (nl + 1) / 4;
        FOREST_HIP_CHECK(hipMalloc((void **)&ctx->leaf_start, sizeof(int32_t) * (size_t)ctx->leaf_cap));
        FOREST_HIP_CHECK(hipMalloc((void **)&ctx->leaf_len, sizeof(int32_t) * (size_t)ctx->leaf_cap));
    }
    hipLaunchKernelGGL(k_leaf_starts, dim3(gridP), dim3(256), 0, ctx->stream, ctx->leaf_flag, ctx->scan_out, P,
                       ctx->leaf_start);
    int32_t *max_len_dev = (int32_t *)(ctx->counters + CNT_MAX_LEAF);
    FOREST_HIP_CHECK(hipMemsetAsync(max_len_dev, 0, sizeof(long long), ctx->stream));
    hipLaunchKernelGGL(k_leaf_lens, dim3((unsigned)((nl + 255) / 256)), dim3(256), 0, ctx->stream, ctx->leaf_start,
                       (int64_t)nl, tree_begin_dev ? P : n, P, ctx->leaf_len, max_len_dev);
    hipLaunchKernelGGL(k_tree_leaf_begin, dim3((T + 63) / 64), dim3(64), 0, ctx->stream, ctx->scan_out, T, n, tree_begin_dev, P, nl, ctx->tree_begin_dev);
    FOREST_HIP_CHECK(hipGetLastError());
    FOREST_HIP_CHECK(hipMemcpyAsync(ctx->h_tree_begin, ctx->tree_begin_dev, sizeof(long long) * T, hipMemcpyDeviceToHost, ctx->stream));
    FOREST_HIP_CHECK(hipMemcpyAsync(ctx->h_pin->max_leaf, max_len_dev, sizeof(long long), hipMemcpyDeviceToHost, ctx->stream));
    FOREST_HIP_CHECK(nnd_sync_spin(ctx));
    ctx->h_leaf_valid = false;
    int32_t mx = leaf_size;
    const int32_t longest = ctx->h_pin->max_leaf[0];
    if (longest > mx) mx = longest;
    ctx->tree_leaf_begin.assign(T + 1, nl);
    for (int t = 0; t < T; t++) ctx->tree_leaf_begin[t] = ctx->h_tree_begin[t];
    ctx->max_leaf = mx;
    ctx->stats.n_leaves = nl;
    ctx->forest_built = true;
    ctx->forest_gen++;
    return FOREST_OK;
}

int nnd_launch_forest(nnd_ctx *ctx) {
    const int64_t n = ctx->n, P = ctx->P;
    const int T = ctx->p.n_trees, leaf_size = ctx->p.leaf_size;
    ctx->forest_built = false;
    ctx->n_leaves = 0;
    ctx->max_leaf = leaf_size;
    ctx->tree_leaf_begin.clear();
    ctx->stats.n_cells = 0;
    if (T <= 0) return 0;
    if (P >= (int64_t)0x7FFFFFF0) {
        ctx->set_error("n_trees * n = %lld exceeds the int32 position space", (long long)P);
        return 1;
    }
    int levels = 0;
    forest_rc rc = FOREST_FALLBACK;
    if (ctx->s_m > 0) rc = forest_by_routing(ctx, &levels);
    if (nnd_knob("NND_FOREST_DEBUG"))
        fprintf(stderr, "forest: n=%lld T=%d s_m=%lld routing rc=%d levels=%d node_cap=%lld cell_cap=%lld max_segs=%lld\n", (long long)n, T,
                (long long)ctx->s_m, rc, levels, (long long)ctx->node_cap, (long long)ctx->cell_cap, (long long)ctx->max_segs);
    if (rc == FOREST_ERROR) return 1;
    if (rc == FOREST_FALLBACK) {
        forest_view v{whole_set_rows(ctx), P, FIN_MAX, false};
        if (forest_levels(ctx, v)) return 1;
        ctx->cur = v.cur;
        levels = v.depth;
    }
    ctx->stats.tree_levels = levels;
    return forest_leaf_tables(ctx, P, T, nullptr);
}


int nnd_forest_sample_gather(nnd_ctx *ctx, int64_t j_lo, int64_t j_hi) {
    if (j_hi <= j_lo) return 0;
    hipLaunchKernelGGL(k_gather_sample, dim3((unsigned)((j_hi - j_lo + 15) / 16)), dim3(256), 0, ctx->stream, ctx->xp, ctx->xh, ctx->nr2,
                       ctx->dp, j_lo, j_hi, ctx->s_stride, ctx->tree_seed, ctx->xs, ctx->xsh, ctx->nr2s);
    NND_HIP_CHECK(hipGetLastError());
    return 0;
}

__global__ void k_tree_cell_begin(const int32_t *__restrict__ leafscan, int T, int64_t M, int32_t *__restrict__ out) {
    const int t = blockIdx.x * blockDim.x + threadIdx.x;
    if (t < T) out[t] = leafscan[(int64_t)t * M];
}

int nnd_forest_tops(nnd_ctx *ctx, int T_loc, int tree_bias, nnd_tops_info *out) {
    out->n_packed = 0;
    out->n_cells = 0;
    out->levels = 0;
    out->n_low = out->high_lo = 0;
    if (T_loc <= 0) return 0;
    const int64_t M = ctx->s_m;
    forest_view v{{ctx->xs, ctx->xsh, ctx->nr2s, M, ctx->cell_leaf}, (int64_t)T_loc * M, FIN_SMALL, true};
    v.T = T_loc;
    v.tm.tree_bias = tree_bias;
    int32_t n_cells = 0;
    const forest_rc rc = forest_tops(ctx, v, &n_cells);
    if (rc == FOREST_FALLBACK) { ctx->set_error("rp-forest (sharded): the recorded tree tops outgrew their tables"); return FOREST_FALLBACK; }
    if (rc) return rc;
    int32_t *tcb = nnd_route_tree_cells(ctx);
    hipLaunchKernelGGL(k_tree_cell_begin, dim3((T_loc + 63) / 64), dim3(64), 0, ctx->stream, ctx->scan_out, T_loc, M, tcb);
    NND_HIP_CHECK(hipMemcpyAsync(ctx->h_tree_begin, tcb, sizeof(int32_t) * T_loc, hipMemcpyDeviceToHost, ctx->stream));
    NND_HIP_CHECK(nnd_sync_spin(ctx));
    const int32_t *hb = (const int32_t *)ctx->h_tree_begin;
    for (int t = 0; t < T_loc; t++) out->tree_cells[t] = (t + 1 < T_loc ? hb[t + 1] : n_cells) - hb[t];
    out->n_cells = n_cells;
    out->n_low = v.n_low;
    out->high_lo = v.high_lo;
    out->n_packed = v.n_low + (ctx->node_cap - v.high_lo);
    out->levels = v.depth;
    return 0;
}

int nnd_forest_tops_pack(nnd_ctx *ctx, const nnd_tops_info *ti, int64_t node_base, const int32_t *cell_gid_dev, unsigned char *pack_dst,
                         float *hf_dst) {
    if (ti->n_packed <= 0) return 0;
    rp_pack_map mp{ti->n_low, ti->high_lo, (int)node_base, 0, cell_gid_dev};
    hipLaunchKernelGGL(k_pack_nodes, dim3((unsigned)((ti->n_packed + 15) / 16)), dim3(256), 0, ctx->stream, ctx->node_hh, ctx->node_hf,
                       ctx->dp + 4, ctx->node_child, ctx->scan_out, ctx->dp, ti->n_packed, mp, pack_dst, hf_dst);
    NND_HIP_CHECK(hipGetLastError());
    return 0;
}

int nnd_forest_route_rows(nnd_ctx *ctx, const unsigned char *pack_all, const float *hf_all, const int32_t *roots_dev, int T_all,
                          int64_t row_lo, int64_t nrows, int64_t n_cells_all, int32_t *cell_count_all) {
    if (nrows <= 0 || T_all <= 0) return 0;
    if ((int64_t)T_all * nrows > ctx->P) { ctx->set_error("rp-forest (sharded): %d trees x %lld rows exceed the position space of %lld", T_all, (long long)nrows, (long long)ctx->P); return 1; }
    rp_route_io io{pack_all, hf_all, roots_dev, T_all, row_lo, nrows, n_cells_all, cell_count_all, ctx->pos_seg[0], ctx->pos_seg[1], ctx->inv, ctx->scan_out, ctx->perm[1]};
    const forest_rc rc = route_coherent(ctx, io);
    if (rc == FOREST_FALLBACK) { ctx->set_error("rp-forest (sharded): the routing passes do not support this row width"); return 1; }
    return rc;
}

__global__ void k_route_records(const int32_t *__restrict__ cell_of, const int32_t *__restrict__ rank_of, const int32_t *__restrict__ cell_scan,
                                int64_t nrows, int64_t row_lo, int32_t *__restrict__ rec_cell, int32_t *__restrict__ rec_row) {
    const int64_t r = (int64_t)blockIdx.x * blockDim.x + threadIdx.x;
    if (r >= nrows) return;
    const int64_t slot = (int64_t)blockIdx.y * nrows + r;
    const int c = cell_of[slot];
    const int at = cell_scan[c] + rank_of[slot];
    rec_cell[at] = c;
    rec_row[at] = (int32_t)(row_lo + r);
}
__global__ void k_dest_offsets(const int32_t *__restrict__ cell_scan, const int32_t *__restrict__ dest_cell, int G, int32_t n_cells_all,
                               const int32_t *__restrict__ total, long long *__restrict__ out) {
    const int q = threadIdx.x;
    if (q > G) return;
    const int c = dest_cell[q];
    const long long at = c < n_cells_all ? cell_scan[c] : total[0];
    out[q] = at;
}
int nnd_forest_route_records(nnd_ctx *ctx, int T_all, int64_t row_lo, int64_t nrows, int32_t n_cells_all, int32_t *cell_count_all ,
                             int32_t *count_copy ,
                             const int32_t *dest_cell_dev, int G, int32_t *rec_cell, int32_t *rec_row, long long *dest_off_dev) {
    int32_t *scan_total = nnd_scan_total(ctx);
    NND_HIP_CHECK(hipMemcpyAsync(count_copy, cell_count_all, sizeof(int32_t) * (size_t)n_cells_all, hipMemcpyDeviceToDevice, ctx->stream));
    if (scan_i32_inplace(ctx, cell_count_all, n_cells_all, scan_total)) return 1;
    if (nrows > 0)
        hipLaunchKernelGGL(k_route_records, dim3((unsigned)((nrows + 255) / 256), (unsigned)T_all), dim3(256), 0, ctx->stream, ctx->pos_seg[0],
                           ctx->pos_seg[1], cell_count_all, nrows, row_lo, rec_cell, rec_row);
    hipLaunchKernelGGL(k_dest_offsets, dim3(1), dim3(128), 0, ctx->stream, cell_count_all, dest_cell_dev, G, n_cells_all, scan_total, dest_off_dev);
    NND_HIP_CHECK(hipGetLastError());
    return 0;
}

__global__ void k_owner_sum_counts(const int32_t *__restrict__ cnt_src , int G, int32_t n_cells, int32_t *__restrict__ cell_count) {
    const int c = blockIdx.x * blockDim.x + threadIdx.x;
    if (c >= n_cells) return;
    int s = 0;
    for (int q = 0; q < G; q++) s += cnt_src[(size_t)q * n_cells + c];
    cell_count[c] = s;
}
__global__ void k_owner_place(const int32_t *__restrict__ rec_cell, const int32_t *__restrict__ rec_row, int64_t n_rec, int32_t cell_base,
                              const int32_t *__restrict__ cell_start, int32_t *__restrict__ cursor, int32_t *__restrict__ perm) {
    const int64_t i = (int64_t)blockIdx.x * blockDim.x + threadIdx.x;
    if (i >= n_rec) return;
    const int c = rec_cell[i] - cell_base;
    perm[cell_start[c] + atomicAdd(&cursor[c], 1)] = rec_row[i];
}
__global__ void k_gather_i32(const int32_t *__restrict__ src, const int32_t *__restrict__ map, int n, int32_t *__restrict__ dst) {
    const int i = blockIdx.x * blockDim.x + threadIdx.x;
    if (i < n) dst[i] = src[map[i]];
}
__global__ void k_tree_pos_begin(const int32_t *__restrict__ cell_start, const int32_t *__restrict__ tree_first_cell, int T, int32_t n_cells,
                                 int32_t P_used, int32_t *__restrict__ out) {
    const int t = blockIdx.x * blockDim.x + threadIdx.x;
    if (t > T) return;
    const int c = t < T ? tree_first_cell[t] : n_cells;
    out[t] = c < n_cells ? cell_start[c] : P_used;
}

int nnd_forest_finish_owned(nnd_ctx *ctx, const int32_t *rec_cell, const int32_t *rec_row, int64_t n_rec, int32_t cell_base, int32_t n_cells_own,
                            const int32_t *cnt_src, int G, const int32_t *cell_depth_all, const int32_t *depth_map_dev,
                            const int32_t *tree_first_cell_dev, int T_all) {
    ctx->forest_built = false;
    ctx->n_leaves = 0;
    ctx->max_leaf = ctx->p.leaf_size;
    ctx->tree_leaf_begin.assign((size_t)T_all + 1, 0);
    if (n_rec > ctx->P || n_cells_own > ctx->cell_cap || n_cells_own + n_rec / (ctx->p.leaf_size + 1) > ctx->max_segs) {
        ctx->set_error("rp-forest (sharded): %lld point-trees / %d cells exceed this rank's forest tables (%lld positions)", (long long)n_rec, n_cells_own,
                       (long long)ctx->P);
        return FOREST_FALLBACK;
    }
    if (n_cells_own <= 0 || n_rec <= 0) {
        ctx->forest_built = true;
        return 0;
    }
    hipLaunchKernelGGL(k_owner_sum_counts, dim3((unsigned)((n_cells_own + 255) / 256)), dim3(256), 0, ctx->stream, cnt_src, G, n_cells_own, ctx->cell_count);
    hipLaunchKernelGGL(k_gather_i32, dim3((unsigned)((n_cells_own + 255) / 256)), dim3(256), 0, ctx->stream, cell_depth_all, depth_map_dev, n_cells_own,
                       ctx->cell_depth);
    NND_HIP_CHECK(hipMemcpyAsync(ctx->cell_start, ctx->cell_count, sizeof(int32_t) * (size_t)n_cells_own, hipMemcpyDeviceToDevice, ctx->stream));
    if (scan_i32_inplace(ctx, ctx->cell_start, n_cells_own, nnd_scan_total(ctx))) return 1;
    int32_t *cursor = nnd_small_list(ctx).start;
    NND_HIP_CHECK(hipMemsetAsync(cursor, 0, sizeof(int32_t) * (size_t)n_cells_own, ctx->stream));
    hipLaunchKernelGGL(k_owner_place, dim3((unsigned)((n_rec + 255) / 256)), dim3(256), 0, ctx->stream, rec_cell, rec_row, n_rec, cell_base, ctx->cell_start,
                       cursor, ctx->perm[0]);
    int32_t *tpb = nnd_route_tree_pos(ctx);
    hipLaunchKernelGGL(k_tree_pos_begin, dim3((T_all + 64) / 64), dim3(64), 0, ctx->stream, ctx->cell_start, tree_first_cell_dev, T_all, n_cells_own,
                       (int32_t)n_rec, tpb);
    NND_HIP_CHECK(hipGetLastError());
    rp_tree_map tm;
    tm.tree_begin = tpb;
    tm.n_tree_begin = T_all;
    const forest_rc rc = forest_place_finish(ctx, n_cells_own, T_all, 0, 0, nullptr, nullptr, n_rec, tm);
    if (rc == FOREST_FALLBACK) { ctx->set_error("rp-forest (sharded): too many over-long cells"); return FOREST_FALLBACK; }
    if (rc) return rc;
    ctx->stats.n_cells = n_cells_own;
    return forest_leaf_tables(ctx, n_rec, T_all, tpb);
}

void nnd_forest_stable_partition(nnd_ctx *ctx, int64_t n, const int32_t *ord, const int32_t *pos, uint8_t *side, const int32_t *seg_start,
                                 const int32_t *seg_len, int n_segs, int32_t *nleft, const int32_t *seg_child, int32_t *ord_out,
                                 int32_t *pos_out) {
    int32_t *scan_total = nnd_scan_total(ctx);
    const int nb = (int)((n + SCAN_TILE - 1) / SCAN_TILE);
    hipLaunchKernelGGL(k_scan_reduce, dim3(nb), dim3(SCAN_BLOCK), 0, ctx->stream, 0, pos, side, n, ctx->scan_blk, (const int32_t *)nullptr,
                       (const uint8_t *)nullptr, n);
    hipLaunchKernelGGL(k_scan_blocks, dim3(1), dim3(256), 0, ctx->stream, ctx->scan_blk, nb, scan_total);
    hipLaunchKernelGGL(k_scan_apply<false>, dim3(nb), dim3(SCAN_BLOCK), 0, ctx->stream, 0, pos, side, n, ctx->scan_blk, ctx->scan_out,
                       (int32_t *)nullptr);
    hipLaunchKernelGGL(k_seg_count, dim3((unsigned)((n_segs + 255) / 256)), dim3(256), 0, ctx->stream, seg_start, seg_len, n_segs,
                       ctx->scan_out, scan_total, n, nleft);
    hipLaunchKernelGGL(k_scatter, dim3((unsigned)((n + 255) / 256)), dim3(256), 0, ctx->stream, ord, pos, side, ctx->scan_out, seg_start,
                       nleft, seg_child, n, n, ord_out, pos_out, (int32_t *)nullptr);
}

int nnd_fetch_leaf_tables(nnd_ctx *ctx) {
    if (ctx->h_leaf_valid) return 0;
    const int64_t nl = ctx->n_leaves;
    ctx->h_leaf_start.resize(nl);
    ctx->h_leaf_len.resize(nl);
    if (nl > 0) {
        NND_HIP_CHECK(hipMemcpyAsync(ctx->h_leaf_start.data(), ctx->leaf_start, sizeof(int32_t) * nl, hipMemcpyDeviceToHost, ctx->stream));
        NND_HIP_CHECK(hipMemcpyAsync(ctx->h_leaf_len.data(), ctx->leaf_len, sizeof(int32_t) * nl, hipMemcpyDeviceToHost, ctx->stream));
        NND_HIP_CHECK(hipStreamSynchronize(ctx->stream));
    }
    ctx->h_leaf_valid = true;
    return 0;
}

int nnd_launch_leaf_array(nnd_ctx *ctx, int32_t *out_dev) {
    int64_t total = ctx->n_leaves * ctx->max_leaf;
    if (total == 0) return 0;
    hipLaunchKernelGGL(k_fill_leaf_array, dim3((unsigned)((total + 255) / 256)), dim3(256), 0, ctx->stream, ctx->perm[ctx->cur],
                       ctx->leaf_start, ctx->leaf_len, ctx->n_leaves, ctx->max_leaf, out_dev);
    NND_HIP_CHECK(hipGetLastError());
    return 0;
}
```

pynndescent_amd/csrc/state.h:

```cpp
#pragma once
#include <mutex>
#include <hip/hip_runtime.h>
#include <stdarg.h>
#include <stddef.h>
#include <stdint.h>
#include <stdio.h>

#include <vector>

#include "../../include/pynnd_amd.h"

#include <stdlib.h>
static inline const char *nnd_knob(const char *name) {
#ifdef NND_EXPERIMENT_KNOBS
    return getenv(name);
#else
    (void)name;
    return nullptr;
#endif
}

enum {
    CNT_ACCEPT = 0,
    CNT_PAIRS,
    CNT_ROWS,
    CNT_PROPOSALS,
    CNT_ACTIVE,
    CNT_DEGENERATE,
    CNT_ACTIVE_SEGS,
    CNT_LEAVES,
    CNT_SCRATCH,
    CNT_MFMA = 12,
    CNT_COUNT = 16
};
enum {
    CNT_ACTIVE_POS = CNT_LEAVES,
    CNT_SCAN_TOTAL = CNT_SCRATCH,
    CNT_FIN_COUNT = CNT_SCRATCH + 1,
    CNT_BIG_COUNT = CNT_SCRATCH + 2,
    CNT_SMALL_COUNT = CNT_SCRATCH + 3,
    CNT_REC_FLAGS = CNT_SCRATCH + 2,
    CNT_MAX_LEAF = CNT_SCRATCH + 2,
    CNT_MAX_STAY = CNT_SCRATCH + 3,
    CNT_PREP_FLAG = CNT_SCRATCH
};
static_assert(CNT_SMALL_COUNT < CNT_MFMA && CNT_MAX_STAY < CNT_MFMA, "the forest's scratch words end below CNT_MFMA");
static_assert(CNT_BIG_COUNT == CNT_FIN_COUNT + 1 && CNT_SMALL_COUNT == CNT_FIN_COUNT + 2, "k_cell_lists counts its three classes in adjacent words");
constexpr int NND_LEVEL_WORDS = 6;
struct nnd_level_words {
    long long segs;
    long long active_pos;
    long long scan_total, fin_count, rec_flags;
    long long max_stay;
};
static_assert(sizeof(nnd_level_words) == NND_LEVEL_WORDS * sizeof(long long), "hand-over layout");
static_assert(CNT_ACTIVE_POS == CNT_ACTIVE_SEGS + 1 && CNT_SCAN_TOTAL == CNT_ACTIVE_SEGS + 2 && CNT_FIN_COUNT == CNT_ACTIVE_SEGS + 3 &&
                  CNT_REC_FLAGS == CNT_ACTIVE_SEGS + 4 && CNT_MAX_STAY == CNT_ACTIVE_SEGS + NND_LEVEL_WORDS - 1,
              "nnd_level_words mirrors the counter layout");
struct nnd_level_flag {
    nnd_level_words w;
    long long seq;
};
static_assert(offsetof(nnd_level_flag, seq) == NND_LEVEL_WORDS * sizeof(long long), "k_children writes seq right behind the words");

struct nnd_sg_tail { uint32_t min_dist_bits, hi0; int32_t max_degree_out, hi1; };
struct nnd_pin_words {
    long long counters[CNT_COUNT];
    nnd_level_words level;
    long long fin_count;
    long long n_big, n_small;
    int32_t rec_flags[2];
    int32_t max_leaf[2];
    int32_t scan_total;
    int32_t sg_forward_nnz, sg_union_nnz, sg_final_nnz;
    long long sg_misc[5];
    nnd_sg_tail sg_tail;
    long long data_flags;
    alignas(64) nnd_level_flag flag;
    long long spare[17];
};
constexpr size_t NND_PIN_WORDS = 64;
static_assert(sizeof(nnd_pin_words) == NND_PIN_WORDS * sizeof(long long), "the pinned block is 64 words");
static_assert(offsetof(nnd_pin_words, n_small) == offsetof(nnd_pin_words, n_big) + sizeof(long long), "one copy brings both counts");

struct nnd_work_list { int32_t *start, *len, *depth; };
constexpr int NND_SEG_CHILD_WORDS = 2;
constexpr int NND_WORK_LIST_ROWS = 3;
constexpr int NND_ROUTE_TREES_MAX = 4096;
constexpr int NND_BY_CELL_TREES_MAX = 1024;
constexpr int NND_BY_CELL_RANK_TREES_MAX = 64;
constexpr int NND_ROUTE_ROOTS_WORDS = 4096;
constexpr int NND_RR_TREE_CELLS = 2048;
constexpr int NND_RR_TREE_POS = NND_RR_TREE_CELLS + NND_BY_CELL_RANK_TREES_MAX;
static_assert(NND_ROUTE_TREES_MAX <= NND_ROUTE_ROOTS_WORDS && NND_RR_TREE_POS + NND_BY_CELL_TREES_MAX + 1 <= NND_ROUTE_ROOTS_WORDS,
              "the sub-tables of route_roots fit its allocation");
#define NND_CNT_STRIPES 512

struct nnd_tlog { int ev; float *dst; bool add; };
struct nnd_hub_result;

struct nnd_handle_s {
    nnd_params p{};
    nnd_stats stats{};
    char err[512] = {0};
    hipStream_t stream = nullptr;
    hipEvent_t ev0 = nullptr, ev1 = nullptr;
    std::vector<hipEvent_t> tev;
    int tev_used = 0;
    std::vector<nnd_tlog> tlog;
    hipEvent_t ev_spin = nullptr;
    int (*wait_hook)(void *user, hipStream_t stream) = nullptr;
    void *wait_user = nullptr;

    int64_t n = 0;
    int d = 0, dp = 0;
    int k = 0, ks = 0;
    int mc = 0, mcp = 0;
    int rcap = 0, pcap = 0;
    int iter = 0;
    int64_t own_lo = 0, own_hi = 0;
    int n_ranks = 0;
    int64_t *shard_bounds = nullptr;
    long long *shard_cursors = nullptr;
    bool stream_owned = true;
    bool lists_replicated = false;
    const int32_t *own_order = nullptr;
    bool slim = false;
    void *slim_alloc[4] = {nullptr, nullptr, nullptr, nullptr};
    int64_t slim_rows() const { return slim ? own_hi - own_lo : n; }
    int64_t slim_row0() const { return slim ? own_lo : 0; }
    uint32_t seed = 0, tree_seed = 0;

    const float *x_orig = nullptr;
    bool x_owned = false;
    bool x_valid = false;
    float *xp = nullptr;
    float *nrm = nullptr;
    float2 *nr2 = nullptr;
    uint16_t *xh = nullptr;
    float *mean = nullptr;

    uint32_t *knn_e = nullptr;
    float *knn_d = nullptr;
    float *th = nullptr;

    int32_t *cand = nullptr;
    uint32_t *rbuf = nullptr;
    uint64_t *pbuf = nullptr;
    uint64_t *pbuf_r = nullptr;
    int pcap_r = 32;
    uint8_t *pdirty = nullptr;
    uint8_t *active = nullptr;

    int64_t P = 0;
    int32_t *perm[2] = {nullptr, nullptr};
    int32_t *pos_seg[2] = {nullptr, nullptr};
    int32_t *inv = nullptr;
    uint8_t *side = nullptr;
    uint8_t *side_pt = nullptr;
    uint8_t *leaf_flag = nullptr;
    int32_t *scan_out = nullptr;
    int32_t *scan_blk = nullptr;
    int32_t *seg_start[2] = {nullptr, nullptr}, *seg_len[2] = {nullptr, nullptr};
    int32_t *seg_nleft = nullptr, *seg_child = nullptr;
    float *hyper = nullptr;
    uint16_t *hyper_h = nullptr;
    int64_t max_segs = 0;
    int cur = 0;
    int64_t s_m = 0, s_stride = 0;
    int cell_leaf = 0;
    int early_stop = 8;
    float *xs = nullptr;
    uint16_t *xsh = nullptr;
    float2 *nr2s = nullptr;
    int64_t node_cap = 0, cell_cap = 0;
    float *node_hf = nullptr;
    uint16_t *node_hh = nullptr;
    int32_t *node_child = nullptr;
    unsigned char *node_pack = nullptr;
    float *node_hfc = nullptr;
    int32_t *route_roots = nullptr;
    unsigned char *route_ws = nullptr;
    size_t route_ws_cap = 0;
    int32_t *s_leaf_depth = nullptr;
    int32_t *cell_count = nullptr, *cell_start = nullptr, *cell_depth = nullptr;
    int32_t *small_list = nullptr;
    int32_t *leaf_start = nullptr, *leaf_len = nullptr;
    double *colsum_partial = nullptr;
    size_t colsum_cap = 0;
    int64_t leaf_cap = 0;
    std::vector<int32_t> h_leaf_start, h_leaf_len;
    bool h_leaf_valid = false;
    long long *tree_begin_dev = nullptr;
    long long *h_tree_begin = nullptr;
    int32_t *wl_start = nullptr, *wl_len = nullptr;
    int64_t wl_cap = 0;
    int64_t n_leaves = 0;
    int32_t max_leaf = 0;
    std::vector<int64_t> tree_leaf_begin;
    bool forest_built = false;
    bool all_new = false;
    int32_t *rv_pos = nullptr;
    int rv_pos_gen = -1;
    int forest_gen = 0;
    uint32_t *rv_in_cursor = nullptr;
    uint2 *rv_in_rec = nullptr;
    uint2 *rv_ov = nullptr;
    int64_t rv_cap_in = 0, rv_cap_ov = 0, rv_cap_pos = 0;
    int rv_in_cap = 0;
    const int32_t *rv_pos_of = nullptr;
    bool rv_off = false;
    bool jb_auto = false;
    int jb_max = 8, jb_div = 2, jb_first = 8;
    int64_t last_updates = -1;
    bool pbuf_clean = false, rbuf_clean = false;

    int32_t *out_idx = nullptr;
    float *out_dist = nullptr;
    size_t out_cap = 0;
    nnd_hub_result *hub = nullptr;
    struct nnd_sg_state *sg = nullptr;

    long long *counters = nullptr;
    long long h_counters[CNT_COUNT] = {0};
    long long *counters_sum = nullptr;
    nnd_pin_words *h_pin = nullptr;
    nnd_pin_words *h_pin_dev = nullptr;
    long long flag_seq = 0;

    void set_error(const char *fmt, ...) {
        va_list ap;
        va_start(ap, fmt);
        vsnprintf(err, sizeof(err), fmt, ap);
        va_end(ap);
    }
};
typedef nnd_handle_s nnd_ctx;

static inline int32_t *nnd_scan_total(const nnd_ctx *ctx) { return (int32_t *)(ctx->counters + CNT_SCAN_TOTAL); }
static inline nnd_work_list nnd_fin_list(const nnd_ctx *ctx) {
    int32_t *s = ctx->seg_child + NND_SEG_CHILD_WORDS * ctx->max_segs;
    return {s, s + ctx->max_segs, s + 2 * ctx->max_segs};
}
static inline nnd_work_list nnd_small_list(const nnd_ctx *ctx) {
    return {ctx->small_list, ctx->small_list + ctx->cell_cap, ctx->small_list + 2 * ctx->cell_cap};
}
static inline nnd_work_list nnd_big_list(const nnd_ctx *ctx) { return {ctx->seg_start[0], ctx->seg_len[0], ctx->seg_nleft}; }
static inline int32_t *nnd_route_tree_cells(const nnd_ctx *ctx) { return &ctx->route_roots[NND_RR_TREE_CELLS]; }
static inline int32_t *nnd_route_tree_pos(const nnd_ctx *ctx) { return &ctx->route_roots[NND_RR_TREE_POS]; }

int nnd_create_impl(nnd_handle_t *out, const nnd_params *p, const int64_t *bounds_host, int n_ranks, int rank);
int nnd_launch_prep(nnd_ctx *ctx);
bool nnd_prep_column_pass(int metric);
void nnd_prep_mean_geometry(int64_t n, int64_t *n_s, int64_t *stride);
int nnd_prep_partial_blocks(int64_t members);
double *nnd_prep_partial_buffer(nnd_ctx *ctx, size_t doubles);
int nnd_prep_mean_partial(nnd_ctx *ctx, const float *x_rows, int64_t row0, int64_t r_lo, int64_t r_hi, int64_t stride, double *partial);
int nnd_prep_mean_finish(nnd_ctx *ctx, const double *partial, int nblocks, int64_t n_s);
// ... 107 lines not shown
```

Measured before the change: 52.20 million.

## Overlap recorded-subtree finishing with forest level splits on an auxiliary stream

Adds an auxiliary HIP stream and events so that subtree-recording finisher kernels run in batches on that stream while the main stream continues splitting later tree levels. The scatter kernel now writes leaf members into a separate buffer so the finisher reads them without rewriting perm, and node packing gains a middle id range for nodes recorded early. The aim is to hide finisher latency behind level launches, at the cost of extra node-table reservation, more fallback conditions, and cross-stream synchronisation complexity.

Result: slower. 48.72 million (-6.7%).

```diff
diff --git a/include/pynnd_amd.h b/include/pynnd_amd.h
--- a/include/pynnd_amd.h
+++ b/include/pynnd_amd.h
@@ -53,6 +53,7 @@
 #define NND_FLAG_TEST_SELECT_HALF 4096
 #define NND_FLAG_TEST_GATHER_INLINE 8192
 #define NND_FLAG_TEST_JOIN_UNSTAGED 16384
+#define NND_FLAG_TEST_FOREST_SERIAL 32768
 
 typedef struct nnd_stats {
     int64_t n_iters_run;
@@ -115,6 +116,7 @@
                   int32_t errlen);
 
 int32_t nnd_get_stats(nnd_handle_t h, nnd_stats *out);
+int32_t nnd_forest_overlap_info(nnd_handle_t h, int32_t *rec_batches, int32_t *pass1_early);
 int32_t nnd_synchronize(nnd_handle_t h);
 
 int32_t nnd_get_graph(nnd_handle_t h, int32_t *idx, float *dist, uint8_t *flags);
diff --git a/pynndescent_amd/_capi.py b/pynndescent_amd/_capi.py
--- a/pynndescent_amd/_capi.py
+++ b/pynndescent_amd/_capi.py
@@ -27,6 +27,7 @@
 NND_FLAG_TEST_FOREST_FALLBACK_SHARE = 1024
 NND_FLAG_TEST_GATHER_INLINE = 8192
 NND_FLAG_TEST_JOIN_UNSTAGED = 16384
+NND_FLAG_TEST_FOREST_SERIAL = 32768
 NND_FLAG_TEST_SELECT_HALF = 4096
 NND_FLAG_TEST_SAMPLE_NOMEM = 2048
 NND_FLAG_TEST_SAMPLE_ATOMIC = 256
@@ -189,6 +190,7 @@
     ("nnd_build", C.c_int32, [C.POINTER(NNDParams), C.c_void_p, C.c_void_p, C.c_void_p, C.c_int32, C.c_void_p,
                               C.c_void_p, C.POINTER(NNDStats), C.c_char_p, C.c_int32]),
     ("nnd_get_stats", C.c_int32, [_H, C.POINTER(NNDStats)]),
+    ("nnd_forest_overlap_info", C.c_int32, [_H, C.POINTER(C.c_int32), C.POINTER(C.c_int32)]),
     ("nnd_synchronize", C.c_int32, [_H]),
     ("nnd_get_graph", C.c_int32, [_H, C.c_void_p, C.c_void_p, C.c_void_p]),
     ("nnd_get_candidates", C.c_int32, [_H, C.c_void_p, C.c_void_p]),
@@ -396,6 +398,11 @@
         self._check(self.lib.nnd_get_stats(self._h, C.byref(s)))
         return s if raw else s.as_dict()
 
+    def forest_overlap_info(self):
+        a, b = C.c_int32(), C.c_int32()
+        self._check(self.lib.nnd_forest_overlap_info(self._h, C.byref(a), C.byref(b)))
+        return a.value, bool(b.value)
+
     def graph(self):
         idx = np.empty((self.n, self.k), np.int32)
         dist = np.empty((self.n, self.k), np.float32)
diff --git a/pynndescent_amd/csrc/capi.hip b/pynndescent_amd/csrc/capi.hip
--- a/pynndescent_amd/csrc/capi.hip
+++ b/pynndescent_amd/csrc/capi.hip
@@ -101,6 +101,8 @@
     F(ctx->shard_bounds); F(ctx->shard_cursors);
     nnd_hub_tree_free(ctx);
     nnd_search_graph_free(ctx);
+    for (hipEvent_t &e : ctx->ev_aux) { if (e) (void)hipEventDestroy(e); e = nullptr; }
+    if (ctx->aux) { (void)hipStreamDestroy(ctx->aux); ctx->aux = nullptr; }
     if (ctx->stream && ctx->stream_owned) (void)hipStreamDestroy(ctx->stream);
 }
 
@@ -188,6 +190,10 @@
     int rc = 0;
     do {
         if (hipStreamCreateWithFlags(&ctx->stream, hipStreamNonBlocking) != hipSuccess) { ctx->set_error("hipStreamCreate failed"); rc = 1; break; }
+        if (hipStreamCreateWithFlags(&ctx->aux, hipStreamNonBlocking) != hipSuccess) { ctx->set_error("hipStreamCreate failed"); rc = 1; break; }
+        for (hipEvent_t &e : ctx->ev_aux)
+            if (hipEventCreateWithFlags(&e, hipEventDisableTiming) != hipSuccess) { ctx->set_error("hipEventCreate failed"); rc = 1; break; }
+        if (rc) break;
         if (hipEventCreate(&ctx->ev0) != hipSuccess || hipEventCreate(&ctx->ev1) != hipSuccess ||
             hipEventCreateWithFlags(&ctx->ev_spin, hipEventDisableTiming) != hipSuccess) { ctx->set_error("hipEventCreate failed"); rc = 1; break; }
         const size_t n = (size_t)ctx->n;
@@ -309,6 +315,7 @@
     std::lock_guard<std::recursive_mutex> lifecycle(nnd_lifecycle_mutex());
     (void)hipSetDevice(ctx->p.device);
     if (ctx->stream) (void)hipStreamSynchronize(ctx->stream);
+    if (ctx->aux) (void)hipStreamSynchronize(ctx->aux);
     free_all(ctx);
     delete ctx;
 }
@@ -913,6 +920,13 @@
     return 0;
 }
 
+extern "C" int32_t nnd_forest_overlap_info(nnd_handle_t ctx, int32_t *rec_batches, int32_t *pass1_early) {
+    if (!ctx) { gerr("null argument"); return 1; }
+    if (rec_batches) *rec_batches = ctx->forest_rec_batches;
+    if (pass1_early) *pass1_early = ctx->forest_pass1_early;
+    return 0;
+}
+
 extern "C" int32_t nnd_synchronize(nnd_handle_t ctx) {
     ENTER(ctx);
     API_HIP(nnd_sync_spin(ctx));
diff --git a/pynndescent_amd/csrc/rpforest.hip b/pynndescent_amd/csrc/rpforest.hip
--- a/pynndescent_amd/csrc/rpforest.hip
+++ b/pynndescent_amd/csrc/rpforest.hip
@@ -497,7 +497,7 @@
                           const uint8_t *__restrict__ side, const int32_t *__restrict__ scan,
                           const int32_t *__restrict__ seg_start, const int32_t *__restrict__ nleft,
                           const int32_t *__restrict__ seg_child, int64_t P, int64_t n, int32_t *__restrict__ perm_out,
-                          int32_t *__restrict__ pos_seg_out, int32_t *__restrict__ inv) {
+                          int32_t *__restrict__ pos_seg_out, int32_t *__restrict__ inv, int32_t *__restrict__ left_out) {
     int64_t g = (int64_t)blockIdx.x * blockDim.x + threadIdx.x;
     if (g >= P) return;
     int s = pos_seg[g];
@@ -521,9 +521,11 @@
         dest = right ? (int64_t)a + nl + ((int)(g - a) - L) : (int64_t)a + L;
     }
     int32_t p = perm[g];
+    const int32_t child = seg_child[2 * s + right];
     perm_out[dest] = p;
-    pos_seg_out[dest] = seg_child[2 * s + right];
-    if (inv) inv[(g / n) * n + p] = seg_child[2 * s + right];
+    pos_seg_out[dest] = child;
+    if (inv) inv[(g / n) * n + p] = child;
+    if (left_out && child < 0) left_out[dest] = p;
 }
 
 #ifndef NND_FIN_MAX
@@ -559,6 +561,7 @@
     int hs, node_top, down_base, lvl_end;
     int *counter, *overflow;
     int min_len, max_len;
+    int read_only_members;
 };
 struct rp_tree_map {
     int tree_bias = 0;
@@ -862,7 +865,7 @@
         }
         __syncthreads();
     }
-    if (!BIG)
+    if (!BIG && !(RECORD && rec.read_only_members))
         for (int i = tid; i < len; i += NTHR) perm[a + i] = ids[i];
 }
 
@@ -933,14 +936,25 @@
     int64_t n_low, high_lo;
     int node_base, cell_base;
     const int32_t *cell_gid;
+    int64_t mid_lo = 0, n_mid = 0;
 };
+__device__ __forceinline__ int64_t rp_pack_source(const rp_pack_map &mp, int64_t vp) {
+    if (vp < mp.n_low) return vp;
+    if (vp < mp.n_low + mp.n_mid) return mp.mid_lo + (vp - mp.n_low);
+    return mp.high_lo + (vp - mp.n_low - mp.n_mid);
+}
+__device__ __forceinline__ int rp_pack_id(const rp_pack_map &mp, int64_t v) {
+    if (v < mp.n_low) return (int)v;
+    if (v >= mp.high_lo) return (int)(v - mp.high_lo + mp.n_low + mp.n_mid);
+    return (int)(v - mp.mid_lo + mp.n_low);
+}
 __global__ void k_pack_nodes(const uint16_t *__restrict__ node_hh, const float *__restrict__ node_hf, int hs,
                              const int32_t *__restrict__ node_child, const int32_t *__restrict__ leafscan, int dp, int64_t n_packed,
                              rp_pack_map mp, unsigned char *__restrict__ pack, float *__restrict__ hf_out) {
     const int sub = threadIdx.x & 15;
     const int64_t vp = (int64_t)blockIdx.x * (blockDim.x >> 4) + (threadIdx.x >> 4);
     if (vp >= n_packed) return;
-    const int64_t v = vp < mp.n_low ? vp : mp.high_lo + (vp - mp.n_low);
+    const int64_t v = rp_pack_source(mp, vp);
     const int rec = 2 * dp + 16;
     uint4 *dst = (uint4 *)(pack + vp * rec);
     const uint4 *src = (const uint4 *)(node_hh + v * dp);
@@ -954,7 +968,7 @@
         for (int q = 0; q < 2; q++) {
             const int c = node_child[2 * v + q];
             if (c >= 0) {
-                ch[q] = (int)((int64_t)c < mp.n_low ? c : c - (mp.high_lo - mp.n_low)) + mp.node_base;
+                ch[q] = rp_pack_id(mp, c) + mp.node_base;
             } else {
                 const int lc = leafscan[-2 - c];
                 ch[q] = -2 - (mp.cell_gid ? mp.cell_gid[lc] : mp.cell_base + lc);
@@ -1623,13 +1637,20 @@
     nnd_level_flag *flag_dev = nullptr;
     std::vector<int64_t> level_base;
     int64_t n_low = 0, high_lo = 0;
+    int64_t mid_lo = 0, n_mid = 0;
+    bool overlap = false;
+    bool forked = false;
+    bool flags_pending = false;
+    long long fin_seen = 0, fin_done = 0;
+    int64_t fin_reserve = 0;
+    int n_batches = 0;
 };
 
 template <bool BIG, int NTHR, int CAP, bool RECORD = false>
 static forest_rc launch_finisher(nnd_ctx *ctx, const forest_rows &r, int32_t *perm, int32_t *other, const nnd_work_list &wl, int depth0,
-                                 long long count, const rp_tree_map &tm, const rp_record &rec = rp_record{}) {
+                                 long long count, const rp_tree_map &tm, const rp_record &rec = rp_record{}, hipStream_t stream = nullptr) {
     const nnd_work_list fin = nnd_fin_list(ctx);
-    hipLaunchKernelGGL((k_finish_subtrees<BIG, NTHR, CAP, RECORD>), dim3((unsigned)count), dim3(NTHR), fin_smem_bytes(ctx->dp, CAP), ctx->stream,
+    hipLaunchKernelGGL((k_finish_subtrees<BIG, NTHR, CAP, RECORD>), dim3((unsigned)count), dim3(NTHR), fin_smem_bytes(ctx->dp, CAP), stream ? stream : ctx->stream,
                        r.xp, r.xh, r.nr, ctx->p.metric, ctx->dp, r.n, perm, wl.start, wl.len, wl.depth, depth0, (int)count,
                        nnd_metric_unit(ctx->p.metric), ctx->tree_seed, ctx->p.max_depth, r.leaf_size, ctx->leaf_flag,
                        BIG ? other : (int32_t *)nullptr, BIG ? ctx->side : (uint8_t *)nullptr, FIN_MAX, fin.start, fin.len, fin.depth,
@@ -1678,6 +1699,16 @@
     v.flag_dev = (ctx->h_pin_dev && !ctx->wait_hook && !nnd_knob("NND_NO_LEVEL_FLAG")) ? &ctx->h_pin_dev->flag : nullptr;
     long long *fin_count = ctx->counters + CNT_FIN_COUNT;
     FOREST_HIP_CHECK(hipMemsetAsync(fin_count, 0, sizeof(long long), ctx->stream));
+    v.forked = v.flags_pending = false;
+    v.fin_seen = v.fin_done = 0;
+    v.n_batches = 0;
+    v.mid_lo = v.n_mid = 0;
+    if (v.overlap) {
+        v.fin_reserve = v.P / (v.rows.leaf_size + 1) + 1;
+        if (!v.record || !ctx->aux || v.fin_reserve > ctx->max_segs || 3 * v.fin_reserve > ctx->node_cap || 2 * v.P > ctx->P) v.overlap = false;
+    }
+    if (v.overlap)
+        FOREST_HIP_CHECK(hipMemsetAsync(ctx->counters + CNT_REC_FLAGS, 0, 2 * sizeof(int), ctx->stream));
     if (!v.record && v.S > 0 && n <= v.fin_max) {
         const nnd_work_list fin = nnd_fin_list(ctx);
         std::vector<int32_t> h_s(T), h_l(T), h_d(T, 0);
@@ -1693,6 +1724,8 @@
     return FOREST_OK;
 }
 
+static int32_t *rec_members(const nnd_ctx *ctx, const forest_view &v) { return ctx->perm[0] + v.P; }
+
 static forest_rc level_launch(nnd_ctx *ctx, forest_view &v) {
     const forest_rows &r = v.rows;
     const int64_t n = r.n, P = v.P, S = v.S, node_base = v.node_base;
@@ -1704,7 +1737,7 @@
         ctx->set_error("rp-forest: %lld segments exceed the allocation of %lld", (long long)S, (long long)ctx->max_segs);
         return FOREST_ERROR;
     }
-    if (v.record && node_base + S > ctx->node_cap) return forest_fallback("a recorded level outgrows the node tables");
+    if (v.record && node_base + S > ctx->node_cap - (v.overlap ? v.fin_reserve : 0)) return forest_fallback("a recorded level outgrows the node tables");
     if (v.record) v.level_base.push_back(node_base);
     float *hyper = v.record ? ctx->node_hf + node_base * hs : ctx->hyper;
     uint16_t *hyper_h = v.record ? ctx->node_hh + node_base * dp : ctx->hyper_h;
@@ -1734,7 +1767,7 @@
                        (int)ctx->node_cap - 1, (long long *)v.flag_dev, v.flag_dev ? ++ctx->flag_seq : 0);
     hipLaunchKernelGGL(k_scatter, dim3(gridP), dim3(256), 0, ctx->stream, ctx->perm[cur], ctx->pos_seg[cur], ctx->side,
                        ctx->scan_out, ctx->seg_start[cur], ctx->seg_nleft, ctx->seg_child, P, n, ctx->perm[1 - cur],
-                       ctx->pos_seg[1 - cur], v.inv_live ? ctx->inv : (int32_t *)nullptr);
+                       ctx->pos_seg[1 - cur], v.inv_live ? ctx->inv : (int32_t *)nullptr, v.overlap ? rec_members(ctx, v) : (int32_t *)nullptr);
     FOREST_HIP_CHECK(hipGetLastError());
     return FOREST_OK;
 }
@@ -1761,7 +1794,77 @@
     return FOREST_OK;
 }
 
+static forest_rc aux_fork(nnd_ctx *ctx, forest_view &v) {
+    hipEvent_t ev = ctx->ev_aux[v.n_batches % 3];
+    FOREST_HIP_CHECK(hipEventRecord(ev, ctx->stream));
+    FOREST_HIP_CHECK(hipStreamWaitEvent(ctx->aux, ev, 0));
+    v.forked = true;
+    return FOREST_OK;
+}
+static forest_rc aux_join(nnd_ctx *ctx, forest_view &v) {
+    if (!v.forked) return FOREST_OK;
+    v.forked = false;
+    FOREST_HIP_CHECK(hipEventRecord(ctx->ev_aux[3], ctx->aux));
+    FOREST_HIP_CHECK(hipStreamWaitEvent(ctx->stream, ctx->ev_aux[3], 0));
+    return FOREST_OK;
+}
+
+static constexpr long long REC_TAIL_WG = 256;
+static constexpr long long REC_BATCH_MIN = 64;
+
+static forest_rc record_batch(nnd_ctx *ctx, forest_view &v, bool last) {
+    const long long lo = v.fin_done, cnt = v.fin_seen - lo;
+    if (cnt <= 0) return FOREST_OK;
+    forest_rc rc = aux_fork(ctx, v);
+    if (rc) return rc;
+    int *flags = (int *)(ctx->counters + CNT_REC_FLAGS);
+    rp_record rec{ctx->node_hf, ctx->node_hh, ctx->node_child, ctx->s_leaf_depth, ctx->dp + 4, (int)(ctx->node_cap - 1 - lo),
+                  (int)(ctx->node_cap - 1 - v.fin_reserve), (int)v.node_base, flags, flags + 1, 0, FIN_MAX, 1};
+    nnd_work_list fin = nnd_fin_list(ctx);
+    fin.start += lo; fin.len += lo; fin.depth += lo;
+    int32_t *members = rec_members(ctx, v);
+    if (last && cnt <= REC_TAIL_WG) {
+        rc = launch_finisher<false, 256, FIN_MAX, true>(ctx, v.rows, members, nullptr, fin, 0, cnt, v.tm, rec, ctx->aux);
+    } else {
+        rp_record rs = rec, rl = rec;
+        rs.max_len = FIN_SMALL;
+        rl.min_len = FIN_SMALL + 1;
+        rc = launch_finisher<false, 64, FIN_SMALL, true>(ctx, v.rows, members, nullptr, fin, 0, cnt, v.tm, rs, ctx->aux);
+        if (!rc && v.fin_max > FIN_SMALL) rc = launch_finisher<false, 256, FIN_MAX, true>(ctx, v.rows, members, nullptr, fin, 0, cnt, v.tm, rl, ctx->aux);
+    }
+    v.fin_done = v.fin_seen;
+    v.n_batches++;
+    return rc;
+}
+
+static forest_rc record_subtrees_batched(nnd_ctx *ctx, forest_view &v) {
+    v.level_base.push_back(v.node_base);
+    v.n_low = v.node_base;
+    v.high_lo = ctx->node_cap - v.fin_seen;
+    forest_rc rc;
+    if (v.fin_seen > v.fin_reserve) {
+        (void)aux_join(ctx, v);
+        return forest_fallback("the subtrees to record outgrow the node tables");
+    }
+    if ((rc = record_batch(ctx, v, true)) || (rc = aux_join(ctx, v))) return rc;
+    v.flags_pending = v.fin_seen > 0;
+    return FOREST_OK;
+}
+static forest_rc record_flags_read(nnd_ctx *ctx, forest_view &v, const nnd_level_words &w) {
+    v.flags_pending = false;
+    const int n_ids = (int)(uint32_t)(w.rec_flags & 0xFFFFFFFFll), overflow = (int)(w.rec_flags >> 32);
+    if (w.fin_count != v.fin_seen) {
+        ctx->set_error("rp-forest: the finisher work list holds %lld entries, %lld were handed over", w.fin_count, v.fin_seen);
+        return FOREST_ERROR;
+    }
+    v.mid_lo = ctx->node_cap - v.fin_reserve - n_ids;
+    v.n_mid = n_ids;
+    if (overflow || v.mid_lo <= v.n_low) return forest_fallback("the recording finisher ran out of node slots");
+    return FOREST_OK;
+}
+
 static forest_rc record_subtrees(nnd_ctx *ctx, forest_view &v) {
+    if (v.overlap) return record_subtrees_batched(ctx, v);
     const int64_t node_base = v.node_base;
     v.level_base.push_back(node_base);
     forest_rc rc;
@@ -1800,6 +1903,8 @@
         v.active_pos = next.active_pos;
         v.cur = 1 - v.cur;
         v.depth++;
+        v.fin_seen = next.fin_count;
+        if (v.overlap && v.S > 0 && v.fin_seen - v.fin_done >= REC_BATCH_MIN && (rc = record_batch(ctx, v, false))) return rc;
         if (!v.record && v.S > 0 && (v.active_pos * 2 < 3 * v.rows.n) && next.max_stay <= BIG_MAX) {
             const nnd_work_list stayers{ctx->seg_start[v.cur], ctx->seg_len[v.cur], nullptr};
             return launch_finishers(ctx, ctx->perm[v.cur], ctx->perm[1 - v.cur], stayers, v.depth, v.S, 0, v.tm);
@@ -2005,9 +2110,21 @@
 
 static forest_rc forest_tops(nnd_ctx *ctx, forest_view &v, int32_t *n_cells_out) {
     forest_rc rc = forest_levels(ctx, v);
-    if (rc) return rc;
+    if (rc) {
+        (void)aux_join(ctx, v);
+        return rc;
+    }
     int32_t n_cells = 0;
-    if ((rc = run_scan(ctx, 1, nullptr, ctx->leaf_flag, nnd_scan_total(ctx), v.P, v.rows.n)) || (rc = read_scan_total(ctx, &n_cells))) return rc;
+    if ((rc = run_scan(ctx, 1, nullptr, ctx->leaf_flag, nnd_scan_total(ctx), v.P, v.rows.n))) return rc;
+    if (v.flags_pending) {
+        FOREST_HIP_CHECK(hipMemcpyAsync(&ctx->h_pin->level, ctx->counters + CNT_ACTIVE_SEGS, sizeof(nnd_level_words), hipMemcpyDeviceToHost, ctx->stream));
+        FOREST_HIP_CHECK(nnd_sync_spin(ctx));
+        const nnd_level_words w = ctx->h_pin->level;
+        n_cells = (int32_t)w.scan_total;
+        if ((rc = record_flags_read(ctx, v, w))) return rc;
+    } else if ((rc = read_scan_total(ctx, &n_cells))) {
+        return rc;
+    }
     if (n_cells > ctx->cell_cap) return forest_fallback("the recorded trees have more cells than the cell tables hold");
     hipLaunchKernelGGL(k_cell_depths, dim3((unsigned)((v.P + 255) / 256)), dim3(256), 0, ctx->stream, ctx->leaf_flag, ctx->scan_out,
                        ctx->s_leaf_depth, v.P, ctx->cell_depth);
@@ -2047,13 +2164,16 @@
                        dp, (int64_t)0, M, ctx->s_stride, ctx->tree_seed, ctx->xs, ctx->xsh, ctx->nr2s);
     static const int rec_fin = [] { const char *e = nnd_knob("NND_REC_FIN"); const int r = e ? atoi(e) : FIN_SMALL; return r <= FIN_SMALL ? FIN_SMALL : FIN_MAX; }();
     forest_view v{{ctx->xs, ctx->xsh, ctx->nr2s, M, ctx->cell_leaf}, Ps, rec_fin, true};
+    v.overlap = !ctx->wait_hook && !(ctx->p.flags & (NND_FLAG_TEST_FOREST_SERIAL | NND_FLAG_TEST_ROUTE_PLAIN));
+    ctx->forest_rec_batches = 0;
     int32_t n_cells = 0;
     forest_rc rc = forest_tops(ctx, v, &n_cells);
     if (rc) return rc;
+    ctx->forest_rec_batches = v.overlap ? v.n_batches : 0;
     if (n_cells + P / (ctx->p.leaf_size + 1) > ctx->max_segs) return forest_fallback("cells and leaves could outgrow the segment tables");
     FOREST_HIP_CHECK(hipMemsetAsync(ctx->cell_count, 0, sizeof(int32_t) * (size_t)n_cells, ctx->stream));
-    const int64_t n_packed = v.n_low + (ctx->node_cap - v.high_lo);
-    rp_pack_map mp{v.n_low, v.high_lo, 0, 0, nullptr};
+    const int64_t n_packed = v.n_low + v.n_mid + (ctx->node_cap - v.high_lo);
+    rp_pack_map mp{v.n_low, v.high_lo, 0, 0, nullptr, v.mid_lo, v.n_mid};
     hipLaunchKernelGGL(k_pack_nodes, dim3((unsigned)((n_packed + 15) / 16)), dim3(256), 0, ctx->stream, ctx->node_hh, ctx->node_hf,
                        dp + 4, ctx->node_child, ctx->scan_out, dp, n_packed, mp, ctx->node_pack, ctx->node_hfc);
     int32_t *roots = ctx->route_roots;
@@ -2310,7 +2430,7 @@
     hipLaunchKernelGGL(k_seg_count, dim3((unsigned)((n_segs + 255) / 256)), dim3(256), 0, ctx->stream, seg_start, seg_len, n_segs,
                        ctx->scan_out, scan_total, n, nleft);
     hipLaunchKernelGGL(k_scatter, dim3((unsigned)((n + 255) / 256)), dim3(256), 0, ctx->stream, ord, pos, side, ctx->scan_out, seg_start,
-                       nleft, seg_child, n, n, ord_out, pos_out, (int32_t *)nullptr);
+                       nleft, seg_child, n, n, ord_out, pos_out, (int32_t *)nullptr, (int32_t *)nullptr);
 }
 
 int nnd_fetch_leaf_tables(nnd_ctx *ctx) {
diff --git a/pynndescent_amd/csrc/state.h b/pynndescent_amd/csrc/state.h
--- a/pynndescent_amd/csrc/state.h
+++ b/pynndescent_amd/csrc/state.h
@@ -104,6 +104,10 @@
     nnd_stats stats{};
     char err[512] = {0};
     hipStream_t stream = nullptr;
+    hipStream_t aux = nullptr;
+    hipEvent_t ev_aux[4] = {nullptr, nullptr, nullptr, nullptr};
+    int forest_rec_batches = 0;
+    int forest_pass1_early = 0;
     hipEvent_t ev0 = nullptr, ev1 = nullptr;
     std::vector<hipEvent_t> tev;
     int tev_used = 0;
```
